# shanjiayao/PTT

Measured on AMD Instinct MI355X. Metric: tracklet frames/sec (hot path: PointNet++ SA stack + Point-Track-Transformer blocks), higher is better.
Workload: dtype f32

## Files before the change

include/ptt_hip.h:

```cpp
#ifndef PTT_HIP_H
#define PTT_HIP_H

#include <stddef.h>
#include <stdint.h>

#ifdef __cplusplus
extern "C" {
#endif

#define PTT_ABI_VERSION 31

enum {
    PTT_OK = 0,
    PTT_EINVAL = -1,
    PTT_EUNSUPPORTED = -2,
    PTT_ELAUNCH = -3,
    PTT_EWORKSPACE = -4
};

typedef void* ptt_stream_t;

int ptt_version(void);
const char* ptt_error_name(int code);
const char* ptt_last_error_string(void);

int ptt_fps_f32(const float* xyz, int B, int N, int npoint, int32_t* idx_out,
                ptt_stream_t stream);
int ptt_fps_ws_f32(const float* xyz, int B, int N, int npoint, int32_t* idx_out, float* workspace,
                   size_t workspace_elems, ptt_stream_t stream);

int ptt_ffps_f32(const float* xyz, const float* feat, int64_t feat_sb, int64_t feat_sc, int64_t feat_sn,
                 int B, int N, int C, int npoint, int32_t* idx_out, ptt_stream_t stream);

int ptt_gather_f32(const float* feat, const int32_t* idx, int B, int C, int N, int M,
                   float* out, ptt_stream_t stream);
int ptt_gather_grad_f32(const float* grad_out, const int32_t* idx, int B, int C, int N,
                        int M, float* grad_feat, ptt_stream_t stream);

int ptt_select_centres_f32(const float* xyz, const int32_t* idx, int B, int N, int M, float* new_xyz,
                           int64_t* idx64_out, ptt_stream_t stream);

int ptt_ball_query_f32(const float* new_xyz, const float* xyz, int B, int M, int N,
                       float radius, int nsample, int32_t* idx_out, ptt_stream_t stream);

int ptt_centres_ball_query_f32(const float* xyz, const int32_t* sel, int B, int N, int M, float radius, int nsample,
                               float* new_xyz, int64_t* idx64_out, int32_t* idx_out, ptt_stream_t stream);

int ptt_group_f32(const float* feat, const int32_t* idx, int B, int C, int N, int M,
                  int ns, float* out, ptt_stream_t stream);
int ptt_group_grad_f32(const float* grad_out, const int32_t* idx, int B, int C, int N,
                       int M, int ns, float* grad_feat, ptt_stream_t stream);

size_t ptt_scatter_add_det_workspace(int B, int N, int E);
int ptt_scatter_add_det_f32(const float* src, const int32_t* idx, int B, int C, int N, int E, float* out,
                            void* workspace, size_t workspace_bytes, ptt_stream_t stream);

int ptt_knn_f32(const float* xyz, int B, int N, int k, int32_t* idx_out,
                ptt_stream_t stream);
int ptt_knn_rel_f32(const float* xyz, int B, int N, int k, int32_t* idx_out, float* rel_out,
                    ptt_stream_t stream);

size_t ptt_packed_weight_elems(int Cout, int K);
int ptt_pack_weight_f32(const float* W, int Cout, int K, float* packed,
// ... 211 lines not shown
    float* template_points;
    float* cls_label;
    float* reg_label;
    int32_t* src_out;
    int32_t* idx_search_out;
    int32_t* idx_template_out;
    int32_t* info;
    int64_t* totals;
    int32_t B, n_cand;
    int32_t search_size, template_size;
    int32_t min_points;
    uint32_t seed_lo, seed_hi;
    int32_t reserved;
} ptt_train_batch_desc;

int ptt_train_batch_f32(const ptt_train_cand* cands_device, const ptt_train_batch_desc* desc_host, ptt_stream_t stream);
int ptt_philox4x32_10(const uint32_t* counter4, const uint32_t* key2, uint32_t* out4);

size_t ptt_bn_stats_workspace(int R, int C);
int ptt_bn_stats_f32(const float* X, int R, int C, int ldx, float eps, float* mean, float* var, float* invstd,
                     void* workspace, size_t workspace_bytes, ptt_stream_t stream);
int ptt_bn_apply_f32(const float* Z, int ldz, const float* mean, const float* invstd, const float* gamma,
                     const float* beta, int R, int C, int relu, float* X, int ldx, ptt_stream_t stream);
int ptt_bn_bwd_f32(const float* G, int ldg, const float* Act, int lda, const float* Z, int ldz, const float* mean,
                   const float* invstd, const float* gamma, int R, int C, int relu, float* dZ, int ldd,
                   float* dgamma, float* dbeta, void* workspace, size_t workspace_bytes, const float* act_scale,
                   const float* act_shift, ptt_stream_t stream);
int ptt_bn_sums_f64(const float* X, int R, int C, int ldx, double* sums, void* workspace, size_t workspace_bytes,
                    ptt_stream_t stream);
int ptt_bn_finish_f64(const double* sums, int C, float eps, float* mean, float* var, float* invstd,
                      ptt_stream_t stream);
int ptt_bn_bwd_sums_f64(const float* G, int ldg, const float* Act, int lda, const float* Z, int ldz, const float* mean,
                        const float* invstd, int R, int C, double* sums, void* workspace, size_t workspace_bytes,
                        const float* act_scale, const float* act_shift, ptt_stream_t stream);
int ptt_bn_bwd_apply_f32(const float* G, int ldg, const float* Act, int lda, const float* Z, int ldz, const float* mean,
                         const float* invstd, const float* gamma, const float* sum_dy, const float* sum_dy_xhat,
                         const double* count, int R, int C, float* dZ, int ldd, const float* act_scale, const float* act_shift,
                         ptt_stream_t stream);
int ptt_pool_rows_f32(const float* X, int ldx, int G, int ns, int C, float* out, int ldo, int32_t* arg,
                      const float* act_scale, const float* act_shift, ptt_stream_t stream);
int ptt_pool_rows_bwd_f32(const float* dOut, int ldo, const int32_t* arg, int G, int ns, int C, float* dX, int ldx,
                          ptt_stream_t stream);
int ptt_pt_pair_input_f32(const float* q, const float* kf, const int32_t* knn, const float* pos, int B, int N, int k, int D,
                          float* t, ptt_stream_t stream);
int ptt_pt_attn_train_fwd_f32(const float* a, const float* vf, const int32_t* knn, const float* pos, int B, int N, int k, int D,
                              float scale, float* attn, float* res, ptt_stream_t stream);
int ptt_pt_attn_train_bwd_f32(const float* attn, const float* vf, const int32_t* knn, const float* pos, const float* dres, int B,
                              int N, int k, int D, float scale, float* da, float* dvp, ptt_stream_t stream);

int ptt_pt_pair_input_ld_f32(const float* q, int ldq, const float* kf, int ldk, const int32_t* knn, const float* pos, int B, int N,
                             int k, int D, float* t, ptt_stream_t stream);
int ptt_pt_attn_fwd_ld_f32(const float* a, const float* vf, int ldv, const int32_t* knn, const float* pos, int B, int N, int k, int D,
                           float scale, float* attn, float* res, ptt_stream_t stream);

int ptt_gather_rows_f32(const float* src, const int32_t* idx, int B, int N, int E, int C, float* out, ptt_stream_t stream);
int ptt_scatter_csr_i32(const int32_t* idx, int B, int N, int E, int32_t* order, int32_t* start, ptt_stream_t stream);
int ptt_scatter_rows_csr_f32(const float* g, const int32_t* order, const int32_t* start, int B, int N, int E, int C,
                             float* out, ptt_stream_t stream);
int ptt_rows_gemm_pool_supported(int rows, int K, int N, int ldx, int ns);
int ptt_rows_gemm_pool_f32(const float* X, int rows, int K, int ldx, const float* in_scale, const float* in_shift,
                           const float* Wpacked, int N, float* out, int ldo, double* stats, size_t stats_elems, int ns,
                           float* pmax, float* pmin, int32_t* amax, int32_t* amin, ptt_stream_t stream);
int ptt_pool_select_f32(const float* pmax, const float* pmin, const int32_t* amax, const int32_t* amin, const float* act_scale,
                        const float* act_shift, int G, int C, float* out, int32_t* arg, ptt_stream_t stream);
size_t ptt_colsum_workspace(int R, int C);
int ptt_colsum_f32(const float* X, int R, int C, int ldx, float* out, void* workspace, size_t workspace_bytes, ptt_stream_t stream);
size_t ptt_linear_wgrad_workspace(int R, int Cout, int Cin);
int ptt_linear_wgrad_f32(const float* dZ, int ldz, const float* X, int ldx, int R, int Cout, int Cin, float* dW,
                         int accumulate, void* workspace, size_t workspace_bytes, const float* x_scale, const float* x_shift,
                         ptt_stream_t stream);
int ptt_linear_act_in_f32(const float* X, int rows, int K, int ldx, const float* in_scale, const float* in_shift,
                          const float* Wpacked, int Cout, float* out, int ldo, ptt_stream_t stream);

int ptt_pack_weight_strided_f32(const float* W, int Cout, int K, int64_t stride_out, int64_t stride_k, int batch,
                                int64_t stride_batch, float* packed, ptt_stream_t stream);
int ptt_linear_batched_f32(const float* X, int rows, int K, int ldx, int64_t x_batch_stride, const float* Wpacked,
                           int64_t w_batch_stride, int Cout, const float* scale, const float* shift, int relu,
                           const float* residual, int ldr, int64_t r_batch_stride, float* out, int ldo,
                           int64_t o_batch_stride, int batch, ptt_stream_t stream);
int ptt_softmax_rows_f32(float* X, int64_t rows, int n, int ld, float scale, ptt_stream_t stream);
int ptt_layernorm_f32(const float* x, int rows, int C, int ldx, const float* weight, const float* bias, float eps,
                      const float* residual, int ldr, float* out, int ldo, ptt_stream_t stream);

int ptt_rows_gemm_supported(int rows, int K, int N, int ldx, int ldo);
int ptt_rows_gemm_stat_chunks(int rows, int K, int N);
int ptt_rows_gemm_f32(const float* X, int rows, int K, int ldx, const float* in_scale, const float* in_shift,
                      const float* Wpacked, int N, const float* bias, int relu, const float* residual, int ldr,
                      float* out, int ldo, double* stats, size_t stats_elems, ptt_stream_t stream);
int ptt_rows_gemm_masked_f32(const float* X, int rows, int K, int ldx, const float* Wpacked, int N, const float* mask, int ldm,
                             float* out, int ldo, double* stats, size_t stats_elems, ptt_stream_t stream);
int ptt_rows_gemm_bnbwd_f32(const float* X, int rows, int K, int ldx, const float* Wpacked, int N, const float* Z, int ldz,
                            const float* mean, const float* invstd, const float* act_scale, const float* act_shift, float* out,
                            int ldo, double* sums_partial, size_t partial_elems, ptt_stream_t stream);
int ptt_bn_bwd_from_partials_f32(const double* partial, int chunks, const float* G, int ldg, const float* Z, int ldz, const float* mean,
                                 const float* invstd, const float* gamma, int R, int C, float* dZ, int ldd, float* dgamma, float* dbeta,
                                 const float* act_scale, const float* act_shift, ptt_stream_t stream);
int ptt_bn_bwd_sums_partials_f64(const double* partial, int chunks, int C, double* sums, ptt_stream_t stream);
typedef struct ptt_bn_bwd_input {
    const float* g; int ldg;
    const int32_t* arg; int ns;
    const float* z; int ldz;
    const float* k1; const float* c0; const float* c1; const float* mean;
    const float* act_a; const float* act_b;
    float* dz_out; int ldd;
} ptt_bn_bwd_input;
int ptt_bn_bwd_consts_f32(const double* partial, int chunks, const float* mean, const float* invstd, const float* gamma, int R, int C,
                          float* dgamma, float* dbeta, float* k1, float* c0, float* c1, ptt_stream_t stream);
int ptt_bn_bwd_pooled_consts_f32(const float* dPooled, int ldp, const int32_t* arg, int ns, const float* Z, int ldz, const float* mean,
                                 const float* invstd, const float* gamma, int R, int C, float* dgamma, float* dbeta, float* k1,
                                 float* c0, float* c1, void* workspace, size_t workspace_bytes, const float* act_scale,
                                 const float* act_shift, ptt_stream_t stream);
int ptt_rows_gemm_bnbwd_fused_supported(int rows, int K, int N, int ns);
int ptt_rows_gemm_bnbwd_fused_f32(const ptt_bn_bwd_input* in, int rows, int K, const float* Wpacked, int N, const float* Z, int ldz,
                                  const float* mean, const float* invstd, const float* act_scale, const float* act_shift, float* out,
                                  int ldo, double* sums_partial, size_t partial_elems, ptt_stream_t stream);
int ptt_bn_finish_partials_f32(const double* partial, int chunks, int C, int R, float eps, float* mean, float* var, float* invstd,
                               ptt_stream_t stream);
int ptt_bn_sums_partials_f64(const double* partial, int chunks, int C, int R, double* sums, ptt_stream_t stream);
int ptt_bn_bwd_pooled_f32(const float* dPooled, int ldp, const int32_t* arg, int ns, const float* Z, int ldz, const float* mean,
                          const float* invstd, const float* gamma, int R, int C, float* dZ, int ldd, float* dgamma, float* dbeta,
                          void* workspace, size_t workspace_bytes, const float* act_scale, const float* act_shift, ptt_stream_t stream);
int ptt_bn_bwd_pooled_sums_f64(const float* dPooled, int ldp, const int32_t* arg, int ns, const float* Z, int ldz, const float* mean,
                               const float* invstd, int R, int C, double* sums, void* workspace, size_t workspace_bytes,
                               const float* act_scale, const float* act_shift, ptt_stream_t stream);
int ptt_bn_bwd_pooled_apply_f32(const float* dPooled, int ldp, const int32_t* arg, int ns, const float* Z, int ldz, const float* mean,
                                const float* invstd, const float* gamma, const float* sum_dy, const float* sum_dy_xhat,
                                const double* count, int R, int C, float* dZ, int ldd, const float* act_scale,
                                const float* act_shift, ptt_stream_t stream);
int ptt_bn_update_running_f32(const float* mean, const float* var, const double* count, float momentum, int C, float* running_mean,
                              float* running_var, int64_t* num_batches_tracked, ptt_stream_t stream);
int ptt_xcorr_z0_f32(const float* P, const float* cos_t, const float* w_sim, int B, int n2, int n1, int C, float* z0, ptt_stream_t stream);
int ptt_xcorr_z0_stat_chunks(int B, int n2, int n1, int C);
int ptt_xcorr_z0_stats_f32(const float* P, const float* cos_t, const float* w_sim, int B, int n2, int n1, int C, float* z0,
                           double* stats_partial, size_t partial_elems, ptt_stream_t stream);
size_t ptt_xcorr_z0_bwd_workspace(int B, int n1, int C);
int ptt_xcorr_z0_bnbwd_f32(const double* partial, int chunks, const float* G, const float* P, const float* cos_t, const float* w_sim,
                           const float* mean, const float* invstd, const float* gamma, const float* act_scale, const float* act_shift,
                           int B, int n2, int n1, int C, float* dP, float* dcos, float* dw, float* dgamma, float* dbeta, void* workspace,
                           size_t workspace_bytes, ptt_stream_t stream);
int ptt_xcorr_z0_bwd_f32(const float* dz0, const float* cos_t, const float* w_sim, int B, int n2, int n1, int C, float* dP, float* dcos,
                         float* dw, void* workspace, size_t workspace_bytes, ptt_stream_t stream);
int ptt_sa_z0_rows_f32(const float* xyz, const float* new_xyz, const int32_t* idx, const float* term, const float* wx, int ldw, int B,
                       int N, int M, int ns, int C, float radius, int normalize_xyz, float* z0, float* rel_rows, ptt_stream_t stream);
int ptt_sa_z0_rows_stat_chunks(int B, int M, int ns, int C);
int ptt_sa_z0_rows_stats_f32(const float* xyz, const float* new_xyz, const int32_t* idx, const float* term, const float* wx, int ldw, int B,
                             int N, int M, int ns, int C, float radius, int normalize_xyz, float* z0, float* rel_rows,
                             double* stats_partial, size_t partial_elems, ptt_stream_t stream);
typedef struct ptt_bn_train_tail {
    const float* gamma; const float* beta;
    float* act_a; float* act_b;
    float* running_mean; float* running_var;
    int64_t* num_batches_tracked;
    float momentum;
} ptt_bn_train_tail;
int ptt_bn_stats_train_f32(const float* X, int R, int C, int ldx, float eps, float* mean, float* var, float* invstd,
                           void* workspace, size_t workspace_bytes, const ptt_bn_train_tail* tail, ptt_stream_t stream);
int ptt_bn_finish_partials_train_f32(const double* partial, int chunks, int C, int R, float eps, float* mean, float* var,
                                     float* invstd, const ptt_bn_train_tail* tail, ptt_stream_t stream);
typedef struct ptt_pack_job {
    const float* W;
    int64_t out_offset, stride_out, stride_k;
    int32_t Cout, K;
} ptt_pack_job;
int ptt_pack_weights_f32(const ptt_pack_job* jobs_device, int n_jobs, float* arena, ptt_stream_t stream);
size_t ptt_linear_wgrad2_workspace(int R, int Cout, int Cin);
int ptt_linear_wgrad2_f32(const float* dZ, int ldz, const float* X, int ldx, int R, int Cout, int Cin, float* dW,
                          int accumulate, void* workspace, size_t workspace_bytes, const float* x_scale, const float* x_shift,
                          ptt_stream_t stream);

typedef struct ptt_track_loss_desc {
    const float* seed_cls;
    const float* cls_label;
    const int64_t* search_inds;
    const float* votes;
    const float* reg_label;
    const float* box_data;
    const float* centres;
    const float* pos_weight_seed;
    const float* pos_weight_box;
    int32_t B, N, Ns, M, ld_reg;
    float w_seed_cls, w_seed_reg, w_box_cls, w_box_reg;
} ptt_track_loss_desc;
int ptt_track_losses_f32(const ptt_track_loss_desc* desc, float* out8, float* total , ptt_stream_t stream);
int ptt_track_losses_bwd_f32(const ptt_track_loss_desc* desc, const float* out8, const float* upstream, float* d_seed_cls,
                             float* d_votes, float* d_box_data, ptt_stream_t stream);
typedef struct ptt_adam_tensor {
    float* param;
    float* grad;
    float* exp_avg;
    float* exp_avg_sq;
    int64_t n;
} ptt_adam_tensor;
typedef struct ptt_adam_hyper {
    float beta1, beta2, one_minus_beta1, one_minus_beta2 , eps, step_size, bias2_sqrt,
          weight_decay, max_norm;
    int32_t write_clipped;
} ptt_adam_hyper;
int ptt_adam_chunk_elems(void);
int ptt_adam_clip_step_f32(const ptt_adam_tensor* tensors_device, const int32_t* chunk_tensor_device, const int64_t* chunk_first_device,
                           int n_chunks, const ptt_adam_hyper* hyper, double* partial, size_t partial_elems, float* norm_out,
                           ptt_stream_t stream);
int ptt_adam_clip_step_dev_f32(const ptt_adam_tensor* tensors_device, const int32_t* chunk_tensor_device, const int64_t* chunk_first_device,
                               int n_chunks, const ptt_adam_hyper* hyper_device, int clip, double* partial, size_t partial_elems,
                               float* norm_out, ptt_stream_t stream);
int ptt_unit_rows_f32(const float* x, long long sb, long long sn, long long sc, int B, int n, int C, float eps, float* unit, float* nrm,
                      ptt_stream_t stream);
int ptt_cos_bwd_rows_f32(const float* A, const float* unit, const float* nrm, const float* G, const float* cosm, long long map_sb,
                         long long own, long long other, int m, int B, int n, int C, float* dx, long long sb, long long sn, long long sc,
                         ptt_stream_t stream);
size_t ptt_sa_z0_bnbwd_workspace(long long R, int C);
int ptt_sa_z0_bnbwd_f32(const double* partial, int chunks, const float* G, const float* Z0, const float* rel_rows, const float* mean,
                        const float* invstd, const float* gamma, const float* act_scale, const float* act_shift, long long R, int C,
                        float* dz_out, float* dwx, float* dgamma, float* dbeta, void* workspace, size_t workspace_bytes, ptt_stream_t stream);

typedef struct ptt_grad_job {
    const float* partial;
    int32_t nchunks, reserved;
} ptt_grad_job;
typedef struct ptt_grad_segment {
    int64_t dst;
    int32_t n, cols, ld, job0, njobs, out, vec, reserved;
} ptt_grad_segment;
int ptt_linear_wgrad_partials_f32(const float* dZ, int ldz, const float* X, int ldx, int R, int Cout, int Cin, void* workspace,
                                  size_t workspace_bytes, const float* x_scale, const float* x_shift, int* nchunks, ptt_stream_t stream);
int ptt_linear_wgrad2_partials_f32(const float* dZ, int ldz, const float* X, int ldx, int R, int Cout, int Cin, void* workspace,
                                   size_t workspace_bytes, const float* x_scale, const float* x_shift, int* nchunks, ptt_stream_t stream);
int ptt_colsum_partials_f32(const float* X, int R, int C, int ldx, void* workspace, size_t workspace_bytes, int* nchunks,
                            ptt_stream_t stream);
int ptt_grad_finish_f32(const ptt_grad_segment* segments_device, const ptt_grad_job* jobs_device, const int32_t* blocks_device,
                        int n_blocks, float* flat, ptt_stream_t stream);

int ptt_rows_gemm_rsum16_supported(int rows, int K, int N, int ldx);
int ptt_rows_gemm_rsum16_f32(const float* X, int rows, int K, int ldx, const float* Wpacked, int N, const float* residual, int ldr,
                             float* out, int ldo, float* plain, int ldp, float* gsum, int ldg, ptt_stream_t stream);
int ptt_scatter_rows_csr_sub_f32(const float* g, const int32_t* order, const int32_t* start, int B, int N, int E, int C,
                                 const float* minuend, float* out, ptt_stream_t stream);

int ptt_layernorm_train_fwd_f32(const float* x, int rows, int C, int ldx, const float* weight, const float* bias, float eps,
                                const float* residual, int ldr, float* out, int ldo, float* mean, float* rstd, ptt_stream_t stream);
size_t ptt_layernorm_bwd_workspace(int rows, int C);
int ptt_layernorm_bwd_f32(const float* dy, int ldg, const float* x, int ldx, const float* mean, const float* rstd, const float* weight,
                          int rows, int C, float* dx, int ldd, float* dweight, float* dbias, void* workspace, size_t workspace_bytes,
                          ptt_stream_t stream);
int ptt_rows_gemm_rsum16_heads_supported(int rows, int D, int hd, int ldx);
int ptt_rows_gemm_rsum16_heads_f32(const float* X, int rows, int D, int hd, int ldx, const float* Wpacked, const float* residual, int ldr,
                                   float* out, int ldo, float* plain, int ldp, float* gsum, int ldg, ptt_stream_t stream);

#ifdef __cplusplus
}
#endif
#endif
```

ptt_amd/_lib.py:

```python
import ctypes
import os
import re
from ctypes import Structure, c_char_p, c_double, c_float, c_int, c_int32, c_int64, c_longlong, c_size_t, c_uint32, c_void_p

from .build import HEADER as HEADER_PATH, LIB as LIB_PATH


def _strip_comments(text):
    return re.sub(r"/\*.*?\*/|//[^\n]*", " ", text, flags=re.S)


def parse_defines(text):
    return {n: int(v) for n, v in re.findall(r"^[ \t]*#[ \t]*define[ \t]+(PTT_\w+)[ \t]+(-?\d+)[ \t]*$", _strip_comments(text), re.M)}


CTYPES = {"int": c_int, "int32_t": c_int32, "uint32_t": c_uint32, "int64_t": c_int64, "long long": c_longlong, "size_t": c_size_t,
          "float": c_float, "double": c_double, "ptt_stream_t": c_void_p}


def _ctype(decl, name, is_return=False):
    words = decl.replace("*", " * ").split()
    if not is_return and len(words) > 1 and words[-1] != "*":
        words.pop()
    if "*" in words:
# ... 37 lines not shown
EXPORTS = list(PROTOTYPES)
DEFINES = parse_defines(_header)
ABI_VERSION = DEFINES["PTT_ABI_VERSION"]
PTT_SA_MAX_LAYERS = DEFINES["PTT_SA_MAX_LAYERS"]
PTT_MAX_SEGMENTS = DEFINES["PTT_MAX_SEGMENTS"]
PTT_CROP_JOBS_BY_VALUE_MAX = DEFINES["PTT_CROP_JOBS_BY_VALUE_MAX"]
PTT_TRAIN_MAX_CANDS = DEFINES["PTT_TRAIN_MAX_CANDS"]


class CropJob(Structure):
    _fields_ = [("points", c_void_p), ("ld", c_int64),
                ("lo1", c_double * 3), ("hi1", c_double * 3), ("trans", c_double * 3), ("rot", c_double * 9),
                ("lo2", c_double * 3), ("hi2", c_double * 3),
                ("out", c_void_p), ("count", c_void_p), ("n_points", c_int32), ("capacity", c_int32),
                ("label_out", c_void_p), ("ltrans", c_double * 3), ("lrot", c_double * 9), ("llo", c_double * 3), ("lhi", c_double * 3),
                ("append", c_int32), ("reserved", c_int32)]


class RegularizeJob(Structure):
    _fields_ = [("seg", c_void_p * PTT_MAX_SEGMENTS), ("seg_count", c_void_p * PTT_MAX_SEGMENTS),
                ("seg_capacity", c_int32 * PTT_MAX_SEGMENTS), ("out", c_void_p), ("info", c_void_p),
                ("n_seg", c_int32), ("input_size", c_int32)]


class TrackBox(Structure):
    _fields_ = [("center", c_double * 3), ("wlh", c_double * 3), ("quat", c_double * 4)]


class TrainCand(Structure):
    _fields_ = [("search", c_void_p), ("label", c_void_p), ("first", c_void_p), ("prev", c_void_p), ("counts", c_void_p),
                ("reg", c_float * 4), ("index", c_uint32), ("epoch", c_uint32), ("capacity", c_int32), ("reserved", c_int32)]


class TrainBatchDesc(Structure):
    _fields_ = [("search_points", c_void_p), ("template_points", c_void_p), ("cls_label", c_void_p), ("reg_label", c_void_p),
                ("src_out", c_void_p), ("idx_search_out", c_void_p), ("idx_template_out", c_void_p), ("info", c_void_p), ("totals", c_void_p),
                ("B", c_int32), ("n_cand", c_int32), ("search_size", c_int32), ("template_size", c_int32), ("min_points", c_int32),
                ("seed_lo", c_uint32), ("seed_hi", c_uint32), ("reserved", c_int32)]


class BnTrainTail(Structure):
    _fields_ = [("gamma", c_void_p), ("beta", c_void_p), ("act_a", c_void_p), ("act_b", c_void_p),
                ("running_mean", c_void_p), ("running_var", c_void_p), ("num_batches_tracked", c_void_p), ("momentum", c_float)]


class BnBwdInput(Structure):
    _fields_ = [("g", c_void_p), ("ldg", c_int), ("arg", c_void_p), ("ns", c_int), ("z", c_void_p), ("ldz", c_int),
                ("k1", c_void_p), ("c0", c_void_p), ("c1", c_void_p), ("mean", c_void_p), ("act_a", c_void_p), ("act_b", c_void_p),
                ("dz_out", c_void_p), ("ldd", c_int)]


class PackJob(Structure):
    _fields_ = [("W", c_void_p), ("out_offset", c_int64), ("stride_out", c_int64), ("stride_k", c_int64),
                ("Cout", c_int32), ("K", c_int32)]


class RowJob(Structure):
    _fields_ = [("X", c_void_p), ("X2", c_void_p), ("Xmax", c_void_p), ("Wpacked", c_void_p), ("scale", c_void_p), ("shift", c_void_p),
                ("res", c_void_p), ("res2", c_void_p), ("out", c_void_p), ("out2", c_void_p), ("raw", c_void_p),
                ("rel", c_void_p), ("w1", c_void_p), ("qkv", c_void_p), ("knn", c_void_p), ("pos", c_void_p),
                ("rows", c_int32), ("K", c_int32), ("K1", c_int32), ("ldx", c_int32), ("ldx2", c_int32), ("Cout", c_int32),
                ("act", c_int32), ("res_split", c_int32), ("ldr", c_int32), ("ldr2", c_int32), ("out_split", c_int32),
                ("out_col0", c_int32), ("ldo", c_int32), ("ldo2", c_int32), ("ldraw", c_int32),
                ("prologue", c_int32), ("epilogue", c_int32), ("ldq", c_int32), ("q_off", c_int32), ("k_off", c_int32),
                ("v_off", c_int32), ("ldp", c_int32), ("N", c_int32), ("sm_scale", c_float), ("col_tiles", c_int32),
                ("idx", c_void_p), ("xyz", c_void_p), ("centres", c_void_p), ("wx", c_void_p), ("radius", c_float),
                ("ns", c_int32), ("M", c_int32), ("normalize_xyz", c_int32), ("pro_relu", c_int32)]


class PointJob(Structure):
    _fields_ = [("xyz", c_void_p), ("centre_sel", c_void_p), ("point_sel", c_void_p), ("new_xyz", c_void_p), ("idx64_out", c_void_p),
                ("idx_out", c_void_p), ("rel_out", c_void_p), ("kind", c_int32), ("sel_ld", c_int32), ("B", c_int32),
                ("Nraw", c_int32), ("Npts", c_int32), ("M", c_int32), ("nsample", c_int32), ("radius", c_float)]


class TrackLossDesc(Structure):
    _fields_ = [("seed_cls", c_void_p), ("cls_label", c_void_p), ("search_inds", c_void_p), ("votes", c_void_p), ("reg_label", c_void_p),
                ("box_data", c_void_p), ("centres", c_void_p), ("pos_weight_seed", c_void_p), ("pos_weight_box", c_void_p),
                ("B", c_int32), ("N", c_int32), ("Ns", c_int32), ("M", c_int32), ("ld_reg", c_int32),
                ("w_seed_cls", c_float), ("w_seed_reg", c_float), ("w_box_cls", c_float), ("w_box_reg", c_float)]


class AdamTensor(Structure):
    _fields_ = [("param", c_void_p), ("grad", c_void_p), ("exp_avg", c_void_p), ("exp_avg_sq", c_void_p), ("n", c_int64)]


class GradJob(Structure):
    _fields_ = [("partial", c_void_p), ("nchunks", c_int32), ("reserved", c_int32)]


class GradSegment(Structure):
    _fields_ = [("dst", c_int64), ("n", c_int32), ("cols", c_int32), ("ld", c_int32), ("job0", c_int32), ("njobs", c_int32), ("out", c_int32),
                ("vec", c_int32), ("reserved", c_int32)]


class AdamHyper(Structure):
    _fields_ = [("beta1", c_float), ("beta2", c_float), ("one_minus_beta1", c_float), ("one_minus_beta2", c_float), ("eps", c_float), ("step_size", c_float), ("bias2_sqrt", c_float),
                ("weight_decay", c_float), ("max_norm", c_float), ("write_clipped", c_int32)]


class SaLayer(Structure):
    _fields_ = [("Wpacked", c_void_p), ("scale", c_void_p), ("shift", c_void_p),
                ("Cin", c_int), ("Cout", c_int), ("relu", c_int)]


class SaDesc(Structure):
    _fields_ = [("xyz", c_void_p), ("new_xyz", c_void_p), ("idx", c_void_p), ("feat", c_void_p),
# ... 58 lines not shown
```

ptt_amd/csrc/gemm_ops.hip:

```cpp
#include <atomic>
#include <math.h>
#include <stdlib.h>
#include <type_traits>
#include "common.h"

namespace ptt {

typedef float g32x16 __attribute__((ext_vector_type(16)));
typedef float g32x4 __attribute__((ext_vector_type(4)));
typedef int gi32x4 __attribute__((ext_vector_type(4)));
typedef unsigned int gu32x4 __attribute__((__vector_size__(4 * sizeof(unsigned int))));

namespace {

__device__ __forceinline__ __amdgpu_buffer_rsrc_t g_rsrc(const void* p) {
    return __builtin_amdgcn_make_buffer_rsrc(const_cast<void*>(p), 0, 0x7fffffff, 0x00020000);
}
__device__ __forceinline__ g32x4 g_load4(__amdgpu_buffer_rsrc_t r, int voff, int soff) {
    return __builtin_bit_cast(g32x4, __builtin_amdgcn_raw_buffer_load_b128(r, voff, soff, 0));
}
__device__ __forceinline__ float g_load1(__amdgpu_buffer_rsrc_t r, int voff, int soff) {
    return __builtin_bit_cast(float, __builtin_amdgcn_raw_buffer_load_b32(r, voff, soff, 0));
}
__device__ __forceinline__ void g_store1(float v, __amdgpu_buffer_rsrc_t r, int voff, int soff) {
// ... 500 lines not shown
void launch_wgrad_finish(const float* partial, int nchunks, size_t n, int accumulate, float* dW, hipStream_t s);

static int cu_count() {
    constexpr int MAX_DEV = 64;
    static std::atomic<int> cached[MAX_DEV];
    int dev = 0;
    if (hipGetDevice(&dev) != hipSuccess || dev < 0 || dev >= MAX_DEV) return 256;
    int n = cached[dev].load(std::memory_order_relaxed);
    if (n == 0) {
        int v = 0;
        n = (hipDeviceGetAttribute(&v, hipDeviceAttributeMultiprocessorCount, dev) == hipSuccess && v > 0) ? v : 256;
        cached[dev].store(n, std::memory_order_relaxed);
    }
    return n;
}

struct RowsGemmGeom { int WR, RT, CT, KC, TR, ncg, ntiles, G, chunks; bool ok; };
static RowsGemmGeom rows_gemm_geom(int rows, int K, int N) {
    RowsGemmGeom g{};
    g.ok = false;
    if (rows <= 0 || K <= 0 || N <= 0) return g;
    if (N % 128 == 0 && K % 128 == 0) {
        const int tiles64 = (rows + 63) / 64;
        g.WR = 1; g.RT = 2; g.KC = 128;
        g.CT = (N % 256 == 0 && (long long)tiles64 * (N / 256) >= 2 * cu_count()) ? 2 : 1;
    }
    else if (N % 128 == 0 && K % 64 == 0) { g.WR = 1; g.RT = 4; g.CT = 1; g.KC = 64; }
    else if (N % 64 == 0 && K % 64 == 0) { g.WR = 2; g.RT = 2; g.CT = 1; g.KC = 64; }
    else return g;
    const int WC = 4 / g.WR;
    g.TR = 32 * g.RT * g.WR;
    g.ncg = N / (32 * WC * g.CT);
    g.ntiles = (rows + g.TR - 1) / g.TR;
    int cap = 2 * cu_count() / g.ncg;
    if (cap >= 8) cap &= ~7;
    if (cap < 1) cap = 1;
    g.G = g.ntiles < cap ? g.ntiles : cap;
    g.chunks = g.G * g.WR;
    g.ok = true;
    return g;
}

}

using namespace ptt;

extern "C" int ptt_rows_gemm_supported(int rows, int K, int N, int ldx, int ldo) {
    const RowsGemmGeom g = rows_gemm_geom(rows, K, N);
    if (!g.ok) return 0;
    if ((long long)rows * ldx >= (1LL << 29) || (long long)rows * ldo >= (1LL << 29) || (ldx & 3)) return 0;
    return 1;
}

extern "C" int ptt_rows_gemm_stat_chunks(int rows, int K, int N) {
    const RowsGemmGeom g = rows_gemm_geom(rows, K, N);
    return g.ok ? g.chunks : 0;
}

struct BnBwdArgs { const float* z; int ldz; const float* mean; const float* invstd; const float* a; const float* b; };
struct PoolArgs { float* pmax; float* pmin; int32_t* amax; int32_t* amin; int ns; };
struct GroupSumArgs { float* gsum; int ldgs; float* plain; int ldpl; int hd; };
static int rows_gemm_launch(const float* X, int rows, int K, int ldx, const float* in_scale, const float* in_shift,
                            const float* Wpacked, int N, const float* bias, int relu, const float* residual, int ldr,
                            const float* mask, int ldm, float* out, int ldo, double* stats, size_t stats_elems, ptt_stream_t stream,
                            const BnBwdArgs* bn = nullptr, const PoolArgs* pool = nullptr, const ptt_bn_bwd_input* ain = nullptr,
                            const GroupSumArgs* gs = nullptr);

extern "C" int ptt_rows_gemm_rsum16_supported(int rows, int K, int N, int ldx) {
    if (!ptt_rows_gemm_supported(rows, K, N, ldx, N) || rows % 16) return 0;
    const RowsGemmGeom g = rows_gemm_geom(rows, K, N);
    return (g.WR == 1 && g.RT == 2 && g.KC == 128) ? 1 : 0;
}

extern "C" int ptt_rows_gemm_rsum16_f32(const float* X, int rows, int K, int ldx, const float* Wpacked, int N, const float* residual,
                                        int ldr, float* out, int ldo, float* plain, int ldp, float* gsum, int ldg,
                                        ptt_stream_t stream) {
    if (!residual || !plain || !gsum || ldp < N || ldg < N) return fail(PTT_EINVAL, "ptt_rows_gemm_rsum16_f32: null pointer or ldp / ldg < N");
    if ((long long)rows * ldp >= (1LL << 31)) return fail(PTT_EUNSUPPORTED, "ptt_rows_gemm_rsum16_f32: rows * ldp >= 2^31");
    if (!ptt_rows_gemm_rsum16_supported(rows, K, N, ldx))
        return fail(PTT_EUNSUPPORTED, "ptt_rows_gemm_rsum16_f32: rows=%d K=%d N=%d (whole groups of 16 rows, K %% 128 == 0, N %% 128 == 0)", rows, K, N);
    const GroupSumArgs gs{gsum, ldg, plain, ldp, 0};
    return rows_gemm_launch(X, rows, K, ldx, nullptr, nullptr, Wpacked, N, nullptr, 0, residual, ldr, nullptr, 0, out, ldo, nullptr, 0, stream,
                            nullptr, nullptr, nullptr, &gs);
}

extern "C" int ptt_rows_gemm_rsum16_heads_supported(int rows, int D, int hd, int ldx) {
    if (hd <= 0 || D <= 0 || D % hd || hd % 128) return 0;
    return ptt_rows_gemm_rsum16_supported(rows, D, D, ldx);
}

extern "C" int ptt_rows_gemm_rsum16_heads_f32(const float* X, int rows, int D, int hd, int ldx, const float* Wpacked, const float* residual,
                                              int ldr, float* out, int ldo, float* plain, int ldp, float* gsum, int ldg,
                                              ptt_stream_t stream) {
    if (!residual || !plain || !gsum || ldp < D || ldg < D)
        return fail(PTT_EINVAL, "ptt_rows_gemm_rsum16_heads_f32: null pointer or ldp / ldg < D");
    if ((long long)rows * ldp >= (1LL << 31)) return fail(PTT_EUNSUPPORTED, "ptt_rows_gemm_rsum16_heads_f32: rows * ldp >= 2^31");
    if (!ptt_rows_gemm_rsum16_heads_supported(rows, D, hd, ldx))
        return fail(PTT_EUNSUPPORTED, "ptt_rows_gemm_rsum16_heads_f32: rows=%d D=%d hd=%d (whole groups of 16 rows, D %% hd == 0, hd %% 128 == 0)",
                    rows, D, hd);
    const GroupSumArgs gs{gsum, ldg, plain, ldp, hd};
    return rows_gemm_launch(X, rows, D, ldx, nullptr, nullptr, Wpacked, D, nullptr, 0, residual, ldr, nullptr, 0, out, ldo, nullptr, 0, stream,
                            nullptr, nullptr, nullptr, &gs);
}

extern "C" int ptt_rows_gemm_bnbwd_fused_supported(int rows, int K, int N, int ns) {
    if (!ptt_rows_gemm_supported(rows, K, N, K, N) || (ns != 0 && ns != 16 && ns != 32 && ns != 64) || (ns > 0 && rows % ns)) return 0;
// ... 197 lines not shown
        else if (stats) PTT_RG_LAUNCH(WR_, RT_, CT_, KC_, true, false)                                                  \
        else if (in_scale) PTT_RG_LAUNCH(WR_, RT_, CT_, KC_, false, true)                                               \
        else PTT_RG_LAUNCH(WR_, RT_, CT_, KC_, false, false)                                                            \
    }
    PTT_RG_CASE(1, 2, 2, 128, PTT_RG_AINS) PTT_RG_CASE(1, 2, 1, 128, PTT_RG_AINS) PTT_RG_CASE(1, 4, 1, 64, PTT_RG_NO_AINS)
    PTT_RG_CASE(2, 2, 1, 64, PTT_RG_AINS)
#undef PTT_RG_CASE
#undef PTT_RG_AINS
#undef PTT_RG_NO_AINS
#undef PTT_RG_AIN
#undef PTT_RG_LAUNCH
    return check_launch("rows_gemm_kernel");
}

namespace ptt {
#ifndef PTT_WG2_MIN_ROWS
#define PTT_WG2_MIN_ROWS 768
#endif
struct Wgrad2Geom { int TN, TK, BN, BK, nbo, nbk, chunk_rows, nchunks; bool ok; };
static Wgrad2Geom wgrad2_geom(int R, int Cout, int Cin) {
    Wgrad2Geom g{};
    g.ok = false;
    if (R < 2048 || Cout % 128 || Cin % 128) return g;
    const int ncu = cu_count();
    const int cand[4][2] = {{4, 2}, {4, 1}, {2, 2}, {2, 1}};
    int first = 0;
#ifdef PTT_GEMM_DEV
    if (const char* e = getenv("PTT_WG2_FIRST")) first = atoi(e);
#endif
    for (int k = first; k < 4; ++k) {
        const int TN = cand[k][0], TK = cand[k][1];
        if (Cout % (64 * TN) || Cin % (128 * TK)) continue;
        const int blocks = (Cout / (64 * TN)) * (Cin / (128 * TK));
        if (blocks > ncu) continue;
        int nch = ncu / blocks;
        int rows = (R + nch - 1) / nch;
        if (rows < PTT_WG2_MIN_ROWS) rows = PTT_WG2_MIN_ROWS;
        rows = (rows + 31) & ~31;
        const int nchunks = (R + rows - 1) / rows;
        if (nchunks * blocks * 4 < ncu * 3 && k < 3) continue;
        if (nchunks * blocks * 2 < ncu) break;
        g.TN = TN; g.TK = TK; g.BN = 64 * TN; g.BK = 128 * TK; g.nbo = Cout / g.BN; g.nbk = Cin / g.BK;
        g.chunk_rows = rows; g.nchunks = nchunks; g.ok = true;
        return g;
    }
    return g;
}
}

extern "C" size_t ptt_linear_wgrad2_workspace(int R, int Cout, int Cin) {
    const Wgrad2Geom g = wgrad2_geom(R, Cout, Cin);
    return g.ok ? (size_t)g.nchunks * Cout * Cin * sizeof(float) : 0;
}

static int linear_wgrad2_run(const float* dZ, int ldz, const float* X, int ldx, int R, int Cout, int Cin, float* dW,
                             int accumulate, void* ws, size_t ws_bytes, const float* x_scale, const float* x_shift,
                             int* nchunks_out, ptt_stream_t stream) {
    const Wgrad2Geom g = wgrad2_geom(R, Cout, Cin);
    if (!g.ok || (ldz & 3) || (ldx & 3) || ((reinterpret_cast<uintptr_t>(dZ) | reinterpret_cast<uintptr_t>(X)) & 15) ||
        (long long)R * ldz >= (1LL << 29) || (long long)R * ldx >= (1LL << 29))
        return fail(PTT_EUNSUPPORTED, "ptt_linear_wgrad2_f32: R=%d Cout=%d Cin=%d ldz=%d ldx=%d (needs R >= 2048, Cout %% 128 == 0, "
                                      "Cin %% 128 == 0, 16-byte aligned rows)", R, Cout, Cin, ldz, ldx);
    if (ldz < Cout || ldx < Cin || !dZ || !X || (!dW && !nchunks_out)) return fail(PTT_EINVAL, "ptt_linear_wgrad2_f32: bad argument");
    if (x_scale && (!x_shift || ((reinterpret_cast<uintptr_t>(x_scale) | reinterpret_cast<uintptr_t>(x_shift)) & 15)))
        return fail(PTT_EINVAL, "ptt_linear_wgrad2_f32: the input transform needs 16-byte aligned scale / shift");
    if (!ws || ws_bytes < ptt_linear_wgrad2_workspace(R, Cout, Cin)) return fail(PTT_EWORKSPACE, "ptt_linear_wgrad2_f32: workspace too small");
    hipStream_t s = as_stream(stream);
    const int lds = 2 * 32 * (g.BN + 4 + g.BK + 4) * (int)sizeof(float);
    const dim3 grid(g.nbo * g.nbk * g.nchunks);
    int rc = PTT_OK;
#define PTT_WG2_CASE(TN_, TK_)                                                                                          \
    if (g.TN == TN_ && g.TK == TK_) {                                                                                   \
        if ((rc = set_lds_limit(reinterpret_cast<const void*>(wgrad2_kernel<TN_, TK_>), lds))) return rc;               \
        hipLaunchKernelGGL((wgrad2_kernel<TN_, TK_>), grid, dim3(512), lds, s, dZ, ldz, X, ldx, R, Cout, Cin, g.nbk, g.chunk_rows, \
                           static_cast<float*>(ws), x_scale, x_shift);                                                  \
    }
#ifdef PTT_GEMM_DEV
    if (const char* e = getenv("PTT_WG2_EXP")) {
        const int x = atoi(e);
#define PTT_WG2_EXP_CASE(X)                                                                                             \
        if (x == X && g.TN == 4 && g.TK == 2) {                                                                         \
            if ((rc = set_lds_limit(reinterpret_cast<const void*>(wgrad2_kernel<4, 2, X>), lds))) return rc;            \
            hipLaunchKernelGGL((wgrad2_kernel<4, 2, X>), grid, dim3(512), lds, s, dZ, ldz, X_, ldx, R, Cout, Cin, g.nbk, g.chunk_rows, \
                               static_cast<float*>(ws), x_scale, x_shift);                                              \
            return check_launch("wgrad2_kernel(exp)");                                                                  \
        }
        const float* X_ = X;
        PTT_WG2_EXP_CASE(1) PTT_WG2_EXP_CASE(2) PTT_WG2_EXP_CASE(3) PTT_WG2_EXP_CASE(4) PTT_WG2_EXP_CASE(7) PTT_WG2_EXP_CASE(8)
        PTT_WG2_EXP_CASE(15) PTT_WG2_EXP_CASE(16) PTT_WG2_EXP_CASE(31)
#undef PTT_WG2_EXP_CASE
    }
#endif
    PTT_WG2_CASE(4, 2) PTT_WG2_CASE(4, 1) PTT_WG2_CASE(2, 2) PTT_WG2_CASE(2, 1)
#undef PTT_WG2_CASE
    if (dW) launch_wgrad_finish(static_cast<const float*>(ws), g.nchunks, (size_t)Cout * Cin, accumulate, dW, s);
    if (nchunks_out) *nchunks_out = g.nchunks;
    return check_launch("wgrad2_kernel");
}
extern "C" int ptt_linear_wgrad2_f32(const float* dZ, int ldz, const float* X, int ldx, int R, int Cout, int Cin, float* dW,
                                     int accumulate, void* ws, size_t ws_bytes, const float* x_scale, const float* x_shift,
                                     ptt_stream_t stream) {
    if (!dW) return fail(PTT_EINVAL, "ptt_linear_wgrad2_f32: bad argument");
    return linear_wgrad2_run(dZ, ldz, X, ldx, R, Cout, Cin, dW, accumulate, ws, ws_bytes, x_scale, x_shift, nullptr, stream);
}
extern "C" int ptt_linear_wgrad2_partials_f32(const float* dZ, int ldz, const float* X, int ldx, int R, int Cout, int Cin, void* ws,
                                              size_t ws_bytes, const float* x_scale, const float* x_shift, int* nchunks,
                                              ptt_stream_t stream) {
    if (!nchunks) return fail(PTT_EINVAL, "ptt_linear_wgrad2_partials_f32: null pointer");
    return linear_wgrad2_run(dZ, ldz, X, ldx, R, Cout, Cin, nullptr, 0, ws, ws_bytes, x_scale, x_shift, nchunks, stream);
}
```

ptt_amd/csrc/mfma_ops.hip:

```cpp
#include <math.h>
#include <stdlib.h>
#include <string.h>
#include "common.h"
#include "mfma_common.h"

#ifndef PTT_PAIR_PF
#define PTT_PAIR_PF 1
#endif
#ifndef PTT_GATHER_BATCH
#define PTT_GATHER_BATCH 16
#endif
#ifndef PTT_SA_WAVES
#define PTT_SA_WAVES 2
#endif

namespace ptt {

#ifdef PTT_DEV
#define PTT_STAMP(i) do { if (p.dbg && threadIdx.x == 0 && blockIdx.x < 4096) p.dbg[blockIdx.x * 8 + (i)] = __builtin_readcyclecounter(); } while (0)
#else
#define PTT_STAMP(i) do { } while (0)
#endif

__device__ __forceinline__ void stagger_second_slot(int first_wave_blocks, int quanta) {
    if ((int)blockIdx.x < first_wave_blocks && quanta > 0) {
        const unsigned alloc = __builtin_amdgcn_s_getreg((31 << 11) | (0 << 6) | 6);
        const unsigned lds_base = alloc & 0xffu, lds_size = (alloc >> 12) & 0x1ffu;
        int slot = lds_size ? (int)(lds_base / lds_size) : 0;
        if (lds_base != 0 && slot == 0) slot = 1;
        for (int i = 0; i < slot * quanta; ++i) __builtin_amdgcn_s_sleep(127);
    }
}

#ifndef PTT_LINEAR_PF
#define PTT_LINEAR_PF 0
#endif
#ifndef PTT_XCD_REMAP
#define PTT_XCD_REMAP 1
#endif
__device__ __forceinline__ int logical_block() {
#if PTT_XCD_REMAP
    const int bid = blockIdx.x, per = (int)gridDim.x >> 3;
    if (bid >= (per << 3)) return bid;
    return (bid & 7) * per + (bid >> 3);
#else
    return blockIdx.x;
#endif
}

__global__ void pack_weight_kernel(const float* __restrict__ W, int Cout, int K, int NT, int rot, size_t total,
                                   float* __restrict__ P, long long so, long long sk, long long sb) {
    const float* Wb = W + (size_t)blockIdx.y * sb;
    float* Pb = P + (size_t)blockIdx.y * total;
    for (size_t e = (size_t)blockIdx.x * blockDim.x + threadIdx.x; e < total; e += (size_t)gridDim.x * blockDim.x) {
        const int j = (int)(e & 3);
        const int lane = (int)((e >> 2) & 63);
        const size_t tile = e >> 8;
        const int ct = (int)(tile % NT);
        const int kb = (int)(tile / NT);
        const int col = ct * 32 + (lane & 31);
        const int k = kb * 8 + 4 * (lane >> 5) + j;
        Pb[e] = (col < Cout && k < K) ? Wb[(size_t)col * so + (size_t)((k + rot) % K) * sk] : 0.0f;
    }
}

__global__ __launch_bounds__(256) void pack_weights_kernel(const ptt_pack_job* __restrict__ jobs, float* __restrict__ arena) {
    const ptt_pack_job jb = jobs[blockIdx.y];
    const int NT = (jb.Cout + 31) / 32;
    const size_t total = (size_t)NT * (size_t)((jb.K + 7) / 8) * 256;
    float* Pb = arena + jb.out_offset;
    for (size_t e = (size_t)blockIdx.x * blockDim.x + threadIdx.x; e < total; e += (size_t)gridDim.x * blockDim.x) {
        const int j = (int)(e & 3);
        const int lane = (int)((e >> 2) & 63);
        const size_t tile = e >> 8;
        const int ct = (int)(tile % NT);
        const int kb = (int)(tile / NT);
        const int col = ct * 32 + (lane & 31);
        const int k = kb * 8 + 4 * (lane >> 5) + j;
        Pb[e] = (col < jb.Cout && k < jb.K) ? jb.W[(long long)col * jb.stride_out + (long long)k * jb.stride_k] : 0.0f;
    }
}

#ifndef PTT_BUFFER_WEIGHTS
#define PTT_BUFFER_WEIGHTS 1
#endif
template <int RT, int CT, int ACT>
__device__ __forceinline__ void gemm_mfma_block(const f32x4 (&a)[RT], const f32x4 (&b)[CT], f32x16 (&acc)[RT][ACT]) {
#pragma unroll
    for (int j = 0; j < 4; ++j)
#pragma unroll
        for (int u = 0; u < CT; ++u)
#pragma unroll
            for (int rt = 0; rt < RT; ++rt)
                acc[rt][u] = __builtin_amdgcn_mfma_f32_32x32x2f32(a[rt][j], b[u][j], acc[rt][u], 0, 0, 0);
}

template <int RT, int CT, int ACT, int CTS = 4, int PF = 1>
__device__ __forceinline__ void gemm_core(const float* Xs, int ldk, int nkb, const f32x4* __restrict__ Wp, int NT,
                                          int ct0, int lane, f32x16 (&acc)[RT][ACT], const f32x4* pre = nullptr) {
    static_assert(CT <= ACT, "accumulator array too narrow");
    const int row = lane & 31, half = lane >> 5;
    const float* arow = Xs + row * ldk + 4 * half;
    const f32x4* bp = Wp + (size_t)ct0 * 64 + lane;
    const size_t bstep = (size_t)NT * 64;
#if PTT_BUFFER_WEIGHTS
    const __amdgpu_buffer_rsrc_t wr = weight_rsrc(Wp);
    const int wvoff = (ct0 * 64 + lane) * 16;
    const int wkstep = NT * 1024;
#define PTT_WFRAG(KB, U) weight_load(wr, wvoff, (KB) * wkstep + (U) * CTS * 1024)
#else
#define PTT_WFRAG(KB, U) (bp[(size_t)(KB) * bstep + (size_t)(U) * CTS * 64])
#endif

    if constexpr (PF == 0) {
        f32x4 a0[RT], a1[RT], b0[CT], b1[CT];
#define PTT_LOAD_BLOCK(A, Bv, KB)                                                             \
        {                                                                                     \
            _Pragma("unroll") for (int u = 0; u < CT; ++u) Bv[u] = PTT_WFRAG(KB, u);          \
            _Pragma("unroll") for (int rt = 0; rt < RT; ++rt)                                 \
                A[rt] = *reinterpret_cast<const f32x4*>(arow + rt * 32 * ldk + (KB) * 8);     \
        }
        if (pre) {
#pragma unroll
            for (int u = 0; u < CT; ++u) b0[u] = pre[u];
#pragma unroll
            for (int rt = 0; rt < RT; ++rt) a0[rt] = *reinterpret_cast<const f32x4*>(arow + rt * 32 * ldk);
        } else {
            PTT_LOAD_BLOCK(a0, b0, 0)
        }
        int kb = 0;
#pragma unroll 1
        for (; kb + 2 < nkb; kb += 2) {
// ... 2207 lines not shown
```

ptt_amd/csrc/train_ops.hip:

```cpp
#include <math.h>
#include "common.h"

namespace ptt {

typedef float f32x4t __attribute__((ext_vector_type(4)));
typedef float f32x16t __attribute__((ext_vector_type(16)));

constexpr int ST_ROWS = 2048;

template <int MODE>
__global__ __launch_bounds__(256) void col_stats_kernel(const float* __restrict__ X, const float* __restrict__ Act,
                                                        const float* __restrict__ Z, const float* __restrict__ mean,
                                                        const float* __restrict__ invstd, int R, int C, int ldx, int lda,
                                                        int ldz, double* __restrict__ partial) {
    __shared__ double red[2][4][64];
    const int lane = threadIdx.x & 63, rg = threadIdx.x >> 6;
    const int r0 = blockIdx.x * ST_ROWS, r1 = min(R, r0 + ST_ROWS);
    for (int cg = 0; cg * 64 < C; ++cg) {
        const int c = cg * 64 + lane;
        double s0 = 0.0, s1 = 0.0;
        if (c < C) {
            float mu = 0.f, is = 0.f;
            if (MODE == 1) { mu = mean[c]; is = invstd[c]; }
            for (int r = r0 + rg; r < r1; r += 4) {
// ... 954 lines not shown
__global__ __launch_bounds__(256) void sa_z0_rows_kernel(const float* __restrict__ xyz, const float* __restrict__ new_xyz,
                                                         const int32_t* __restrict__ idx, const float* __restrict__ term,
                                                         const float* __restrict__ wx, int ldw, int N, int M, int ns, int C,
                                                         float rmul, float* __restrict__ z0, float* __restrict__ rel_out,
                                                         double* __restrict__ stats) {
#pragma clang fp contract(off)
    __shared__ double red[2][256][4];
    const int Cq = C >> 2, span = Cq < 256 ? Cq : 256, RG = 256 / span;
    const int q0 = threadIdx.x % span, rg = threadIdx.x / span;
    const int b = blockIdx.y, E = M * ns;
    const float* xb = xyz + (size_t)b * N * 3;
    const float* cb = new_xyz + (size_t)b * M * 3;
    const float* tb = term ? term + (size_t)b * N * C : nullptr;
    const int32_t* ib = idx + (size_t)b * E;
    float* zb = z0 + (size_t)b * E * C;
    float* rb = rel_out + (size_t)b * E * 3;
    double s1[4] = {0.0, 0.0, 0.0, 0.0}, s2[4] = {0.0, 0.0, 0.0, 0.0};
    if (rg < RG) {
        for (int e = blockIdx.x * RG + rg; e < E; e += gridDim.x * RG) {
            const int n = ib[e], m = e / ns;
            const float rx = (xb[3 * n + 0] - cb[3 * m + 0]) * rmul, ry = (xb[3 * n + 1] - cb[3 * m + 1]) * rmul,
                        rz = (xb[3 * n + 2] - cb[3 * m + 2]) * rmul;
            if (q0 == 0) { rb[3 * e + 0] = rx; rb[3 * e + 1] = ry; rb[3 * e + 2] = rz; }
            for (int q = q0; q < Cq; q += span) {
                f32x4t v = tb ? *reinterpret_cast<const f32x4t*>(tb + (size_t)n * C + 4 * q) : f32x4t{0.f, 0.f, 0.f, 0.f};
#pragma unroll
                for (int j = 0; j < 4; ++j) {
                    const float* w = wx + (size_t)(4 * q + j) * ldw;
                    const float y = __builtin_fmaf(w[2], rz, __builtin_fmaf(w[1], ry, w[0] * rx));
                    v[j] = v[j] + y;
                    if (stats) { s1[j] += (double)v[j]; s2[j] += (double)v[j] * (double)v[j]; }
                }
                *reinterpret_cast<f32x4t*>(zb + (size_t)e * C + 4 * q) = v;
            }
        }
    }
    if (!stats) return;
#pragma unroll
    for (int j = 0; j < 4; ++j) { red[0][threadIdx.x][j] = s1[j]; red[1][threadIdx.x][j] = s2[j]; }
    __syncthreads();
    if (rg == 0) {
        double* sp = stats + ((size_t)blockIdx.y * gridDim.x + blockIdx.x) * 2 * C;
#pragma unroll
        for (int j = 0; j < 4; ++j) {
            double t1 = 0.0, t2 = 0.0;
            for (int g = 0; g < RG; ++g) { t1 += red[0][g * span + q0][j]; t2 += red[1][g * span + q0][j]; }
            sp[4 * q0 + j] = t1; sp[C + 4 * q0 + j] = t2;
        }
    }
}

__global__ __launch_bounds__(256) void scatter_rows_det_kernel(const float* __restrict__ g, const int32_t* __restrict__ order,
                                                               const int32_t* __restrict__ start, int N, int E, int C,
                                                               float* __restrict__ out, const float* __restrict__ minuend, int negate) {
    const int Cq = C >> 2, span = Cq < 256 ? Cq : 256, RG = 256 / span;
    const int q0 = threadIdx.x % span, rg = threadIdx.x / span;
    if (rg >= RG) return;
    const int b = blockIdx.y;
    const float* gb = g + (size_t)b * E * C;
    const int32_t* ob = order + (size_t)b * E;
    const int32_t* st = start + (size_t)b * (N + 1);
    for (int n = blockIdx.x * RG + rg; n < N; n += gridDim.x * RG) {
        const int k0 = st[n], k1 = st[n + 1];
        for (int q = q0; q < Cq; q += span) {
            f32x4t acc = {0.f, 0.f, 0.f, 0.f};
            int k = k0;
            for (; k + 3 < k1; k += 4) {
                const int e0 = ob[k], e1 = ob[k + 1], e2 = ob[k + 2], e3 = ob[k + 3];
                const f32x4t v0 = *reinterpret_cast<const f32x4t*>(gb + (size_t)e0 * C + 4 * q);
                const f32x4t v1 = *reinterpret_cast<const f32x4t*>(gb + (size_t)e1 * C + 4 * q);
                const f32x4t v2 = *reinterpret_cast<const f32x4t*>(gb + (size_t)e2 * C + 4 * q);
                const f32x4t v3 = *reinterpret_cast<const f32x4t*>(gb + (size_t)e3 * C + 4 * q);
#pragma unroll
                for (int x = 0; x < 4; ++x) acc[x] = (((acc[x] + v0[x]) + v1[x]) + v2[x]) + v3[x];
            }
            for (; k < k1; ++k) {
                const f32x4t v = *reinterpret_cast<const f32x4t*>(gb + (size_t)ob[k] * C + 4 * q);
                acc[0] += v[0]; acc[1] += v[1]; acc[2] += v[2]; acc[3] += v[3];
            }
            if (negate) {
                f32x4t m = {0.f, 0.f, 0.f, 0.f};
                if (minuend) m = *reinterpret_cast<const f32x4t*>(minuend + ((size_t)b * N + n) * C + 4 * q);
#pragma unroll
                for (int x = 0; x < 4; ++x) acc[x] = m[x] - acc[x];
            }
            *reinterpret_cast<f32x4t*>(out + ((size_t)b * N + n) * C + 4 * q) = acc;
        }
    }
}

__global__ __launch_bounds__(256) void sa_z0_bnbwd_kernel(const float* __restrict__ G, const float* __restrict__ Z0,
                                                          const float* __restrict__ rel, const float* __restrict__ mean,
                                                          const float* __restrict__ invstd, const float* __restrict__ gamma,
                                                          const float* __restrict__ s0, const float* __restrict__ s1,
                                                          const float* __restrict__ act_a, const float* __restrict__ act_b, float rinv,
                                                          long long R, int C, int rows_per_wg, float* dz_out,
                                                          float* __restrict__ dwx_partial) {
    __shared__ float red[256][12];
    const int Cq = C >> 2, span = Cq < 256 ? Cq : 256, RG = 256 / span;
    const int q = threadIdx.x % span, rg = threadIdx.x / span;
    float wacc[4][3];
#pragma unroll
    for (int x = 0; x < 4; ++x) wacc[x][0] = wacc[x][1] = wacc[x][2] = 0.f;
    if (rg < RG) {
        const f32x4t mu = *reinterpret_cast<const f32x4t*>(mean + 4 * q), is = *reinterpret_cast<const f32x4t*>(invstd + 4 * q);
        const f32x4t ga = *reinterpret_cast<const f32x4t*>(gamma + 4 * q);
        const f32x4t a0 = *reinterpret_cast<const f32x4t*>(s0 + 4 * q), a1 = *reinterpret_cast<const f32x4t*>(s1 + 4 * q);
        const f32x4t ca = *reinterpret_cast<const f32x4t*>(act_a + 4 * q), cb = *reinterpret_cast<const f32x4t*>(act_b + 4 * q);
        auto dz_of = [&](const f32x4t& g, const f32x4t& z) {
            f32x4t d;
#pragma unroll
            for (int x = 0; x < 4; ++x) {
                const float dy = __builtin_fmaf(z[x], ca[x], cb[x]) > 0.f ? g[x] : 0.f;
                const float xh = (z[x] - mu[x]) * is[x];
                d[x] = ga[x] * is[x] * (dy - a0[x] * rinv - xh * (a1[x] * rinv));
            }
            return d;
        };
        const long long r0 = (long long)blockIdx.x * rows_per_wg, r1 = r0 + rows_per_wg < R ? r0 + rows_per_wg : R;
        long long r = r0 + rg;
        for (; r + 3LL * RG < r1; r += 4LL * RG) {
            f32x4t g[4], z[4];
            float rl[4][3];
#pragma unroll
            for (int u = 0; u < 4; ++u) {
                const long long e = r + (long long)u * RG;
                g[u] = *reinterpret_cast<const f32x4t*>(G + e * C + 4 * q);
                z[u] = *reinterpret_cast<const f32x4t*>(Z0 + e * C + 4 * q);
                rl[u][0] = rel[e * 3 + 0]; rl[u][1] = rel[e * 3 + 1]; rl[u][2] = rel[e * 3 + 2];
            }
#pragma unroll
            for (int u = 0; u < 4; ++u) {
                const f32x4t d = dz_of(g[u], z[u]);
                if (dz_out) *reinterpret_cast<f32x4t*>(dz_out + (r + (long long)u * RG) * C + 4 * q) = d;
#pragma unroll
                for (int x = 0; x < 4; ++x) {
                    wacc[x][0] = __builtin_fmaf(d[x], rl[u][0], wacc[x][0]);
                    wacc[x][1] = __builtin_fmaf(d[x], rl[u][1], wacc[x][1]);
                    wacc[x][2] = __builtin_fmaf(d[x], rl[u][2], wacc[x][2]);
// ... 47 lines not shown
            const f32x4t pv = *reinterpret_cast<const f32x4t*>(pos + (pt * KN + j) * D + c);
            f32x4t o;
#pragma unroll
            for (int x = 0; x < 4; ++x) o[x] = (qv[x] - kv[x]) + pv[x];
            *reinterpret_cast<f32x4t*>(t + (pt * KN + j) * D + c) = o;
        }
    }
}

template <int KN>
__global__ __launch_bounds__(256) void attn_fwd_kernel(const float* __restrict__ a, const float* __restrict__ vf,
                                                       const int32_t* __restrict__ knn, const float* __restrict__ pos, int N, int D,
                                                       long long total_pts, float scale, float* __restrict__ attn,
                                                       float* __restrict__ res, int ldv) {
    const int Dq = D >> 2;
    for (long long e = (long long)blockIdx.x * 256 + threadIdx.x; e < total_pts * Dq; e += (long long)gridDim.x * 256) {
        const long long pt = e / Dq;
        const int c = (int)(e - pt * Dq) * 4;
        const long long b = pt / N;
        f32x4t av[KN];
        f32x4t m = {-3.0e38f, -3.0e38f, -3.0e38f, -3.0e38f};
#pragma unroll
        for (int j = 0; j < KN; ++j) {
            av[j] = *reinterpret_cast<const f32x4t*>(a + (pt * KN + j) * D + c);
#pragma unroll
            for (int x = 0; x < 4; ++x) { av[j][x] *= scale; m[x] = fmaxf(m[x], av[j][x]); }
        }
        f32x4t sum = {0.f, 0.f, 0.f, 0.f};
#pragma unroll
        for (int j = 0; j < KN; ++j)
#pragma unroll
            for (int x = 0; x < 4; ++x) { av[j][x] = __expf(av[j][x] - m[x]); sum[x] += av[j][x]; }
        f32x4t inv, acc = {0.f, 0.f, 0.f, 0.f};
#pragma unroll
        for (int x = 0; x < 4; ++x) inv[x] = 1.0f / sum[x];
#pragma unroll
        for (int j = 0; j < KN; ++j) {
            const int n = knn[pt * KN + j];
            const f32x4t vv = *reinterpret_cast<const f32x4t*>(vf + (b * N + n) * ldv + c);
            const f32x4t pv = *reinterpret_cast<const f32x4t*>(pos + (pt * KN + j) * D + c);
            f32x4t w;
#pragma unroll
            for (int x = 0; x < 4; ++x) { w[x] = av[j][x] * inv[x]; acc[x] += w[x] * (vv[x] + pv[x]); }
            if (attn) *reinterpret_cast<f32x4t*>(attn + (pt * KN + j) * D + c) = w;
        }
        *reinterpret_cast<f32x4t*>(res + pt * D + c) = acc;
    }
}

template <int KN>
__global__ __launch_bounds__(256) void attn_bwd_kernel(const float* __restrict__ attn, const float* __restrict__ vf,
                                                       const int32_t* __restrict__ knn, const float* __restrict__ pos,
                                                       const float* __restrict__ dres, int N, int D, long long total_pts, float scale,
                                                       float* __restrict__ da, float* __restrict__ dvp) {
    const int Dq = D >> 2;
    for (long long e = (long long)blockIdx.x * 256 + threadIdx.x; e < total_pts * Dq; e += (long long)gridDim.x * 256) {
        const long long pt = e / Dq;
        const int c = (int)(e - pt * Dq) * 4;
        const long long b = pt / N;
        const f32x4t g = *reinterpret_cast<const f32x4t*>(dres + pt * D + c);
        f32x4t w[KN], dat[KN];
        f32x4t s = {0.f, 0.f, 0.f, 0.f};
#pragma unroll
        for (int j = 0; j < KN; ++j) {
            const int n = knn[pt * KN + j];
            w[j] = *reinterpret_cast<const f32x4t*>(attn + (pt * KN + j) * D + c);
            const f32x4t vv = *reinterpret_cast<const f32x4t*>(vf + (b * N + n) * D + c);
            const f32x4t pv = *reinterpret_cast<const f32x4t*>(pos + (pt * KN + j) * D + c);
            f32x4t o;
#pragma unroll
            for (int x = 0; x < 4; ++x) { dat[j][x] = g[x] * (vv[x] + pv[x]); s[x] += w[j][x] * dat[j][x]; o[x] = w[j][x] * g[x]; }
            *reinterpret_cast<f32x4t*>(dvp + (pt * KN + j) * D + c) = o;
        }
#pragma unroll
        for (int j = 0; j < KN; ++j) {
            f32x4t o;
#pragma unroll
            for (int x = 0; x < 4; ++x) o[x] = w[j][x] * (dat[j][x] - s[x]) * scale;
            *reinterpret_cast<f32x4t*>(da + (pt * KN + j) * D + c) = o;
        }
    }
}

void launch_wgrad_finish(const float* partial, int nchunks, size_t n, int accumulate, float* dW, hipStream_t s) {
    const int out = nchunks > 1024 ? 4 : nchunks > 256 ? 8 : nchunks > 64 ? 16 : nchunks > 8 ? 32 : nchunks > 2 ? 64 : 256;
    size_t fgrid = (n + out - 1) / out;
    if (fgrid > 4096) fgrid = 4096;
#define PTT_WF(O) if (out == O) hipLaunchKernelGGL(wgrad_finish_kernel<O>, dim3((unsigned)fgrid), dim3(256), 0, s, partial, nchunks, n, accumulate, dW);
    PTT_WF(4) PTT_WF(8) PTT_WF(16) PTT_WF(32) PTT_WF(64) PTT_WF(256)
#undef PTT_WF
}

constexpr int LNT_VPL = 16, LNB_ROWS = 32;

__device__ __forceinline__ float ln_wave_sum(float v) {
#pragma unroll
    for (int o = 32; o > 0; o >>= 1) v += __shfl_xor(v, o, 64);
    return v;
}

__global__ __launch_bounds__(256) void layernorm_train_fwd_kernel(const float* __restrict__ X, int rows, int C, int ldx,
                                                                  const float* __restrict__ weight, const float* __restrict__ bias,
                                                                  float eps, const float* __restrict__ R, int ldr,
                                                                  float* __restrict__ Y, int ldy, float* __restrict__ mean_out,
                                                                  float* __restrict__ rstd_out) {
    const int lane = threadIdx.x & 63;
    const int r = blockIdx.x * 4 + (threadIdx.x >> 6);
    if (r >= rows) return;
    const float* x = X + (size_t)r * ldx;
    float v[LNT_VPL];
    float sum = 0.f;
#pragma unroll
    for (int i = 0; i < LNT_VPL; ++i) {
        const int c = lane + 64 * i;
        v[i] = c < C ? x[c] : 0.f;
        sum += v[i];
    }
    const float mean0 = ln_wave_sum(sum) / (float)C;
    float rest = 0.f;
#pragma unroll
// ... 368 lines not shown
extern "C" int ptt_gather_rows_f32(const float* src, const int32_t* idx, int B, int N, int E, int C, float* out,
                                   ptt_stream_t stream) {
    if (B < 0 || N <= 0 || E < 0 || C <= 0 || (C & 3)) return fail(PTT_EINVAL, "ptt_gather_rows_f32: B=%d N=%d E=%d C=%d (C %% 4)", B, N, E, C);
    if (B == 0 || E == 0) return PTT_OK;
    if (!src || !idx || !out || ((reinterpret_cast<uintptr_t>(src) | reinterpret_cast<uintptr_t>(out)) & 15))
        return fail(PTT_EINVAL, "ptt_gather_rows_f32: null or unaligned pointer");
    const int Cq = C >> 2, RG = 256 / (Cq < 256 ? Cq : 256);
    int gx = (E + RG * 4 - 1) / (RG * 4);
    if (gx > 4096) gx = 4096;
    hipLaunchKernelGGL(gather_rows_kernel, dim3(gx, B), dim3(256), 0, as_stream(stream), src, idx, N, E, C, out);
    return check_launch("gather_rows_kernel");
}

static inline int sa_z0_grid(int B, int M, int ns, int C, bool stats) {
    const int E = M * ns, Cq = C >> 2, RG = 256 / (Cq < 256 ? Cq : 256);
    int gx = (E + RG * 4 - 1) / (RG * 4);
    if (gx > 4096) gx = 4096;
    if (stats) { const int cap = (4096 + B - 1) / B; if (gx > cap) gx = cap; }
    return gx;
}
extern "C" int ptt_sa_z0_rows_stat_chunks(int B, int M, int ns, int C) {
    if (B <= 0 || M <= 0 || ns <= 0 || C <= 0 || (C & 3) || C > 1024) return 0;
    return sa_z0_grid(B, M, ns, C, true) * B;
}
static int sa_z0_rows_launch(const float* xyz, const float* new_xyz, const int32_t* idx, const float* term, const float* wx,
                             int ldw, int B, int N, int M, int ns, int C, float radius, int normalize_xyz, float* z0,
                             float* rel_rows, double* stats, ptt_stream_t stream) {
    if (B < 0 || N <= 0 || M <= 0 || ns <= 0 || C <= 0 || (C & 3) || !(radius > 0.f) || ldw < 3)
        return fail(PTT_EINVAL, "ptt_sa_z0_rows_f32: B=%d N=%d M=%d ns=%d C=%d (C %% 4) radius=%g", B, N, M, ns, C, (double)radius);
    if ((long long)M * ns > 0x7fffffffLL / 4) return fail(PTT_EUNSUPPORTED, "ptt_sa_z0_rows_f32: M * ns = %lld rows per cloud", (long long)M * ns);
    if (stats && C > 1024) return fail(PTT_EUNSUPPORTED, "ptt_sa_z0_rows_stats_f32: C=%d (at most 1024 channels)", C);
    if (B == 0) return PTT_OK;
    if (!xyz || !new_xyz || !idx || !wx || !z0 || !rel_rows ||
        ((reinterpret_cast<uintptr_t>(z0) | reinterpret_cast<uintptr_t>(term)) & 15))
        return fail(PTT_EINVAL, "ptt_sa_z0_rows_f32: null or unaligned pointer");
    hipLaunchKernelGGL(sa_z0_rows_kernel, dim3(sa_z0_grid(B, M, ns, C, stats != nullptr), B), dim3(256), 0, as_stream(stream), xyz, new_xyz, idx, term, wx, ldw,
                       N, M, ns, C, normalize_xyz ? 1.0f / radius : 1.0f, z0, rel_rows, stats);
    return check_launch("sa_z0_rows_kernel");
}
extern "C" int ptt_sa_z0_rows_f32(const float* xyz, const float* new_xyz, const int32_t* idx, const float* term, const float* wx,
                                  int ldw, int B, int N, int M, int ns, int C, float radius, int normalize_xyz, float* z0,
                                  float* rel_rows, ptt_stream_t stream) {
    return sa_z0_rows_launch(xyz, new_xyz, idx, term, wx, ldw, B, N, M, ns, C, radius, normalize_xyz, z0, rel_rows, nullptr, stream);
}
extern "C" int ptt_sa_z0_rows_stats_f32(const float* xyz, const float* new_xyz, const int32_t* idx, const float* term, const float* wx,
                                        int ldw, int B, int N, int M, int ns, int C, float radius, int normalize_xyz, float* z0,
                                        float* rel_rows, double* stats_partial, size_t partial_elems, ptt_stream_t stream) {
    if (!stats_partial || partial_elems < (size_t)ptt_sa_z0_rows_stat_chunks(B, M, ns, C) * 2 * (size_t)C)
        return fail(PTT_EWORKSPACE, "ptt_sa_z0_rows_stats_f32: the partial sums need %d x 2 x %d doubles", ptt_sa_z0_rows_stat_chunks(B, M, ns, C), C);
    return sa_z0_rows_launch(xyz, new_xyz, idx, term, wx, ldw, B, N, M, ns, C, radius, normalize_xyz, z0, rel_rows, stats_partial, stream);
}

static int scatter_rows_run(const float* g, const int32_t* order, const int32_t* start, int B, int N, int E, int C, float* out,
                            const float* minuend, int negate, ptt_stream_t stream) {
    if (B < 0 || N <= 0 || E < 0 || C <= 0 || (C & 3)) return fail(PTT_EINVAL, "ptt_scatter_rows_csr_f32: B=%d N=%d E=%d C=%d", B, N, E, C);
    if (B == 0) return PTT_OK;
    if (!g || !order || !start || !out || ((reinterpret_cast<uintptr_t>(g) | reinterpret_cast<uintptr_t>(out) | reinterpret_cast<uintptr_t>(minuend)) & 15))
        return fail(PTT_EINVAL, "ptt_scatter_rows_csr_f32: null or unaligned pointer");
    const int Cq = C >> 2, RG = 256 / (Cq < 256 ? Cq : 256);
    int gx = (N + RG - 1) / RG;
    if (gx > 4096) gx = 4096;
    hipLaunchKernelGGL(scatter_rows_det_kernel, dim3(gx, B), dim3(256), 0, as_stream(stream), g, order, start, N, E, C, out, minuend, negate);
    return check_launch("scatter_rows_det_kernel");
}
extern "C" int ptt_scatter_rows_csr_f32(const float* g, const int32_t* order, const int32_t* start, int B, int N, int E, int C,
                                        float* out, ptt_stream_t stream) {
    return scatter_rows_run(g, order, start, B, N, E, C, out, nullptr, 0, stream);
}
extern "C" int ptt_scatter_rows_csr_sub_f32(const float* g, const int32_t* order, const int32_t* start, int B, int N, int E, int C,
                                            const float* minuend, float* out, ptt_stream_t stream) {
    return scatter_rows_run(g, order, start, B, N, E, C, out, minuend, 1, stream);
}

static int pt_train_check(const char* what, int B, int N, int k, int D, const void* p0, const void* p1, const void* p2, const void* p3) {
    if (B < 0 || N <= 0 || D <= 0 || (D & 3)) return fail(PTT_EINVAL, "%s: B=%d N=%d D=%d (D %% 4)", what, B, N, D);
    if (k != 8 && k != 16 && k != 32) return fail(PTT_EUNSUPPORTED, "%s: k=%d (8, 16 and 32 neighbours are instantiated)", what, k);
    if (B > 0 && (!p0 || !p1 || !p2 || !p3)) return fail(PTT_EINVAL, "%s: null pointer", what);
    return PTT_OK;
}

#define PTT_PAIR_EW(KERNEL, ...)                                                                                                 \
    do {                                                                                                                         \
        const dim3 g_(ew_grid((size_t)pts * (D >> 2)));                                                                          \
        if (k == 8) hipLaunchKernelGGL((KERNEL<8>), g_, dim3(256), 0, as_stream(stream), __VA_ARGS__);                           \
        else if (k == 16) hipLaunchKernelGGL((KERNEL<16>), g_, dim3(256), 0, as_stream(stream), __VA_ARGS__);                    \
        else hipLaunchKernelGGL((KERNEL<32>), g_, dim3(256), 0, as_stream(stream), __VA_ARGS__);                                 \
    } while (0)

extern "C" int ptt_pt_pair_input_f32(const float* q, const float* kf, const int32_t* knn, const float* pos, int B, int N, int k,
                                     int D, float* t, ptt_stream_t stream) {
    if (int rc = pt_train_check("ptt_pt_pair_input_f32", B, N, k, D, q, kf, knn, pos)) return rc;
    if (B == 0) return PTT_OK;
    if (!t) return fail(PTT_EINVAL, "ptt_pt_pair_input_f32: null pointer");
    const long long pts = (long long)B * N;
    PTT_PAIR_EW(pair_input_kernel, q, kf, knn, pos, N,
                       D, pts, t, D, D);
    return check_launch("pair_input_kernel");
}

extern "C" int ptt_pt_pair_input_ld_f32(const float* q, int ldq, const float* kf, int ldk, const int32_t* knn, const float* pos, int B,
                                        int N, int k, int D, float* t, ptt_stream_t stream) {
    if (int rc = pt_train_check("ptt_pt_pair_input_ld_f32", B, N, k, D, q, kf, knn, pos)) return rc;
    if (ldq < D || ldk < D || (ldq & 3) || (ldk & 3)) return fail(PTT_EINVAL, "ptt_pt_pair_input_ld_f32: ldq=%d ldk=%d", ldq, ldk);
    if (B == 0) return PTT_OK;
    if (!t) return fail(PTT_EINVAL, "ptt_pt_pair_input_ld_f32: null pointer");
    const long long pts = (long long)B * N;
    PTT_PAIR_EW(pair_input_kernel, q, kf, knn, pos, N,
                       D, pts, t, ldq, ldk);
    return check_launch("pair_input_kernel");
}

extern "C" int ptt_pt_attn_fwd_ld_f32(const float* a, const float* vf, int ldv, const int32_t* knn, const float* pos, int B, int N, int k,
                                      int D, float scale, float* attn, float* res, ptt_stream_t stream) {
    if (int rc = pt_train_check("ptt_pt_attn_fwd_ld_f32", B, N, k, D, a, vf, knn, pos)) return rc;
    if (ldv < D || (ldv & 3)) return fail(PTT_EINVAL, "ptt_pt_attn_fwd_ld_f32: ldv=%d", ldv);
    if (B == 0) return PTT_OK;
    if (!res) return fail(PTT_EINVAL, "ptt_pt_attn_fwd_ld_f32: null pointer");
    const long long pts = (long long)B * N;
    PTT_PAIR_EW(attn_fwd_kernel, a, vf, knn, pos, N, D,
                       pts, scale, attn, res, ldv);
    return check_launch("attn_fwd_kernel");
}

extern "C" int ptt_pt_attn_train_fwd_f32(const float* a, const float* vf, const int32_t* knn, const float* pos, int B, int N, int k,
                                         int D, float scale, float* attn, float* res, ptt_stream_t stream) {
    if (int rc = pt_train_check("ptt_pt_attn_train_fwd_f32", B, N, k, D, a, vf, knn, pos)) return rc;
    if (B == 0) return PTT_OK;
    if (!attn || !res) return fail(PTT_EINVAL, "ptt_pt_attn_train_fwd_f32: null pointer");
    const long long pts = (long long)B * N;
    PTT_PAIR_EW(attn_fwd_kernel, a, vf, knn, pos, N, D,
                       pts, scale, attn, res, D);
    return check_launch("attn_fwd_kernel");
}

extern "C" int ptt_pt_attn_train_bwd_f32(const float* attn, const float* vf, const int32_t* knn, const float* pos, const float* dres,
                                         int B, int N, int k, int D, float scale, float* da, float* dvp, ptt_stream_t stream) {
    if (int rc = pt_train_check("ptt_pt_attn_train_bwd_f32", B, N, k, D, attn, vf, knn, pos)) return rc;
    if (B == 0) return PTT_OK;
    if (!dres || !da || !dvp) return fail(PTT_EINVAL, "ptt_pt_attn_train_bwd_f32: null pointer");
    const long long pts = (long long)B * N;
    PTT_PAIR_EW(attn_bwd_kernel, attn, vf, knn, pos,
                       dres, N, D, pts, scale, da, dvp);
    return check_launch("attn_bwd_kernel");
}

#undef PTT_PAIR_EW

static inline bool wgrad_smallk_ok(int Cout, int Cin) { return Cin >= 1 && Cin <= 4 && (Cout & 3) == 0; }

static inline int colsum_rows_per_chunk(int R, int C) {
    const int colblocks = (C + 255) / 256;
    int chunks = 512 / colblocks;
    int rows = (R + chunks - 1) / chunks;
    if (rows < CS_ROWS) rows = CS_ROWS;
    return (rows + 3) / 4 * 4;
}
extern "C" size_t ptt_colsum_workspace(int R, int C) {
    if (R <= 0 || C <= 0) return 0;
    const int rows = colsum_rows_per_chunk(R, C);
    return (size_t)((R + rows - 1) / rows) * (size_t)C * sizeof(float);
}
static int colsum_run(const float* X, int R, int C, int ldx, float* out, void* ws, size_t ws_bytes, int* nchunks_out, ptt_stream_t stream) {
    if (R <= 0 || C <= 0 || ldx < C) return fail(PTT_EINVAL, "ptt_colsum_f32: R=%d C=%d ldx=%d", R, C, ldx);
    if (!X || (!out && !nchunks_out)) return fail(PTT_EINVAL, "ptt_colsum_f32: null pointer");
    const int rows = colsum_rows_per_chunk(R, C), nch = (R + rows - 1) / rows;
    hipStream_t s2 = as_stream(stream);
    if ((nch > 1 || !out) && (!ws || ws_bytes < ptt_colsum_workspace(R, C))) return fail(PTT_EWORKSPACE, "ptt_colsum_f32: workspace too small");
    float* part = (nch == 1 && out) ? out : static_cast<float*>(ws);
    const bool vec = !(C & 3) && !(ldx & 3) && !((reinterpret_cast<uintptr_t>(X) | reinterpret_cast<uintptr_t>(part)) & 15);
    if (vec) hipLaunchKernelGGL(colsum_partial_kernel, dim3(nch, (C / 4 + 63) / 64), dim3(256), 0, s2, X, ldx, R, C, rows, part);
    else hipLaunchKernelGGL(colsum_partial_scalar_kernel, dim3(nch, (C + 63) / 64), dim3(256), 0, s2, X, ldx, R, C, rows, part);
    if (nch > 1 && out) launch_wgrad_finish(part, nch, (size_t)C, 0, out, s2);
    if (nchunks_out) *nchunks_out = nch;
    return check_launch("colsum_partial_kernel");
}
extern "C" int ptt_colsum_f32(const float* X, int R, int C, int ldx, float* out, void* ws, size_t ws_bytes, ptt_stream_t stream) {
    if (!out) return fail(PTT_EINVAL, "ptt_colsum_f32: null pointer");
    return colsum_run(X, R, C, ldx, out, ws, ws_bytes, nullptr, stream);
}
extern "C" int ptt_colsum_partials_f32(const float* X, int R, int C, int ldx, void* ws, size_t ws_bytes, int* nchunks, ptt_stream_t stream) {
    if (!nchunks) return fail(PTT_EINVAL, "ptt_colsum_partials_f32: null pointer");
    return colsum_run(X, R, C, ldx, nullptr, ws, ws_bytes, nchunks, stream);
}

extern "C" size_t ptt_linear_wgrad_workspace(int R, int Cout, int Cin) {
    if (R <= 0 || Cout <= 0 || Cin <= 0) return 0;
    int rows = wgrad_stream_ok(R, Cout, Cin, Cout, Cin) ? wgrad_stream_rows(R) : wgrad_chunk_rows(R, Cout, Cin);
    if (wgrad_smallk_ok(Cout, Cin) && WK_ROWS < rows) rows = WK_ROWS;
    return (size_t)((R + rows - 1) / rows) * (size_t)Cout * Cin * sizeof(float);
}

static int linear_wgrad_run(const float* dZ, int ldz, const float* X, int ldx, int R, int Cout, int Cin, float* dW,
                            int accumulate, void* ws, size_t ws_bytes, const float* x_scale, const float* x_shift,
                            int* nchunks_out, ptt_stream_t stream) {
    if (x_scale && (!x_shift || (Cin & 3) || ((reinterpret_cast<uintptr_t>(x_scale) | reinterpret_cast<uintptr_t>(x_shift)) & 15)))
        return fail(PTT_EINVAL, "ptt_linear_wgrad_f32: the input transform needs Cin %% 4 == 0 and 16-byte aligned scale / shift");
    if (R <= 0 || Cout <= 0 || Cin <= 0 || ldz < Cout || ldx < Cin)
        return fail(PTT_EINVAL, "ptt_linear_wgrad_f32: R=%d Cout=%d Cin=%d ldz=%d ldx=%d", R, Cout, Cin, ldz, ldx);
    if (!dZ || !X || (!dW && !nchunks_out)) return fail(PTT_EINVAL, "ptt_linear_wgrad_f32: null pointer");
    if (!ws || ws_bytes < ptt_linear_wgrad_workspace(R, Cout, Cin))
        return fail(PTT_EWORKSPACE, "ptt_linear_wgrad_f32: workspace too small");
    if (wgrad_smallk_ok(Cout, Cin) && !x_scale && (ldz & 3) == 0 && (reinterpret_cast<uintptr_t>(dZ) & 15) == 0) {
        const int nch = (R + WK_ROWS - 1) / WK_ROWS;
        hipStream_t s2 = as_stream(stream);
        float* part = static_cast<float*>(ws);
        if (Cin == 1) hipLaunchKernelGGL((wgrad_smallk_kernel<1>), dim3(nch), dim3(256), 0, s2, dZ, ldz, X, ldx, R, Cout, part);
        else if (Cin == 2) hipLaunchKernelGGL((wgrad_smallk_kernel<2>), dim3(nch), dim3(256), 0, s2, dZ, ldz, X, ldx, R, Cout, part);
        else if (Cin == 3) hipLaunchKernelGGL((wgrad_smallk_kernel<3>), dim3(nch), dim3(256), 0, s2, dZ, ldz, X, ldx, R, Cout, part);
        else hipLaunchKernelGGL((wgrad_smallk_kernel<4>), dim3(nch), dim3(256), 0, s2, dZ, ldz, X, ldx, R, Cout, part);
        if (dW) launch_wgrad_finish(part, nch, (size_t)Cout * Cin, accumulate, dW, s2);
        if (nchunks_out) *nchunks_out = nch;
        return check_launch("wgrad_smallk_kernel");
    }
    if (wgrad_stream_ok(R, Cout, Cin, ldz, ldx)) {
        const int rows = wgrad_stream_rows(R), nch = (R + rows - 1) / rows;
        hipStream_t s2 = as_stream(stream);
        if (int rc = launch_wgrad_stream(dZ, ldz, X, ldx, R, Cout, Cin, rows, static_cast<float*>(ws), x_scale, x_shift, s2)) return rc;
        if (dW) launch_wgrad_finish(static_cast<const float*>(ws), nch, (size_t)Cout * Cin, accumulate, dW, s2);
        if (nchunks_out) *nchunks_out = nch;
        return check_launch("wgrad_stream_kernel");
    }
    const int rows = wgrad_chunk_rows(R, Cout, Cin);
    const int nchunks = (R + rows - 1) / rows;
    const int nbo = (Cout + 127) / 128, nbi = (Cin + 127) / 128;
    hipStream_t s = as_stream(stream);
    const int lds = 4 * WG_KC * WG_LD * (int)sizeof(float);
    const bool vz = (ldz & 3) == 0 && (reinterpret_cast<uintptr_t>(dZ) & 15) == 0;
    const bool vx = (ldx & 3) == 0 && (reinterpret_cast<uintptr_t>(X) & 15) == 0;
    const int narrow_o = (Cout <= 64), narrow_i = (Cin <= 64);
    const int ns = (narrow_o ? 2 : 1) * (narrow_i ? 2 : 1);
#define PTT_WGRAD_CASE(VZ, VX)                                                                                        \
    if (vz == VZ && vx == VX) {                                                                                       \
        if (ns == 1) {                                                                                                \
            if (int rc = set_lds_limit(reinterpret_cast<const void*>(linear_wgrad_kernel<VZ, VX, 1>), lds)) return rc; \
            hipLaunchKernelGGL((linear_wgrad_kernel<VZ, VX, 1>), dim3(nbo * nbi, nchunks), dim3(256), lds, s, dZ, ldz, X, ldx, R, Cout, \
                               Cin, nbi, rows, static_cast<float*>(ws), x_scale, x_shift, 0, 0);                      \
        } else if (ns == 2) {                                                                                         \
            if (int rc = set_lds_limit(reinterpret_cast<const void*>(linear_wgrad_kernel<VZ, VX, 2>), lds)) return rc; \
            hipLaunchKernelGGL((linear_wgrad_kernel<VZ, VX, 2>), dim3(nbo * nbi, nchunks), dim3(256), lds, s, dZ, ldz, X, ldx, R, Cout, \
                               Cin, nbi, rows, static_cast<float*>(ws), x_scale, x_shift, narrow_o, narrow_i);        \
        } else {                                                                                                      \
            if (int rc = set_lds_limit(reinterpret_cast<const void*>(linear_wgrad_kernel<VZ, VX, 4>), lds)) return rc; \
// ... 246 lines not shown
```

ptt_amd/models/transformer_block/multitransformer.py:

```python
import numpy as np
import torch
import torch.nn as nn
import torch.nn.functional as F

from ... import ops, train_ops
from ...param_cache import ParamCache
from ..model_utils import get_clones, index_points, square_distance
from .variants import PER_LAYER_MAX_POINTS, SPATIAL_ORDER_MIN_POINTS, _rows2d

FUSED_HEADS = (1, 2, 4, 8)


class MulHeadTransformerLayer(nn.Module):
    def __init__(self, d_points, d_model, k, heads, drop=0.) -> None:
        super().__init__()
        self.heads = heads
        head_dim = d_model // heads
        self.fc1 = nn.Linear(d_points, d_model)
        self.fc2 = nn.Linear(d_model, d_points)
        self.fc_delta = nn.Sequential(nn.Linear(3, d_model), nn.ReLU(), nn.Linear(d_model, d_model))
        self.fc_gamma = nn.Sequential(nn.Linear(head_dim, head_dim), nn.ReLU(), nn.Linear(head_dim, head_dim))
        self.w_qs = nn.Linear(d_model, d_model, bias=False)
        self.w_ks = nn.Linear(d_model, d_model, bias=False)
        self.w_vs = nn.Linear(d_model, d_model, bias=False)
# ... 14 lines not shown
              self.fc_gamma[2].bias, self.proj.weight, self.norm1.weight, self.norm1.bias, self.norm2.weight, self.norm2.bias]
        return self._cache.get(ts, ts[0].device, self._pack)

    def _pack(self):
        f = lambda t: t.detach().float().contiguous()
        H = self.heads
        wqkv = torch.cat([self.w_qs.weight, self.w_ks.weight, self.w_vs.weight], 0).double()
        blockdiag = lambda wt: torch.block_diag(*([f(wt)] * H)).contiguous()
        return dict(
            qkv=ops.pack_weight((wqkv @ self.fc1.weight.double()).float().contiguous()),
            qkv_b=(wqkv @ self.fc1.bias.double()).float().contiguous(),
            wd1=ops.pack_delta0(self.fc_delta[0].weight, self.fc_delta[0].bias),
            wd2=ops.pack_weight(self.fc_delta[2].weight), bd2=f(self.fc_delta[2].bias),
            wg1=ops.pack_weight(self.fc_gamma[0].weight), wg2=ops.pack_weight(self.fc_gamma[2].weight),
            bg1=f(self.fc_gamma[0].bias).repeat(H).contiguous(), bg2=f(self.fc_gamma[2].bias).repeat(H).contiguous(),
            wg1_bd=ops.pack_weight(blockdiag(self.fc_gamma[0].weight)),
            wg2_bd=ops.pack_weight(blockdiag(self.fc_gamma[2].weight)),
            w1b=torch.cat((f(self.fc_delta[0].weight), f(self.fc_delta[0].bias)[:, None]), 1).contiguous(),
            proj=ops.pack_weight(self.proj.weight),
            fc2=ops.pack_weight(self.fc2.weight), fc2_b=f(self.fc2.bias),
            n1w=f(self.norm1.weight), n1b=f(self.norm1.bias), n2w=f(self.norm2.weight), n2b=f(self.norm2.bias))

    def _fused(self, xyz, features, knn_idx, rel, want_attn, order):
        P = self._params()
        D, H, k = self.d_model, self.heads, self.k
        B, N = xyz.shape[0], xyz.shape[1]
        dev = xyz.device
        if B * N <= PER_LAYER_MAX_POINTS and not want_attn:
            qkv = torch.empty((B, N, 3 * D), dtype=torch.float32, device=dev)
            pos = torch.empty((B * N * k, D), dtype=torch.float32, device=dev)
            g = torch.empty_like(pos)
            res = torch.empty((B, N, D), dtype=torch.float32, device=dev)
            knn2 = knn_idx.view(-1, k)
            ops.row_jobs([ops.row_job(P['wd2'], D, prologue=1, rel=rel.view(-1, 3), w1=P['w1b'], K=D, shift=P['bd2'], out=pos),
                          ops.row_job(P['qkv'], 3 * D, x=features, shift=P['qkv_b'], out=qkv)])
            ops.row_jobs([ops.row_job(P['wg1_bd'], D, prologue=2, qkv=qkv, knn=knn2, pos=pos, q_off=0, k_off=D, N=N, K=D,
                                      shift=P['bg1'], act=1, out=g)])
            ops.row_jobs([ops.row_job(P['wg2_bd'], D, x=g, epilogue=1, qkv=qkv, knn=knn2, pos=pos, v_off=2 * D, N=N,
                                      sm_scale=1.0 / np.sqrt(self.head_dim), out=res)])
            attn = None
        else:
            qkv = ops.linear(features, P['qkv'], 3 * D, None, P['qkv_b'])
            res, attn = ops.pt_attn_pair(xyz, knn_idx, qkv, P['wd1'], P['wd2'], P['bd2'], P['wg1'], P['bg1'], P['wg2'],
                                         P['bg2'], D, want_attn, rel=rel, order=order, heads=H)
        r = ops.linear(res, P['proj'], D)
        ops.layernorm(r, P['n1w'], P['n1b'], self.norm1.eps, out=r)
        o = ops.linear(r, P['fc2'], self.d_points, None, P['fc2_b'])
        ops.layernorm(o, P['n2w'], P['n2b'], self.norm2.eps, residual=features, out=o)
        return o, attn

    def _train_rows(self, features, knn_idx, rel, order, start, want_attn):
        H = self.heads
        x = train_ops.rows_linear(self.fc1, features)
        q, kf, vf = (train_ops.rows_linear(m, x) for m in (self.w_qs, self.w_ks, self.w_vs))
        pos_enc = train_ops.rows_mlp2(self.fc_delta, rel)
        res, attn = train_ops.attn_core(self.fc_gamma, q, kf, vf, knn_idx, pos_enc, 1.0 / np.sqrt(self.head_dim), order, start, heads=H)
        res = train_ops.rows_layernorm(self.norm1, train_ops.rows_linear(self.proj, res))
        res = train_ops.rows_layernorm(self.norm2, train_ops.rows_linear(self.fc2, res), residual=features)
        if not want_attn:
            return res, None
        B, N, k, D = attn.shape
        return res, attn.view(B, N, k, H, D // H).permute(0, 3, 1, 2, 4).flatten(0, 1)

    def forward(self, xyz, features):
        dists = square_distance(xyz, xyz)
        knn_idx = dists.argsort()[:, :, :self.k]
        knn_xyz = index_points(xyz, knn_idx)
        pre = features
        x = self.fc1(features)
        B, N, C = x.shape
        H = self.heads
        query, key, value = self.w_qs(x), index_points(self.w_ks(x), knn_idx), index_points(self.w_vs(x), knn_idx)
        query = query.view(B, N, H, -1).permute(0, 2, 1, 3).flatten(0, 1)
        pos_enc = _rows2d(self.fc_delta, xyz[:, :, None] - knn_xyz)
        pos_enc, key, value = (t.view(B, N, t.shape[2], H, -1).permute(0, 3, 1, 2, 4).flatten(0, 1)
                               for t in (pos_enc, key, value))
        attn = _rows2d(self.fc_gamma, query[:, :, None] - key + pos_enc)
        attn = F.softmax(attn / np.sqrt(key.size(-1)), dim=-2)
        res = (attn * (value + pos_enc)).sum(dim=2)
        if H > 1:
            res = res.permute(0, 2, 1).reshape(B, C, N).permute(0, 2, 1)
        res = self.norm1(self.proj_drop(self.proj(res)))
        res = self.norm2(self.fc2(res)) + pre
        return res, attn


class MulTransformerBlock(nn.Module):
    def __init__(self, d_points, d_model, k, heads, layers, **kwargs):
        super().__init__()
        transformer_layer = MulHeadTransformerLayer(d_points, d_model, k, heads)
        self.layers = get_clones(transformer_layer, layers)
        self.k = k
        self.heads = heads
        self.d_model = d_model
        self.d_points = d_points

    def _fusable(self, xyz, features):
        if self.training or not xyz.is_cuda:
            return False
        name = 'MulTransformerBlock(d_model=%d, k=%d, heads=%d)' % (self.d_model, self.k, self.heads)
        if ops.autograd_recording(self, xyz, features):
            return ops.note_unfused(name, 'autograd is recording (wrap inference in torch.no_grad())')
        if self.d_model != 512 or self.k != 16:
            return ops.note_unfused(name, 'ptt_pt_attn_pair_f32 instantiates d_model 512, k 16')
        if self.heads not in FUSED_HEADS:
            return ops.note_unfused(name, 'ptt_pt_attn_pair_f32 instantiates heads %s' % (FUSED_HEADS,))
        if xyz.shape[1] % 2 != 0 or xyz.shape[1] < self.k:
            return ops.note_unfused(name, 'needs an even number of points >= k (got %d)' % xyz.shape[1])
        if features.dtype != torch.float32 or xyz.dtype != torch.float32:
# ... 30 lines not shown
```

ptt_amd/models/transformer_block/variants.py:

```python
import numpy as np
import torch
import torch.nn as nn
import torch.nn.functional as F

from ... import ops, train_ops
from ...param_cache import ParamCache
from ..model_utils import index_points, square_distance


PER_LAYER_MAX_POINTS = ops.ONE_FRAME_MAX_POINTS


def _rows2d(layers, x):
    return layers(x.reshape(-1, x.shape[-1])).reshape(*x.shape[:-1], -1)


SPATIAL_ORDER_MIN_POINTS = 512
FUSED_D_MODEL, FUSED_KNN = (128, 256, 512), (8, 16, 32)


class TransformerBlock(nn.Module):
    def __init__(self, d_points, d_model, k, **kwargs) -> None:
        super().__init__()
        self.fc1 = nn.Linear(d_points, d_model)
# ... 41 lines not shown
            wg1=ops.pack_weight(self.fc_gamma[0].weight), bg1=f(self.fc_gamma[0].bias),
            wg2=ops.pack_weight(self.fc_gamma[2].weight), bg2=f(self.fc_gamma[2].bias),
            fc2=ops.pack_weight(self.fc2.weight), fc2_b=f(self.fc2.bias),
            wd1_lin=ops.pack_weight(self.fc_delta[0].weight), bd1=f(self.fc_delta[0].bias),
            w1b=torch.cat((f(self.fc_delta[0].weight), f(self.fc_delta[0].bias)[:, None]), 1).contiguous())

    def forward(self, xyz, features, knn=None, want_attn=True):
        if self._fusable(xyz, features):
            P = self._params()
            D = self.d_model
            xyz = xyz.contiguous()
            if knn is not None and knn[0].shape == (xyz.shape[0], xyz.shape[1], self.k):
                knn_idx, rel = knn
            else:
                knn_idx, rel = ops.knn(xyz, self.k, want_rel=True)
            per_layer = (D, self.k) == (512, 16) and xyz.shape[0] * xyz.shape[1] <= PER_LAYER_MAX_POINTS
            if per_layer and not want_attn:
                B, N = xyz.shape[0], xyz.shape[1]
                dev = xyz.device
                qkv = torch.empty((B, N, 3 * D), dtype=torch.float32, device=dev)
                pos = torch.empty((B * N * self.k, D), dtype=torch.float32, device=dev)
                g = torch.empty_like(pos)
                res = torch.empty((B, N, D), dtype=torch.float32, device=dev)
                out = torch.empty((B, N, self.d_points), dtype=torch.float32, device=dev)
                ops.row_jobs([ops.row_job(P['wd2'], D, prologue=1, rel=rel.view(-1, 3), w1=P['w1b'], K=D, shift=P['bd2'], out=pos),
                              ops.row_job(P['qkv'], 3 * D, x=features, shift=P['qkv_b'], out=qkv)])
                ops.row_jobs([ops.row_job(P['wg1'], D, prologue=2, qkv=qkv, knn=knn_idx.view(-1, self.k), pos=pos, q_off=0, k_off=D,
                                          N=N, K=D, shift=P['bg1'], act=1, out=g)])
                ops.row_jobs([ops.row_job(P['wg2'], D, x=g, epilogue=1, qkv=qkv, knn=knn_idx.view(-1, self.k), pos=pos, v_off=2 * D,
                                          N=N, sm_scale=1.0 / np.sqrt(D), out=res)])
                ops.row_jobs([ops.row_job(P['fc2'], self.d_points, x=res, shift=P['fc2_b'], res=features, out=out)])
                return out, None
            qkv = ops.linear(features, P['qkv'], 3 * D, None, P['qkv_b'])
            if per_layer:
                pairs = rel.view(-1, 3)
                h = ops.linear(pairs, P['wd1_lin'], D, None, P['bd1'], relu=True)
                pos = ops.linear(h, P['wd2'], D, None, P['bd2']).view(xyz.shape[0], xyz.shape[1], self.k, D)
                t = ops.pt_pair_input_qkv(qkv, knn_idx, pos, D)
                g = ops.linear(t.view(-1, D), P['wg1'], D, None, P['bg1'], relu=True)
                a = ops.linear(g, P['wg2'], D, None, P['bg2']).view_as(t)
                res, attn = ops.pt_attn_fwd_qkv(a, qkv, knn_idx, pos, D, 1.0 / np.sqrt(D), want_attn)
            else:
                order = ops.spatial_order(xyz) if SPATIAL_ORDER_MIN_POINTS <= xyz.shape[1] <= 8192 else None
                res, attn = ops.pt_attn_pair(xyz, knn_idx, qkv, P['wd1'], P['wd2'], P['bd2'], P['wg1'],
                                             P['bg1'], P['wg2'], P['bg2'], D, want_attn, rel=rel, order=order)
            res = ops.linear(res, P['fc2'], self.d_points, None, P['fc2_b'], False, features)
            return res, attn

        if train_ops.pt_block_usable(self, xyz, features):
            knn_idx, rel = ops.knn(xyz.contiguous(), self.k, want_rel=True)
            if xyz.requires_grad:
                rel = train_ops._KnnRel.apply(xyz, knn_idx, rel)
            x = train_ops.rows_linear(self.fc1, features)
            q, kf, vf = (train_ops.rows_linear(m, x) for m in (self.w_qs, self.w_ks, self.w_vs))
            pos_enc = train_ops.rows_mlp2(self.fc_delta, rel)
            order, start = ops.scatter_csr(knn_idx.view(knn_idx.shape[0], -1), knn_idx.shape[1])
            if train_ops.ATTN_CORE:
                res, attn = train_ops.attn_core(self.fc_gamma, q, kf, vf, knn_idx, pos_enc, 1.0 / np.sqrt(self.d_model), order, start)
            else:
                t = train_ops._PairInput.apply(q, kf, knn_idx, pos_enc, order, start)
                a = train_ops.rows_mlp2(self.fc_gamma, t)
                res, attn = train_ops._AttnAggregate.apply(a, vf, knn_idx, pos_enc, 1.0 / np.sqrt(self.d_model), order, start)
            res = train_ops.rows_linear(self.fc2, res, residual=features)
            return res, attn

        dists = square_distance(xyz, xyz)
        knn_idx = dists.argsort()[:, :, :self.k]
        knn_xyz = index_points(xyz, knn_idx)
        pre = features
        x = self.fc1(features)
        q, k, v = self.w_qs(x), index_points(self.w_ks(x), knn_idx), index_points(self.w_vs(x), knn_idx)
        pos_enc = _rows2d(self.fc_delta, xyz[:, :, None] - knn_xyz)
        attn = _rows2d(self.fc_gamma, q[:, :, None] - k + pos_enc)
        attn = F.softmax(attn / np.sqrt(k.size(-1)), dim=-2)
        res = (attn * (v + pos_enc)).sum(dim=2)
        res = self.fc2(res) + pre
        return res, attn


class TransformerBlockSTD(nn.Module):

    def __init__(self, d_points, d_model, k, **kwargs) -> None:
        super().__init__()
        self.fc1 = nn.Linear(d_points, d_model)
        self.fc2 = nn.Linear(d_model, d_points)
        self.fc_delta = nn.Sequential(nn.Linear(3, d_model), nn.ReLU(), nn.Linear(d_model, d_model))
        self.w_qs = nn.Linear(d_model, d_model, bias=False)
        self.w_ks = nn.Linear(d_model, d_model, bias=False)
        self.w_vs = nn.Linear(d_model, d_model, bias=False)
        self.k = k
        self.d_model = d_model
        self.d_points = d_points
        self._cache = ParamCache()

    def _fusable(self, xyz, features):
        if self.training or not xyz.is_cuda:
            return False
        name = 'TransformerBlockSTD(d_model=%d)' % self.d_model
        if ops.autograd_recording(self, xyz, features):
            return ops.note_unfused(name, 'autograd is recording (wrap inference in torch.no_grad())')
        if features.dtype != torch.float32 or xyz.dtype != torch.float32:
            return ops.note_unfused(name, 'inputs must be float32')
        return True

    def _params(self):
        ts = [self.fc1.weight, self.fc1.bias, self.fc2.weight, self.fc2.bias, self.w_qs.weight, self.w_ks.weight,
              self.w_vs.weight, self.fc_delta[0].weight, self.fc_delta[0].bias, self.fc_delta[2].weight, self.fc_delta[2].bias]
        return self._cache.get(ts, ts[0].device, self._pack)

    def _pack(self):
        f = lambda t: t.detach().float().contiguous()
        wqkv = torch.cat([self.w_qs.weight, self.w_ks.weight, self.w_vs.weight], 0).double()
# ... 28 lines not shown
```

ptt_amd/ops.py:

```python
import contextlib
import ctypes
import os

import torch

from . import _lib
from ._lib import AttnDesc, SaDesc, SaLayer, XcorrDesc


def _stream():
    return ctypes.c_void_p(torch.cuda.current_stream().cuda_stream)


_timing = None


def start_kernel_timing(names):
    global _timing
    _timing = {n: [] for n in names}


def stop_kernel_timing():
    global _timing
    t, _timing = _timing, None
# ... 893 lines not shown
    _rows(dpooled, "dpooled"); _rows(z, "z")
    R, C = z.shape
    sums = torch.empty((2, C), dtype=torch.float64, device=z.device)
    ws, ws_arg = _workspace("ptt_bn_stats_workspace", z.device, R, C)
    _launch("ptt_bn_bwd_pooled_sums_f64", z.device, _ptr(dpooled), dpooled.stride(0), _ptr(arg), int(ns), _ptr(z), z.stride(0), _ptr(mean),
            _ptr(invstd), R, C, _ptr(sums), *ws_arg, _ptr(act_scale), _ptr(act_shift))
    return sums


def bn_bwd_pooled_apply(dpooled, arg, ns, z, mean, invstd, gamma, sum_dy, sum_dy_xhat, count, act_scale, act_shift, out=None):
    _rows(dpooled, "dpooled"); _rows(z, "z")
    R, C = z.shape
    if out is None:
        out = torch.empty((R, C), dtype=torch.float32, device=z.device)
    _launch("ptt_bn_bwd_pooled_apply_f32", z.device, _ptr(dpooled), dpooled.stride(0), _ptr(arg), int(ns), _ptr(z), z.stride(0), _ptr(mean),
            _ptr(invstd), _ptr(gamma), _ptr(sum_dy), _ptr(sum_dy_xhat), _ptr(count), R, C, _ptr(out), out.stride(0), _ptr(act_scale), _ptr(act_shift))
    return out


def pool_rows(x, ns, act_scale=None, act_shift=None):
    _rows(x, "x")
    R, C = x.shape
    G = R // int(ns)
    out = torch.empty((G, C), dtype=torch.float32, device=x.device)
    arg = torch.empty((G, C), dtype=torch.int32, device=x.device)
    _launch("ptt_pool_rows_f32", x.device, _ptr(x), x.stride(0), G, int(ns), C, _ptr(out), C, _ptr(arg), _ptr(act_scale), _ptr(act_shift))
    return out, arg


def pool_rows_bwd(dout, arg, ns):
    _rows(dout, "dout")
    G, C = dout.shape
    dx = torch.empty((G * int(ns), C), dtype=torch.float32, device=dout.device)
    _launch("ptt_pool_rows_bwd_f32", dout.device, _ptr(dout), dout.stride(0), _ptr(arg), G, int(ns), C, _ptr(dx), C)
    return dx


def linear_act_in(x, in_scale, in_shift, wpacked, cout):
    _rows(x, "x")
    rows, K = x.shape
    out = torch.empty((rows, int(cout)), dtype=torch.float32, device=x.device)
    _launch("ptt_linear_act_in_f32", x.device, _ptr(x), rows, K, x.stride(0), _ptr(in_scale), _ptr(in_shift), _ptr(wpacked), int(cout), _ptr(out),
            int(cout), timed='ptt_linear_f32')
    return out


def rows_gemm_supported(rows, K, N, ldx=None, ldo=None, x=None):
    if x is not None and x.data_ptr() % 16:
        return False
    return bool(_host("ptt_rows_gemm_supported", int(rows), int(K), int(N), int(ldx if ldx is not None else K),
                                                   int(ldo if ldo is not None else N)))


def rows_gemm(x, wpacked, cout, in_scale=None, in_shift=None, bias=None, relu=False, residual=None, want_stats=False, out=None):
    _rows(x, "x")
    rows, K = x.shape
    cout = int(cout)
    if out is None:
        out = torch.empty((rows, cout), dtype=torch.float32, device=x.device)
    stats = None
    if want_stats:
        chunks = _host("ptt_rows_gemm_stat_chunks", rows, K, cout)
        stats = torch.empty((max(1, chunks), 2, cout), dtype=torch.float64, device=x.device)
    r2 = None
    if residual is not None:
        r2 = _rows(residual, "residual")
    _launch("ptt_rows_gemm_f32", x.device, _ptr(x), rows, K, x.stride(0), _ptr(in_scale), _ptr(in_shift), _ptr(wpacked), cout, _ptr(bias),
            1 if relu else 0, _ptr(r2), r2.stride(0) if r2 is not None else cout, _ptr(out), out.stride(0), _ptr(stats),
            stats.numel() if stats is not None else 0, timed='ptt_rows_gemm_f32')
    return (out, stats) if want_stats else out


def rows_gemm_pool_supported(rows, K, N, ldx, ns, x=None):
    if x is not None and x.data_ptr() % 16:
        return False
    return bool(_host("ptt_rows_gemm_pool_supported", int(rows), int(K), int(N), int(ldx), int(ns)))


def rows_gemm_pool(x, wpacked, cout, in_scale, in_shift, ns):
    _rows(x, "x")
    rows, K = x.shape
    cout, ns = int(cout), int(ns)
    G = rows // ns
    out = torch.empty((rows, cout), dtype=torch.float32, device=x.device)
    chunks = _host("ptt_rows_gemm_stat_chunks", rows, K, cout)
    stats = torch.empty((max(1, chunks), 2, cout), dtype=torch.float64, device=x.device)
    pmax = torch.empty((G, cout), dtype=torch.float32, device=x.device)
    pmin = torch.empty((G, cout), dtype=torch.float32, device=x.device)
    amax = torch.empty((G, cout), dtype=torch.int32, device=x.device)
    amin = torch.empty((G, cout), dtype=torch.int32, device=x.device)
    _launch("ptt_rows_gemm_pool_f32", x.device, _ptr(x), rows, K, x.stride(0), _ptr(in_scale), _ptr(in_shift), _ptr(wpacked), cout, _ptr(out), cout,
            _ptr(stats), stats.numel(), ns, _ptr(pmax), _ptr(pmin), _ptr(amax), _ptr(amin), timed='ptt_rows_gemm_f32')
    return out, stats, (pmax, pmin, amax, amin)


def pool_select(extrema, act_scale, act_shift):
    pmax, pmin, amax, amin = extrema
    G, C = pmax.shape
    out = torch.empty((G, C), dtype=torch.float32, device=pmax.device)
    arg = torch.empty((G, C), dtype=torch.int32, device=pmax.device)
    _launch("ptt_pool_select_f32", pmax.device, _ptr(pmax), _ptr(pmin), _ptr(amax), _ptr(amin), _ptr(act_scale), _ptr(act_shift), G, C, _ptr(out),
            _ptr(arg))
    return out, arg


def rows_gemm_masked(x, wpacked, cout, mask, want_colsum=False):
# ... 97 lines not shown
        _bn_tail_done(bn)
        return mean, var, invstd, a, b
    _launch("ptt_bn_finish_partials_f32", partials.device, _ptr(partials), chunks, C, int(rows), float(eps), _ptr(mean), _ptr(var), _ptr(invstd))
    return mean, var, invstd


def bn_sums_partials(partials, rows):
    chunks, _, C = partials.shape
    sums = torch.empty((2 * C + 1,), dtype=torch.float64, device=partials.device)
    _launch("ptt_bn_sums_partials_f64", partials.device, _ptr(partials), chunks, C, int(rows), _ptr(sums))
    return sums


def colsum(x, out=None):
    _rows(x, "x")
    R, C = x.shape
    if R == 0:
        return x.sum(0) if out is None else out.zero_()
    if out is None:
        out = torch.empty((C,), dtype=torch.float32, device=x.device)
    ws, ws_arg = _workspace("ptt_colsum_workspace", x.device, R, C)
    _launch("ptt_colsum_f32", x.device, _ptr(x), R, C, x.stride(0), _ptr(out), *ws_arg)
    return out


def linear_wgrad(dz, x, out=None, accumulate=False, x_scale=None, x_shift=None):
    _rows(dz, "dz"); _rows(x, "x")
    R, Cout = dz.shape
    Cin = x.shape[1]
    if out is None:
        out = torch.empty((Cout, Cin), dtype=torch.float32, device=dz.device)
    ok2 = (dz.stride(0) % 4 == 0 and x.stride(0) % 4 == 0 and dz.data_ptr() % 16 == 0 and x.data_ptr() % 16 == 0
           and R * max(dz.stride(0), x.stride(0)) < (1 << 29))
    nb2 = _host("ptt_linear_wgrad2_workspace", R, Cout, Cin) if ok2 else 0
    two = bool(nb2 and WGRAD2)
    ws = _ws(nb2 if two else _host("ptt_linear_wgrad_workspace", R, Cout, Cin), dz.device)
    _launch("ptt_linear_wgrad2_f32" if two else "ptt_linear_wgrad_f32", dz.device, _ptr(dz), dz.stride(0), _ptr(x), x.stride(0), R, Cout, Cin,
            _ptr(out), int(bool(accumulate)), _ptr(ws), ws.numel() * 8, _ptr(x_scale), _ptr(x_shift), timed='ptt_linear_wgrad_f32')
    return out


def linear_wgrad_partials(dz, x, x_scale=None, x_shift=None):
    _rows(dz, "dz"); _rows(x, "x")
    R, Cout = dz.shape
    Cin = x.shape[1]
    ok2 = (dz.stride(0) % 4 == 0 and x.stride(0) % 4 == 0 and dz.data_ptr() % 16 == 0 and x.data_ptr() % 16 == 0
           and R * max(dz.stride(0), x.stride(0)) < (1 << 29))
    nb2 = _host("ptt_linear_wgrad2_workspace", R, Cout, Cin) if ok2 else 0
    nch = ctypes.c_int(0)
    two = bool(nb2 and WGRAD2)
    ws = _ws(nb2 if two else _host("ptt_linear_wgrad_workspace", R, Cout, Cin), dz.device)
    _launch("ptt_linear_wgrad2_partials_f32" if two else "ptt_linear_wgrad_partials_f32", dz.device, _ptr(dz), dz.stride(0), _ptr(x), x.stride(0),
            R, Cout, Cin, _ptr(ws), ws.numel() * 8, _ptr(x_scale), _ptr(x_shift), ctypes.byref(nch), timed='ptt_linear_wgrad_f32')
    return ws, nch.value


def colsum_partials(x):
    _rows(x, "x")
    R, C = x.shape
    ws, ws_arg = _workspace("ptt_colsum_workspace", x.device, R, C)
    nch = ctypes.c_int(0)
    _launch("ptt_colsum_partials_f32", x.device, _ptr(x), R, C, x.stride(0), *ws_arg, ctypes.byref(nch))
    return ws, nch.value


_capture_uploads = []


def finish_capture_uploads():
    done = []
    while _capture_uploads:
        table, host, keep = _capture_uploads.pop(0)
        table.copy_(host)
        done.append((table, keep))
    return done


class GradFinishPlan(object):

    def __init__(self, device):
        self.device = torch.device(device)
        self.signature = None
        self.capture_table = None
        self.uploaded = torch.cuda.Event()

    def prepare_capture(self):
        if self.signature is None:
            raise RuntimeError("GradFinishPlan: a step must have run eagerly before it is captured")
        self.capture_table = (torch.empty_like(self.table), torch.zeros(tuple(self.host.shape), dtype=torch.uint8))

    @staticmethod
    def _outputs_per_group(total_chunks):
        return 4 if total_chunks > 1024 else 8 if total_chunks > 256 else 16 if total_chunks > 64 else 32 if total_chunks > 8 else 64 if total_chunks > 2 else 256

    def _build(self, sig):
        by_dst, order = {}, []
        for k, (dst, cols, ld, n, nch) in enumerate(sig):
            key = (dst, cols, ld, n)
            if key not in by_dst:
                by_dst[key] = []
                order.append(key)
            by_dst[key].append(k)
        nseg = len(order)
        segs = (_lib.GradSegment * nseg)()
        blocks, self.job_order = [], []
        for si, key in enumerate(order):
# ... 18 lines not shown
        self.blocks = torch.tensor(blocks, dtype=torch.int32, device=self.device)
        nj = len(self.job_order)
        self.host = torch.zeros((nj, ctypes.sizeof(_lib.GradJob)), dtype=torch.uint8).pin_memory()
        self.rows = (_lib.GradJob * nj).from_address(self.host.data_ptr())
        self.table = torch.empty_like(self.host, device=self.device)
        self.signature = sig

    def run(self, jobs, flat):
        if not jobs:
            return
        if flat.dtype != torch.float32 or not flat.is_contiguous() or flat.device != self.device or flat.data_ptr() % 16:
            raise ValueError("GradFinishPlan: a contiguous, 16-byte aligned float32 gradient buffer on %s expected" % self.device)
        total = flat.numel()
        sig = tuple((int(d), int(c), int(l), int(n), int(nch)) for d, c, l, n, _, nch in jobs)
        if sig != self.signature:
            for d, c, l, n, nch in sig:
                if n <= 0 or c <= 0 or n % c or l < c or nch <= 0 or d < 0 or d + (n // c - 1) * l + c > total:
                    raise ValueError("GradFinishPlan: job (dst %d, cols %d, ld %d, n %d, chunks %d) outside the %d-element buffer" % (d, c, l, n, nch, total))
            self._build(sig)
        capturing = torch.cuda.is_current_stream_capturing()
        if capturing:
            if sig != self.signature:
                raise RuntimeError("GradFinishPlan: a step must have run eagerly before it is captured (the segment tables are built then)")
            if self.capture_table is None:
                raise RuntimeError("GradFinishPlan: prepare_capture() must be called before the stream starts capturing")
            table, host = self.capture_table
            self.capture_table = None
            rows = (_lib.GradJob * len(self.job_order)).from_address(host.data_ptr())
            _capture_uploads.append((table, host, (self.segs, self.blocks)))
        else:
            self.uploaded.synchronize()
            rows, table = self.rows, self.table
        for r, k, vec in zip(rows, self.job_order, self.vec_jobs):
            ptr = int(jobs[k][4])
            if vec and ptr % 16:
                raise ValueError("GradFinishPlan: partial sums of a float4 segment must be 16-byte aligned")
            r.partial, r.nchunks = ptr, sig[k][4]
        if not capturing:
            self.table.copy_(self.host, non_blocking=True)
            self.uploaded.record()
        _launch("ptt_grad_finish_f32", self.device, _ptr(self.segs), _ptr(table), _ptr(self.blocks), self.n_blocks, _ptr(flat))


def pack_weight_strided(src, cout, k, stride_out, stride_k, batch, stride_batch):
    if not src.is_cuda or src.dtype != torch.float32:
        raise RuntimeError("src must be a float32 device tensor")
    n = _host("ptt_packed_weight_elems", int(cout), int(k))
    out = torch.empty((int(batch), n), dtype=torch.float32, device=src.device)
    _launch("ptt_pack_weight_strided_f32", src.device, _ptr(src), int(cout), int(k), int(stride_out), int(stride_k), int(batch), int(stride_batch),
            _ptr(out))
    return out


def pack_jobs_table(jobs, device):
    arr = (_lib.PackJob * len(jobs))()
    for n, (ptr, off, so, sk, cout, k) in enumerate(jobs):
        arr[n] = _lib.PackJob(W=ptr, out_offset=off, stride_out=so, stride_k=sk, Cout=cout, K=k)
    host = torch.frombuffer(bytearray(bytes(arr)), dtype=torch.uint8)
    return host.to(device)


def pack_weights(table, n_jobs, arena):
    if not arena.is_cuda or arena.dtype != torch.float32 or not arena.is_contiguous():
        raise RuntimeError("arena must be a contiguous float32 device tensor")
    _launch("ptt_pack_weights_f32", arena.device, _ptr(table), int(n_jobs), _ptr(arena))
    return arena


def linear_batched(x, wpacked, cout, residual=None):
    if not x.is_cuda or x.dtype != torch.float32 or x.dim() != 3 or x.stride(2) != 1:
        raise RuntimeError("x must be a (batch, rows, K) float32 device tensor with contiguous channels")
    Bt, rows, K = x.shape
    out = torch.empty((Bt, rows, int(cout)), dtype=torch.float32, device=x.device)
    r = residual
    if r is not None and (r.dim() != 3 or r.stride(2) != 1):
        raise RuntimeError("residual must be (batch, rows, cout) with contiguous channels")
    _launch("ptt_linear_batched_f32", x.device, _ptr(x), rows, K, x.stride(1), x.stride(0), _ptr(wpacked), wpacked.stride(0), int(cout), None, None,
            0, _ptr(r), r.stride(1) if r is not None else int(cout), r.stride(0) if r is not None else 0, _ptr(out), int(cout), rows * int(cout), Bt,
            timed='ptt_linear_f32')
    return out


def softmax_rows_(x, scale):
    _chk(x, "x", torch.float32)
    n = x.shape[-1]
    _launch("ptt_softmax_rows_f32", x.device, _ptr(x), x.numel() // n, n, n, float(scale))
    return x


def gather_rows(src, idx):
    _chk(src, "src", torch.float32, 3)
    _chk(idx, "idx", torch.int32, 2)
    B, N, C = src.shape
    E = idx.shape[1]
    out = torch.empty((B, E, C), dtype=torch.float32, device=src.device)
    _launch("ptt_gather_rows_f32", src.device, _ptr(src), _ptr(idx), B, N, E, C, _ptr(out))
    return out


def sa_z0_rows(xyz, new_xyz, idx, term, wx, radius, normalize_xyz, want_stats=False):
    _chk(xyz, "xyz", torch.float32, 3)
    _chk(new_xyz, "new_xyz", torch.float32, 3)
    _chk(idx, "idx", torch.int32, 3)
    if not (wx.is_cuda and wx.dtype == torch.float32 and wx.dim() == 2 and wx.stride(1) == 1):
        raise RuntimeError("wx must be a float32 (C,3) device tensor with unit column stride (a column slice of the weight is fine)")
    B, N, _ = xyz.shape
    _, M, ns = idx.shape
    C = wx.shape[0]
    if term is not None:
        _chk(term, "term", torch.float32, 3)
        if tuple(term.shape) != (B, N, C):
            raise RuntimeError("term must be (B,N,C) = %s, got %s" % ((B, N, C), tuple(term.shape)))
    if wx.shape[1] != 3 or new_xyz.shape[1] != M:
        raise RuntimeError("wx must be (C,3) and new_xyz (B,M,3)")
    z0 = torch.empty((B * M * ns, C), dtype=torch.float32, device=xyz.device)
    rel = torch.empty((B * M * ns, 3), dtype=torch.float32, device=xyz.device)
    chunks = _host("ptt_sa_z0_rows_stat_chunks", B, M, ns, C) if want_stats else 0
    if chunks:
        part = torch.empty((chunks, 2, C), dtype=torch.float64, device=xyz.device)
        _launch("ptt_sa_z0_rows_stats_f32", xyz.device, _ptr(xyz), _ptr(new_xyz), _ptr(idx), _ptr(term), _ptr(wx), wx.stride(0), B, N, M, ns, C,
                float(radius), int(bool(normalize_xyz)), _ptr(z0), _ptr(rel), _ptr(part), part.numel())
        return z0, rel, part
    _launch("ptt_sa_z0_rows_f32", xyz.device, _ptr(xyz), _ptr(new_xyz), _ptr(idx), _ptr(term), _ptr(wx), wx.stride(0), B, N, M, ns, C, float(radius),
            int(bool(normalize_xyz)), _ptr(z0), _ptr(rel))
    return (z0, rel, None) if want_stats else (z0, rel)


def sa_z0_bnbwd(part, g, z0, rel, mean, invstd, gamma, act_scale, act_shift, want_dz, dwx_partials=False):
    _rows(g, "g"); _rows(z0, "z0")
    R, C = z0.shape
    dev = g.device
    d_wx = torch.empty((C, 3), dtype=torch.float32, device=dev) if not dwx_partials else None
    dgamma, dbeta = (torch.empty((C,), dtype=torch.float32, device=dev) for _ in range(2))
    ws, ws_arg = _workspace("ptt_sa_z0_bnbwd_workspace", dev, R, C)
    _launch("ptt_sa_z0_bnbwd_f32", dev, _ptr(part), part.shape[0], _ptr(g), _ptr(z0), _ptr(rel), _ptr(mean), _ptr(invstd), _ptr(gamma),
            _ptr(act_scale), _ptr(act_shift), R, C, _ptr(g) if want_dz else None, _ptr(d_wx), _ptr(dgamma), _ptr(dbeta), *ws_arg)
    if dwx_partials:
        d_wx = (ws, _host("ptt_sa_z0_bnbwd_workspace", R, C) // (12 * C))
    return (g if want_dz else None), d_wx, dgamma, dbeta


def scatter_csr(idx, N):
    _chk(idx, "idx", torch.int32, 2)
    B, E = idx.shape
    order = torch.empty((B, E), dtype=torch.int32, device=idx.device)
    start = torch.empty((B, int(N) + 1), dtype=torch.int32, device=idx.device)
    _launch("ptt_scatter_csr_i32", idx.device, _ptr(idx), B, int(N), E, _ptr(order), _ptr(start))
    return order, start


def scatter_rows_det(g, idx, N, csr=None, minuend=None, negate=False):
    _chk(g, "g", torch.float32, 3)
    _chk(idx, "idx", torch.int32, 2)
    B, E, C = g.shape
    order, start = csr if csr is not None else scatter_csr(idx, N)
    out = torch.empty((B, int(N), C), dtype=torch.float32, device=g.device)
    if minuend is None and not negate:
        _launch("ptt_scatter_rows_csr_f32", g.device, _ptr(g), _ptr(order), _ptr(start), B, int(N), E, C, _ptr(out))
    else:
        if minuend is not None:
            _chk(minuend, "minuend", torch.float32, 3)
            if tuple(minuend.shape) != (B, int(N), C):
                raise ValueError("minuend: (B,N,C) expected")
        _launch("ptt_scatter_rows_csr_sub_f32", g.device, _ptr(g), _ptr(order), _ptr(start), B, int(N), E, C, _ptr(minuend), _ptr(out))
    return out


def rows_gemm_rsum16_supported(x, K, N):
    return bool(x.dim() == 2 and x.stride(1) == 1 and x.data_ptr() % 16 == 0
                and _host("ptt_rows_gemm_rsum16_supported", x.shape[0], int(K), int(N), x.stride(0)))


def rows_gemm_rsum16(x, wpacked, N, residual):
    _rows(x, "x"); _rows(residual, "residual")
    rows, K = x.shape
    if tuple(residual.shape) != (rows, int(N)):
        raise ValueError("rows_gemm_rsum16: residual (rows, N) expected")
    out, plain = (torch.empty((rows, int(N)), dtype=torch.float32, device=x.device) for _ in range(2))
    gsum = torch.empty((rows // 16, int(N)), dtype=torch.float32, device=x.device)
    _launch("ptt_rows_gemm_rsum16_f32", x.device, _ptr(x), rows, K, x.stride(0), _ptr(wpacked), int(N), _ptr(residual), residual.stride(0), _ptr(out),
            int(N), _ptr(plain), int(N), _ptr(gsum), int(N), timed='ptt_linear_f32')
    return plain, out, gsum


def rows_gemm_rsum16_heads_supported(x, D, hd):
    return bool(x.dim() == 2 and x.stride(1) == 1 and x.data_ptr() % 16 == 0 and x.shape[1] == int(D)
                and _host("ptt_rows_gemm_rsum16_heads_supported", x.shape[0], int(D), int(hd), x.stride(0)))


def rows_gemm_rsum16_heads(x, wpacked, hd, residual):
    _rows(x, "x"); _rows(residual, "residual")
    rows, D = x.shape
    hd = int(hd)
    if tuple(residual.shape) != (rows, D):
        raise ValueError("rows_gemm_rsum16_heads: residual (rows, D) expected")
    if hd <= 0 or D % hd or wpacked.numel() < hd * hd:
        raise ValueError("rows_gemm_rsum16_heads: D %% hd == 0 and a packed hd x hd weight expected (D=%d hd=%d)" % (D, hd))
    out, plain = (torch.empty((rows, D), dtype=torch.float32, device=x.device) for _ in range(2))
    gsum = torch.empty((rows // 16, D), dtype=torch.float32, device=x.device)
    _launch("ptt_rows_gemm_rsum16_heads_f32", x.device, _ptr(x), rows, D, hd, x.stride(0), _ptr(wpacked), _ptr(residual), residual.stride(0),
            _ptr(out), D, _ptr(plain), D, _ptr(gsum), D, timed='ptt_linear_f32')
    return plain, out, gsum


def layernorm_train_fwd(x, weight, bias, eps, residual=None):
    _rows(x, "x")
    rows, C = x.shape
    for t, name in ((weight, "weight"), (bias, "bias")):
        if t is None or not t.is_cuda or t.dtype != torch.float32 or not t.is_contiguous() or t.numel() != C:
            raise RuntimeError("%s must be a contiguous float32 (%d,) device tensor" % (name, C))
    if residual is not None:
        _rows(residual, "residual")
        if tuple(residual.shape) != (rows, C):
            raise ValueError("layernorm_train_fwd: residual (rows, C) expected")
    y = torch.empty((rows, C), dtype=torch.float32, device=x.device)
    mean, rstd = (torch.empty((rows,), dtype=torch.float32, device=x.device) for _ in range(2))
    _launch("ptt_layernorm_train_fwd_f32", x.device, _ptr(x), rows, C, x.stride(0) if rows > 1 else C, _ptr(weight), _ptr(bias), float(eps),
            _ptr(residual), (residual.stride(0) if (residual is not None and rows > 1) else C), _ptr(y), C, _ptr(mean), _ptr(rstd),
            timed='ptt_layernorm_train_fwd_f32')
    return y, mean, rstd


def layernorm_bwd(dy, x, mean, rstd, weight):
    _rows(dy, "dy"); _rows(x, "x")
    rows, C = x.shape
    if tuple(dy.shape) != (rows, C):
        raise ValueError("layernorm_bwd: dy (rows, C) expected")
    for t, name, n in ((mean, "mean", rows), (rstd, "rstd", rows), (weight, "weight", C)):
        if t is None or not t.is_cuda or t.dtype != torch.float32 or not t.is_contiguous() or t.numel() != n:
            raise RuntimeError("%s must be a contiguous float32 (%d,) device tensor" % (name, n))
    dx = torch.empty((rows, C), dtype=torch.float32, device=x.device)
    dw, db = (torch.empty((C,), dtype=torch.float32, device=x.device) for _ in range(2))
    if rows == 0:
        return dx, dw.zero_(), db.zero_()
    ws, ws_arg = _workspace("ptt_layernorm_bwd_workspace", x.device, rows, C)
    _launch("ptt_layernorm_bwd_f32", x.device, _ptr(dy), dy.stride(0) if rows > 1 else C, _ptr(x), x.stride(0) if rows > 1 else C, _ptr(mean),
            _ptr(rstd), _ptr(weight), rows, C, _ptr(dx), C, _ptr(dw), _ptr(db), *ws_arg, timed='ptt_layernorm_bwd_f32')
    return dx, dw, db


def pt_pair_input(q, kf, knn, pos):
    B, N, D = q.shape
    k = knn.shape[2]
    t = torch.empty((B, N, k, D), dtype=torch.float32, device=q.device)
    _launch("ptt_pt_pair_input_f32", q.device, _ptr(q), _ptr(kf), _ptr(knn), _ptr(pos), B, N, k, D, _ptr(t))
    return t


def pt_pair_input_qkv(qkv, knn, pos, D):
    B, N, _ = qkv.shape
    k = knn.shape[2]
    t = torch.empty((B, N, k, D), dtype=torch.float32, device=qkv.device)
    _launch("ptt_pt_pair_input_ld_f32", qkv.device, qkv.data_ptr(), 3 * D, qkv.data_ptr() + 4 * D, 3 * D, _ptr(knn), _ptr(pos), B, N, k, D, _ptr(t))
    return t


def pt_attn_fwd_qkv(a, qkv, knn, pos, D, scale, want_attn=False):
    B, N, k, _ = a.shape
    res = torch.empty((B, N, D), dtype=torch.float32, device=a.device)
    attn = torch.empty_like(a) if want_attn else None
    _launch("ptt_pt_attn_fwd_ld_f32", a.device, _ptr(a), qkv.data_ptr() + 8 * D, 3 * D, _ptr(knn), _ptr(pos), B, N, k, D, float(scale), _ptr(attn),
            _ptr(res))
    return res, attn


def pt_attn_train_fwd(a, vf, knn, pos, scale):
    B, N, k, D = a.shape
    attn = torch.empty_like(a)
    res = torch.empty((B, N, D), dtype=torch.float32, device=a.device)
    _launch("ptt_pt_attn_train_fwd_f32", a.device, _ptr(a), _ptr(vf), _ptr(knn), _ptr(pos), B, N, k, D, float(scale), _ptr(attn), _ptr(res))
    return attn, res


def pt_attn_train_bwd(attn, vf, knn, pos, dres, scale):
    B, N, k, D = attn.shape
    da, dvp = torch.empty_like(attn), torch.empty_like(attn)
    _launch("ptt_pt_attn_train_bwd_f32", attn.device, _ptr(attn), _ptr(vf), _ptr(knn), _ptr(pos), _ptr(dres), B, N, k, D, float(scale), _ptr(da),
            _ptr(dvp))
    return da, dvp


def _rows2(t, name):
    if t is None:
        return None
    if not t.is_cuda or t.dtype != torch.float32:
        raise RuntimeError("%s must be a float32 device tensor" % name)
    t2 = t.reshape(-1, t.shape[-1])
    if t2.shape[1] > 1 and t2.stride(1) != 1:
        raise RuntimeError("%s must have unit column stride" % name)
    return t2


def _ld(t2):
    return int(t2.stride(0)) if t2.shape[0] > 1 else max(int(t2.shape[1]), int(t2.stride(0)))


def row_job(wpacked, cout, x=None, x2=None, xmax=None, scale=None, shift=None, act=0, res=None, res2=None, res_split=0, out=None,
            out2=None, out_split=0, out_col0=0, raw=None, rel=None, w1=None, qkv=None, knn=None, pos=None, q_off=0,
            k_off=0, v_off=0, N=0, sm_scale=1.0, prologue=0, epilogue=0, K=None, col_tiles=0, idx=None, xyz=None, centres=None,
            wx=None, radius=1.0, ns=0, M=0, normalize_xyz=False, pro_relu=False):
    j = _lib.RowJob()
    keep = [wpacked, scale, shift]
    j.Wpacked, j.scale, j.shift = wpacked.data_ptr(), (scale.data_ptr() if scale is not None else None), \
        (shift.data_ptr() if shift is not None else None)
    j.Cout, j.act, j.prologue, j.epilogue, j.col_tiles = int(cout), int(act), int(prologue), int(epilogue), int(col_tiles)
    if prologue == 0:
        x_ = _rows2(x, "x")
        j.X, j.ldx, j.K1, j.rows = x_.data_ptr(), _ld(x_), x_.shape[1], x_.shape[0]
        j.K = j.K1
        if x2 is not None:
            y_ = _rows2(x2, "x2")
            if y_.shape[0] != x_.shape[0]:
                raise RuntimeError("x and x2 must have the same number of rows")
            j.X2, j.ldx2, j.K = y_.data_ptr(), _ld(y_), j.K1 + y_.shape[1]
            keep.append(y_)
        if xmax is not None:
            m_ = _rows2(xmax, "xmax")
            if m_.shape != x_.shape or _ld(m_) != _ld(x_):
                raise RuntimeError("xmax must have x's shape and row stride")
            j.Xmax = m_.data_ptr()
            keep.append(m_)
        keep.append(x_)
    elif prologue == 1:
        r_ = _rows2(rel, "rel")
        if r_.shape[1] != 3 or not r_.is_contiguous() or w1.shape != (int(K), 4) or not w1.is_contiguous():
            raise RuntimeError("prologue 1: rel (rows,3) and w1 (K,4) contiguous")
        j.rel, j.w1, j.rows, j.K, j.K1 = r_.data_ptr(), w1.data_ptr(), r_.shape[0], int(K), int(K)
        keep += [r_, w1]
    elif prologue == 2:
# ... 241 lines not shown
```

ptt_amd/train_ops.py:

```python
import os
import weakref
from collections import namedtuple

import torch
import torch.distributed as dist
import torch.nn as nn

from . import ops


def _raw_pointer_ready(conv, bn, device):
    ts = [conv.weight] + ([conv.bias] if conv.bias is not None else [])
    if bn is not None:
        ts += [bn.weight, bn.bias, bn.running_mean, bn.running_var]
        nbt = bn.num_batches_tracked
        if nbt is not None and (nbt.dtype != torch.int64 or nbt.device != device):
            return False
    return all(t is not None and t.dtype == torch.float32 and t.device == device and t.is_contiguous() for t in ts)


def _pointwise_conv(conv, conv_cls, one):
    return (isinstance(conv, conv_cls) and conv.kernel_size == one and conv.stride == one and conv.padding == (0,) * len(one)
            and conv.groups == 1)


def _conv_bn_relu_unit(unit, conv_cls, bn_cls, one, device):
    conv = getattr(unit, 'conv', None)
    bn = getattr(getattr(unit, 'normlayer', None), 'bn', None)
    if not _pointwise_conv(conv, conv_cls, one) or conv.bias is not None or conv.weight.shape[0] % 4:
        return False
    if not isinstance(bn, (bn_cls, nn.SyncBatchNorm)) or not bn.affine or not bn.track_running_stats or bn.momentum is None:
        return False
    if not bn.training:
        return False
    if not isinstance(getattr(unit, 'activation', None), nn.ReLU) or list(unit._modules.keys()) != ['conv', 'normlayer', 'activation']:
        return False
    return _raw_pointer_ready(conv, bn, device)


def usable(mlp, x):
    if not (mlp.training and x.is_cuda and x.dtype == torch.float32 and len(mlp) > 0):
        return False
    return all(_conv_bn_relu_unit(unit, nn.Conv2d, nn.BatchNorm2d, (1, 1), x.device) and unit.conv.dilation == (1, 1) for unit in mlp)


_pack_cache = {}


def _pack_slot(base):
    e = _pack_cache.get(id(base))
    if e is not None and e[0]() is base:
        return e[1]
    slot = {}
    try:
        ref = weakref.ref(base, lambda _r, k=id(base): _pack_cache.pop(k, None))
    except TypeError:
        return slot
    _pack_cache[id(base)] = (ref, slot)
    return slot


class _PackPlan:

    def __init__(self):
        self.entries = {}
        self.table = None

    def register(self, ekey, base, elems):
        if ekey not in self.entries:
            self.entries[ekey] = [weakref.ref(base), int(elems)]
            self.table = None

    def _build(self, device):
        jobs, keys, ptrs, off = [], [], [], 0
        for ekey, (ref, elems) in list(self.entries.items()):
            base = ref()
            if base is None or id(base) != ekey[0] or not base.is_cuda or base.device != device:
                del self.entries[ekey]
                continue
            _, boff, shape, stride, transposed = ekey
            so, sk = (stride[1], stride[0]) if transposed else (stride[0], stride[1])
            cout, k = (shape[1], shape[0]) if transposed else (shape[0], shape[1])
            jobs.append((base.data_ptr() + boff, off, so, sk, cout, k))
            keys.append(ekey)
            ptrs.append(base.data_ptr())
            off += elems
        self.table = (ops.pack_jobs_table(jobs, device), keys, ptrs, off) if jobs else None

    def repack(self, device):
        if self.table is not None:
            for ekey, ptr in zip(self.table[1], self.table[2]):
                base = self.entries[ekey][0]()
                if base is None or base.data_ptr() != ptr:
                    self.table = None
                    break
        if self.table is None:
            self._build(device)
            if self.table is None:
                return False
        table, keys, _, total = self.table
        arena = ops.pack_weights(table, len(keys), torch.empty((total,), dtype=torch.float32, device=device))
        off = 0
        for ekey in keys:
            ref, elems = self.entries[ekey]
            base = ref()
            slot = _pack_slot(base)
            version = (base._version, base.data_ptr())
            for k in [k for k in slot if k[3] != version]:
                del slot[k]
            slot[(ekey[1], ekey[2], ekey[3], version, ekey[4])] = arena[off:off + elems]
            off += elems
        return True


FUSED_BN_BWD = os.environ.get("PTT_FUSED_BN_BWD", "1") != "0"
_pack_plans = {}
PACK_PLAN = True


_pack_capture = None


class PackCapture(object):

    def __init__(self, params, device):
        ids = set(id(p) for p in params)
        self.device = torch.device(device)
        self.plan = _PackPlan()
        shared = _pack_plans.get(self.device)
        for ekey, (ref, elems) in (list(shared.entries.items()) if shared is not None else []):
            if ekey[0] in ids and ref() is not None:
                self.plan.entries[ekey] = [ref, elems]
        self.plan._build(self.device)
        self.cache, self.arena = {}, None

    def __enter__(self):
        global _pack_capture
        if _pack_capture is not None:
            raise RuntimeError("PackCapture: another capture is active")
        _pack_capture = self
        return self

    def __exit__(self, *exc):
        global _pack_capture
        _pack_capture = None

    def get(self, W, transpose):
        base = W._base if W._base is not None else W
        ekey = (id(base), W.data_ptr() - base.data_ptr(), tuple(W.shape), tuple(W.stride()), bool(transpose))
        hit = self.cache.get(ekey)
        if hit is not None:
            return hit
        if self.arena is None and self.plan.table is not None:
            table, keys, _, total = self.plan.table
            self.arena = ops.pack_weights(table, len(keys), torch.empty((total,), dtype=torch.float32, device=self.device))
            off = 0
            for k in keys:
                elems = self.plan.entries[k][1]
                self.cache[k] = self.arena[off:off + elems]
                off += elems
            hit = self.cache.get(ekey)
            if hit is not None:
                return hit
        w = W.detach()
        cout, k = (w.shape[1], w.shape[0]) if transpose else w.shape
        so, sk = (w.stride(1), w.stride(0)) if transpose else (w.stride(0), w.stride(1))
        hit = self.cache[ekey] = ops.pack_weight_strided(w, cout, k, so, sk, 1, 0)[0]
        return hit


def packed(W, transpose=False):
    if _pack_capture is not None:
        return _pack_capture.get(W, transpose)
    base = W._base if W._base is not None else W
    slot = _pack_slot(base)
    off = (W.data_ptr() - base.data_ptr())
    key = (off, tuple(W.shape), tuple(W.stride()), (W._version, base.data_ptr()), bool(transpose))
    hit = slot.get(key)
    if hit is not None:
        return hit
    ekey = (id(base), off, key[1], key[2], key[4])
    plan = _pack_plans.setdefault(W.device, _PackPlan()) if PACK_PLAN and W.dim() == 2 else None
    if plan is not None and ekey in plan.entries and plan.repack(W.device):
        hit = slot.get(key)
        if hit is not None:
            return hit
    for k in [k for k in slot if k[3] != key[3]]:
        del slot[k]
    w = W.detach()
    cout, k = (w.shape[1], w.shape[0]) if transpose else w.shape
    so, sk = (w.stride(1), w.stride(0)) if transpose else (w.stride(0), w.stride(1))
    hit = slot[key] = ops.pack_weight_strided(w, cout, k, so, sk, 1, 0)[0]
    if plan is not None:
        plan.register(ekey, base, hit.numel())
    return hit


def invalidate_packed():
    _pack_cache.clear()
    _pack_plans.clear()


def conv_rows(x, W2d, in_a=None, in_b=None, want_stats=False, transpose=False):
    cout, K = (W2d.shape[1], W2d.shape[0]) if transpose else W2d.shape
    wp = packed(W2d, transpose)
    if ops.rows_gemm_supported(x.shape[0], K, cout, x.stride(0), cout, x=x):
        if want_stats:
            return ops.rows_gemm(x, wp, cout, in_scale=in_a, in_shift=in_b, want_stats=True)
        return ops.rows_gemm(x, wp, cout, in_scale=in_a, in_shift=in_b), None
    z = ops.linear_act_in(x, in_a, in_b, wp, cout) if in_a is not None else ops.linear(x, wp, cout)
    return z, None


_row_counts = {}


def _row_count(rows, device):
    key = (int(rows), str(device))
    if key not in _row_counts:
        _row_counts[key] = torch.full((1,), float(rows), dtype=torch.float64, device=device)
# ... 32 lines not shown
                if GradSink.active is not None:
                    raise RuntimeError("GradSink: another backward pass is being collected")
                if any(p.grad is not v for p, v in zip(sink.params, sink.views)):
                    sink.attach()
                sink.flat.zero_()
                sink.jobs, sink.keep = [], []
                GradSink.active = sink

            def __exit__(self, *exc):
                GradSink.active = None
                if exc[0] is not None:
                    sink.jobs, sink.keep = [], []
        return _Scope()

    def locate(self, w):
        if w is None:
            return None
        base = w._base if w._base is not None else w
        hit = self.index.get(base.data_ptr())
        if hit is None or hit[1] != base.numel():
            return None
        rel = (w.data_ptr() - base.data_ptr()) // 4
        n = w.numel()
        if n == 0 or rel < 0 or w.dtype != torch.float32:
            return None
        if w.is_contiguous():
            return (hit[0] + rel, n, n, n) if rel + n <= hit[1] else None
        if w.dim() == 2 and w.stride(1) == 1 and w.stride(0) >= w.shape[1] and rel + (w.shape[0] - 1) * w.stride(0) + w.shape[1] <= hit[1]:
            return (hit[0] + rel, w.shape[1], w.stride(0), n)
        return None

    def push(self, loc, partials, nchunks):
        self.jobs.append((loc[0], loc[1], loc[2], loc[3], partials.data_ptr(), int(nchunks)))
        self.keep.append(partials)

    def flush(self):
        self.plan.run(self.jobs, self.flat)
        self.jobs, self.keep = [], []


def _sunk(w):
    sink = GradSink.active
    loc = sink.locate(w) if sink is not None else None
    return (sink, loc) if loc is not None else (None, None)


def weight_grad(w, dz, x, x_scale=None, x_shift=None):
    sink, loc = _sunk(w)
    if sink is None:
        return ops.linear_wgrad(dz, x, x_scale=x_scale, x_shift=x_shift)
    ws, nch = ops.linear_wgrad_partials(dz, x, x_scale, x_shift)
    sink.push(loc, ws, nch)
    return None


def bias_grad(b, g2):
    sink, loc = _sunk(b)
    if sink is None:
        return ops.colsum(g2)
    ws, nch = ops.colsum_partials(g2)
    sink.push(loc, ws, nch)
    return None


def small_grad(p, g):
    if g is None:
        return None
    sink, loc = _sunk(p)
    if sink is None or g.numel() != loc[3] or g.dtype != torch.float32:
        return g
    g = g.contiguous()
    if g.data_ptr() % 16:
        g = g.clone()
    sink.push(loc, g, 1)
    return None


class _GatherRows(torch.autograd.Function):

    @staticmethod
    def forward(ctx, rows, idx):
        ctx.save_for_backward(idx)
        ctx.N = rows.shape[1]
        return ops.gather_rows(rows.contiguous(), idx)

    @staticmethod
    def backward(ctx, g):
        (idx,) = ctx.saved_tensors
        return ops.scatter_rows_det(g.contiguous(), idx, ctx.N), None


def gather_rows(rows, idx):
    return _GatherRows.apply(rows, idx)


class _AddRelTerm(torch.autograd.Function):

    @staticmethod
    def forward(ctx, gathered, rel, wx):
        ctx.save_for_backward(rel, wx)
        ctx.wx = wx
        return ops.linear(rel.contiguous(), packed(wx), wx.shape[0], residual=gathered.contiguous())

    @staticmethod
    def backward(ctx, g):
        rel, wx = ctx.saved_tensors
# ... 374 lines not shown

ATTN_CORE = os.environ.get("PTT_ATTN_CORE", "1") != "0"


class _AttnCore(torch.autograd.Function):

    @staticmethod
    def forward(ctx, q, kf, vf, knn, pos, W1, b1, W2, b2, scale, order, start, heads=1):
        ctx.set_materialize_grads(False)
        q, kf, vf, pos = q.contiguous(), kf.contiguous(), vf.contiguous(), pos.contiguous()
        t = ops.pt_pair_input(q, kf, knn, pos)
        x2 = t.view(-1, t.shape[-1] // heads)
        h, a = _mlp2_forward(x2, W1, b1, W2, b2)
        a = a.view(*t.shape[:-1], W2.shape[0] * heads)
        attn, res = ops.pt_attn_train_fwd(a, vf, knn, pos, scale)
        ctx.save_for_backward(x2, h, attn, vf, knn, pos, order, start, W1, W2)
        ctx.Ws, ctx.bs, ctx.scale, ctx.heads = (W1, W2), (b1, b2), float(scale), int(heads)
        ctx.mark_non_differentiable(attn)
        return res, attn

    @staticmethod
    def backward(ctx, dres, _dattn):
        x2, h, attn, vf, knn, pos, order, start = ctx.saved_tensors[:8]
        W1, W2 = ctx.Ws
        B, N, k, D = attn.shape
        csr = (order, start)
        dres = dres.contiguous()
        da, dvp = ops.pt_attn_train_bwd(attn, vf, knn, pos, dres, ctx.scale)
        dvf = ops.scatter_rows_det(dvp.view(B, N * k, D), knn.view(B, N * k), N, csr)
        heads = ctx.heads
        dz1, dW1, db1, dW2, db2 = _mlp2_backward(da.view(-1, D // heads), x2, h, W1, ctx.bs[0], W2, ctx.bs[1])
        D1, Din = W1.shape
        if heads == 1 and ops.rows_gemm_rsum16_supported(dz1, D1, Din) and k == 16 and Din == D:
            dt, dpos, dq = ops.rows_gemm_rsum16(dz1, packed(W1, True), Din, dvp.view(-1, D))
            dkf = ops.scatter_rows_det(dt.view(B, N * k, D), knn.view(B, N * k), N, csr, negate=True)
            dq, dpos = dq.view(B, N, D), dpos.view(B, N, k, D)
        elif heads > 1 and k == 16 and Din * heads == D and ops.rows_gemm_rsum16_heads_supported(dz1.view(-1, D), D, Din):
            dt, dpos, dq = ops.rows_gemm_rsum16_heads(dz1.view(-1, D), packed(W1, True), Din, dvp.view(-1, D))
            dkf = ops.scatter_rows_det(dt.view(B, N * k, D), knn.view(B, N * k), N, csr, negate=True)
            dq, dpos = dq.view(B, N, D), dpos.view(B, N, k, D)
        else:
            dt = lin_rows(dz1, W1, transpose=True).view(B, N, k, D)
            dq = dt.sum(dim=2)
            dkf = ops.scatter_rows_det(dt.view(B, N * k, D), knn.view(B, N * k), N, csr).neg_()
            dpos = dt + dvp
        return dq, dkf, dvf, None, dpos, dW1, db1, dW2, db2, None, None, None, None


def attn_core(fc_gamma, q, kf, vf, knn, pos, scale, order, start, heads=1):
    return _AttnCore.apply(q, kf, vf, knn, pos, fc_gamma[0].weight, fc_gamma[0].bias, fc_gamma[2].weight, fc_gamma[2].bias, scale, order, start,
                           int(heads))


def pt_block_usable(block, xyz, features):
    return (block.training and xyz.is_cuda and features.dtype == torch.float32 and block.k in (8, 16, 32) and block.d_model % 4 == 0
            and xyz.shape[1] * block.k <= 16384)


MUL_BLOCK_HEADS = (1, 2, 4, 8)


def mul_block_usable(block, xyz, features):
    return bool(block.training and xyz.is_cuda and features.is_cuda and features.dtype == torch.float32 and xyz.dtype == torch.float32
                and block.k == 16 and block.d_model == 512 and block.heads in MUL_BLOCK_HEADS and xyz.shape[1] >= block.k
                and xyz.shape[1] * block.k <= 16384 and all(layer.proj_drop.p == 0 for layer in block.layers))


class _RowsLayerNorm(torch.autograd.Function):

    @staticmethod
    def forward(ctx, x, w, b, eps, residual):
        x2 = x.reshape(-1, x.shape[-1]).contiguous()
        r2 = residual.reshape(-1, x.shape[-1]).contiguous() if residual is not None else None
        wd = w.detach()
        y, mean, rstd = ops.layernorm_train_fwd(x2, wd, b.detach(), eps, r2)
        ctx.save_for_backward(x2, mean, rstd, w)
        ctx.w, ctx.b, ctx.shape = w, b, x.shape
        return y.view(x.shape)

    @staticmethod
    def backward(ctx, dy):
        x2, mean, rstd, _ = ctx.saved_tensors
        dy2 = dy.reshape(-1, dy.shape[-1]).contiguous()
        dx, dw, db = ops.layernorm_bwd(dy2, x2, mean, rstd, ctx.w.detach())
        return (dx.view(ctx.shape) if ctx.needs_input_grad[0] else None, small_grad(ctx.w, dw) if ctx.needs_input_grad[1] else None,
                small_grad(ctx.b, db) if ctx.needs_input_grad[2] else None, None, (dy if ctx.needs_input_grad[4] else None))


def rows_layernorm(norm, x, residual=None):
    return _RowsLayerNorm.apply(x, norm.weight, norm.bias, float(norm.eps), residual)


def lin_rows(x2, W, b=None, relu=False, residual=None, transpose=False):
    cout, K = (W.shape[1], W.shape[0]) if transpose else W.shape
    wp = packed(W, transpose)
    if ops.rows_gemm_supported(x2.shape[0], K, cout, x2.stride(0), cout, x=x2):
        return ops.rows_gemm(x2, wp, cout, bias=b, relu=relu, residual=residual)
    return ops.linear(x2, wp, cout, None, b, relu, residual)


def _mlp2_forward(x2, W1, b1, W2, b2):
    h = lin_rows(x2, W1, b1.detach(), relu=True)
    return h, lin_rows(h, W2, b2.detach())


def _mlp2_backward(dy2, x2, h, W1, b1, W2, b2):
# ... 196 lines not shown
```

Before: 17380.

## Stack Q/K/V projections into one GEMM with fused attention core and stacked wgrad

New measurement: 17400, median of 4. About the same (+0.1%).

```diff
diff --git a/include/ptt_hip.h b/include/ptt_hip.h
--- a/include/ptt_hip.h
+++ b/include/ptt_hip.h
@@ -8,7 +8,7 @@
 extern "C" {
 #endif
 
-#define PTT_ABI_VERSION 31
+#define PTT_ABI_VERSION 32
 
 enum {
     PTT_OK = 0,
@@ -326,6 +326,8 @@
                              int k, int D, float* t, ptt_stream_t stream);
 int ptt_pt_attn_fwd_ld_f32(const float* a, const float* vf, int ldv, const int32_t* knn, const float* pos, int B, int N, int k, int D,
                            float scale, float* attn, float* res, ptt_stream_t stream);
+int ptt_pt_attn_train_bwd_ld_f32(const float* attn, const float* vf, int ldv, const int32_t* knn, const float* pos, const float* dres,
+                                 int B, int N, int k, int D, float scale, float* da, float* dvp, ptt_stream_t stream);
 
 int ptt_gather_rows_f32(const float* src, const int32_t* idx, int B, int N, int E, int C, float* out, ptt_stream_t stream);
 int ptt_scatter_csr_i32(const int32_t* idx, int B, int N, int E, int32_t* order, int32_t* start, ptt_stream_t stream);
@@ -358,6 +360,7 @@
 
 int ptt_rows_gemm_supported(int rows, int K, int N, int ldx, int ldo);
 int ptt_rows_gemm_stat_chunks(int rows, int K, int N);
+int ptt_rows_gemm_rounds(int rows, int K, int N);
 int ptt_rows_gemm_f32(const float* X, int rows, int K, int ldx, const float* in_scale, const float* in_shift,
                       const float* Wpacked, int N, const float* bias, int relu, const float* residual, int ldr,
                       float* out, int ldo, double* stats, size_t stats_elems, ptt_stream_t stream);
@@ -435,8 +438,15 @@
     const float* W;
     int64_t out_offset, stride_out, stride_k;
     int32_t Cout, K;
+    int32_t NT_stack, tile0;
 } ptt_pack_job;
 int ptt_pack_weights_f32(const ptt_pack_job* jobs_device, int n_jobs, float* arena, ptt_stream_t stream);
+size_t ptt_linear_wgrad2_stack_workspace(int R, int Cout_part, int parts, int Cin);
+int ptt_linear_wgrad2_stack_partials_f32(const float* dZ, int ldz, const float* X, int ldx, int R, int Cout_part, int parts, int Cin,
+                                         void* workspace, size_t workspace_bytes, int* nchunks, ptt_stream_t stream);
+size_t ptt_linear_wgrad_stack_workspace(int R, int Cout_part, int parts, int Cin);
+int ptt_linear_wgrad_stack_partials_f32(const float* dZ, int ldz, const float* X, int ldx, int R, int Cout_part, int parts, int Cin,
+                                        void* workspace, size_t workspace_bytes, int* nchunks, ptt_stream_t stream);
 size_t ptt_linear_wgrad2_workspace(int R, int Cout, int Cin);
 int ptt_linear_wgrad2_f32(const float* dZ, int ldz, const float* X, int ldx, int R, int Cout, int Cin, float* dW,
                           int accumulate, void* workspace, size_t workspace_bytes, const float* x_scale, const float* x_shift,
@@ -509,6 +519,8 @@
                              float* out, int ldo, float* plain, int ldp, float* gsum, int ldg, ptt_stream_t stream);
 int ptt_scatter_rows_csr_sub_f32(const float* g, const int32_t* order, const int32_t* start, int B, int N, int E, int C,
                                  const float* minuend, float* out, ptt_stream_t stream);
+int ptt_scatter_rows_csr_ld_f32(const float* g, const int32_t* order, const int32_t* start, int B, int N, int E, int C,
+                                const float* minuend, int negate, float* out, int ldo, ptt_stream_t stream);
 
 int ptt_layernorm_train_fwd_f32(const float* x, int rows, int C, int ldx, const float* weight, const float* bias, float eps,
                                 const float* residual, int ldr, float* out, int ldo, float* mean, float* rstd, ptt_stream_t stream);
diff --git a/ptt_amd/_lib.py b/ptt_amd/_lib.py
--- a/ptt_amd/_lib.py
+++ b/ptt_amd/_lib.py
@@ -113,7 +113,7 @@
 
 class PackJob(Structure):
     _fields_ = [("W", c_void_p), ("out_offset", c_int64), ("stride_out", c_int64), ("stride_k", c_int64),
-                ("Cout", c_int32), ("K", c_int32)]
+                ("Cout", c_int32), ("K", c_int32), ("NT_stack", c_int32), ("tile0", c_int32)]
 
 
 class RowJob(Structure):
diff --git a/ptt_amd/csrc/gemm_ops.hip b/ptt_amd/csrc/gemm_ops.hip
--- a/ptt_amd/csrc/gemm_ops.hip
+++ b/ptt_amd/csrc/gemm_ops.hip
@@ -576,6 +576,11 @@
     return 1;
 }
 
+extern "C" int ptt_rows_gemm_rounds(int rows, int K, int N) {
+    const RowsGemmGeom g = rows_gemm_geom(rows, K, N);
+    return g.ok ? (g.ntiles + g.G - 1) / g.G : 0;
+}
+
 extern "C" int ptt_rows_gemm_stat_chunks(int rows, int K, int N) {
     const RowsGemmGeom g = rows_gemm_geom(rows, K, N);
     return g.ok ? g.chunks : 0;
@@ -879,11 +884,17 @@
     const Wgrad2Geom g = wgrad2_geom(R, Cout, Cin);
     return g.ok ? (size_t)g.nchunks * Cout * Cin * sizeof(float) : 0;
 }
+extern "C" size_t ptt_linear_wgrad2_stack_workspace(int R, int Cout_part, int parts, int Cin) {
+    if (parts < 1 || parts > 64) return 0;
+    const Wgrad2Geom g = wgrad2_geom(R, Cout_part, Cin);
+    return g.ok ? (size_t)g.nchunks * parts * Cout_part * Cin * sizeof(float) : 0;
+}
 
 static int linear_wgrad2_run(const float* dZ, int ldz, const float* X, int ldx, int R, int Cout, int Cin, float* dW,
                              int accumulate, void* ws, size_t ws_bytes, const float* x_scale, const float* x_shift,
-                             int* nchunks_out, ptt_stream_t stream) {
-    const Wgrad2Geom g = wgrad2_geom(R, Cout, Cin);
+                             int* nchunks_out, ptt_stream_t stream, int parts = 1) {
+    Wgrad2Geom g = wgrad2_geom(R, Cout / parts, Cin);
+    g.nbo = g.ok ? Cout / g.BN : 0;
     if (!g.ok || (ldz & 3) || (ldx & 3) || ((reinterpret_cast<uintptr_t>(dZ) | reinterpret_cast<uintptr_t>(X)) & 15) ||
         (long long)R * ldz >= (1LL << 29) || (long long)R * ldx >= (1LL << 29))
         return fail(PTT_EUNSUPPORTED, "ptt_linear_wgrad2_f32: R=%d Cout=%d Cin=%d ldz=%d ldx=%d (needs R >= 2048, Cout %% 128 == 0, "
@@ -891,7 +902,7 @@
     if (ldz < Cout || ldx < Cin || !dZ || !X || (!dW && !nchunks_out)) return fail(PTT_EINVAL, "ptt_linear_wgrad2_f32: bad argument");
     if (x_scale && (!x_shift || ((reinterpret_cast<uintptr_t>(x_scale) | reinterpret_cast<uintptr_t>(x_shift)) & 15)))
         return fail(PTT_EINVAL, "ptt_linear_wgrad2_f32: the input transform needs 16-byte aligned scale / shift");
-    if (!ws || ws_bytes < ptt_linear_wgrad2_workspace(R, Cout, Cin)) return fail(PTT_EWORKSPACE, "ptt_linear_wgrad2_f32: workspace too small");
+    if (!ws || ws_bytes < (size_t)g.nchunks * Cout * Cin * sizeof(float)) return fail(PTT_EWORKSPACE, "ptt_linear_wgrad2_f32: workspace too small");
     hipStream_t s = as_stream(stream);
     const int lds = 2 * 32 * (g.BN + 4 + g.BK + 4) * (int)sizeof(float);
     const dim3 grid(g.nbo * g.nbk * g.nchunks);
@@ -936,3 +947,9 @@
     if (!nchunks) return fail(PTT_EINVAL, "ptt_linear_wgrad2_partials_f32: null pointer");
     return linear_wgrad2_run(dZ, ldz, X, ldx, R, Cout, Cin, nullptr, 0, ws, ws_bytes, x_scale, x_shift, nchunks, stream);
 }
+extern "C" int ptt_linear_wgrad2_stack_partials_f32(const float* dZ, int ldz, const float* X, int ldx, int R, int Cout_part, int parts,
+                                                    int Cin, void* ws, size_t ws_bytes, int* nchunks, ptt_stream_t stream) {
+    if (!nchunks || parts < 1 || parts > 64 || Cout_part <= 0)
+        return fail(PTT_EINVAL, "ptt_linear_wgrad2_stack_partials_f32: parts=%d Cout_part=%d", parts, Cout_part);
+    return linear_wgrad2_run(dZ, ldz, X, ldx, R, Cout_part * parts, Cin, nullptr, 0, ws, ws_bytes, nullptr, nullptr, nchunks, stream, parts);
+}
diff --git a/ptt_amd/csrc/mfma_ops.hip b/ptt_amd/csrc/mfma_ops.hip
--- a/ptt_amd/csrc/mfma_ops.hip
+++ b/ptt_amd/csrc/mfma_ops.hip
@@ -69,6 +69,8 @@
     const int NT = (jb.Cout + 31) / 32;
     const size_t total = (size_t)NT * (size_t)((jb.K + 7) / 8) * 256;
     float* Pb = arena + jb.out_offset;
+    const size_t NTs = jb.NT_stack > 0 ? (size_t)jb.NT_stack : (size_t)NT;
+    const size_t t0 = jb.NT_stack > 0 ? (size_t)jb.tile0 : 0;
     for (size_t e = (size_t)blockIdx.x * blockDim.x + threadIdx.x; e < total; e += (size_t)gridDim.x * blockDim.x) {
         const int j = (int)(e & 3);
         const int lane = (int)((e >> 2) & 63);
@@ -77,7 +79,8 @@
         const int kb = (int)(tile / NT);
         const int col = ct * 32 + (lane & 31);
         const int k = kb * 8 + 4 * (lane >> 5) + j;
-        Pb[e] = (col < jb.Cout && k < jb.K) ? jb.W[(long long)col * jb.stride_out + (long long)k * jb.stride_k] : 0.0f;
+        Pb[(((size_t)kb * NTs + t0 + ct) << 8) + (e & 255)] =
+            (col < jb.Cout && k < jb.K) ? jb.W[(long long)col * jb.stride_out + (long long)k * jb.stride_k] : 0.0f;
     }
 }
 
diff --git a/ptt_amd/csrc/train_ops.hip b/ptt_amd/csrc/train_ops.hip
--- a/ptt_amd/csrc/train_ops.hip
+++ b/ptt_amd/csrc/train_ops.hip
@@ -1030,7 +1030,8 @@
 
 __global__ __launch_bounds__(256) void scatter_rows_det_kernel(const float* __restrict__ g, const int32_t* __restrict__ order,
                                                                const int32_t* __restrict__ start, int N, int E, int C,
-                                                               float* __restrict__ out, const float* __restrict__ minuend, int negate) {
+                                                               float* __restrict__ out, const float* __restrict__ minuend, int negate,
+                                                               int ldo) {
     const int Cq = C >> 2, span = Cq < 256 ? Cq : 256, RG = 256 / span;
     const int q0 = threadIdx.x % span, rg = threadIdx.x / span;
     if (rg >= RG) return;
@@ -1062,7 +1063,7 @@
 #pragma unroll
                 for (int x = 0; x < 4; ++x) acc[x] = m[x] - acc[x];
             }
-            *reinterpret_cast<f32x4t*>(out + ((size_t)b * N + n) * C + 4 * q) = acc;
+            *reinterpret_cast<f32x4t*>(out + ((size_t)b * N + n) * ldo + 4 * q) = acc;
         }
     }
 }
@@ -1216,7 +1217,7 @@
 __global__ __launch_bounds__(256) void attn_bwd_kernel(const float* __restrict__ attn, const float* __restrict__ vf,
                                                        const int32_t* __restrict__ knn, const float* __restrict__ pos,
                                                        const float* __restrict__ dres, int N, int D, long long total_pts, float scale,
-                                                       float* __restrict__ da, float* __restrict__ dvp) {
+                                                       float* __restrict__ da, float* __restrict__ dvp, int ldv) {
     const int Dq = D >> 2;
     for (long long e = (long long)blockIdx.x * 256 + threadIdx.x; e < total_pts * Dq; e += (long long)gridDim.x * 256) {
         const long long pt = e / Dq;
@@ -1229,7 +1230,7 @@
         for (int j = 0; j < KN; ++j) {
             const int n = knn[pt * KN + j];
             w[j] = *reinterpret_cast<const f32x4t*>(attn + (pt * KN + j) * D + c);
-            const f32x4t vv = *reinterpret_cast<const f32x4t*>(vf + (b * N + n) * D + c);
+            const f32x4t vv = *reinterpret_cast<const f32x4t*>(vf + (b * N + n) * ldv + c);
             const f32x4t pv = *reinterpret_cast<const f32x4t*>(pos + (pt * KN + j) * D + c);
             f32x4t o;
 #pragma unroll
@@ -1704,24 +1705,29 @@
 }
 
 static int scatter_rows_run(const float* g, const int32_t* order, const int32_t* start, int B, int N, int E, int C, float* out,
-                            const float* minuend, int negate, ptt_stream_t stream) {
+                            const float* minuend, int negate, ptt_stream_t stream, int ldo) {
     if (B < 0 || N <= 0 || E < 0 || C <= 0 || (C & 3)) return fail(PTT_EINVAL, "ptt_scatter_rows_csr_f32: B=%d N=%d E=%d C=%d", B, N, E, C);
+    if (ldo < C || (ldo & 3)) return fail(PTT_EINVAL, "ptt_scatter_rows_csr_ld_f32: ldo=%d (C=%d)", ldo, C);
     if (B == 0) return PTT_OK;
     if (!g || !order || !start || !out || ((reinterpret_cast<uintptr_t>(g) | reinterpret_cast<uintptr_t>(out) | reinterpret_cast<uintptr_t>(minuend)) & 15))
         return fail(PTT_EINVAL, "ptt_scatter_rows_csr_f32: null or unaligned pointer");
     const int Cq = C >> 2, RG = 256 / (Cq < 256 ? Cq : 256);
     int gx = (N + RG - 1) / RG;
     if (gx > 4096) gx = 4096;
-    hipLaunchKernelGGL(scatter_rows_det_kernel, dim3(gx, B), dim3(256), 0, as_stream(stream), g, order, start, N, E, C, out, minuend, negate);
+    hipLaunchKernelGGL(scatter_rows_det_kernel, dim3(gx, B), dim3(256), 0, as_stream(stream), g, order, start, N, E, C, out, minuend, negate, ldo);
     return check_launch("scatter_rows_det_kernel");
 }
 extern "C" int ptt_scatter_rows_csr_f32(const float* g, const int32_t* order, const int32_t* start, int B, int N, int E, int C,
                                         float* out, ptt_stream_t stream) {
-    return scatter_rows_run(g, order, start, B, N, E, C, out, nullptr, 0, stream);
+    return scatter_rows_run(g, order, start, B, N, E, C, out, nullptr, 0, stream, C);
 }
 extern "C" int ptt_scatter_rows_csr_sub_f32(const float* g, const int32_t* order, const int32_t* start, int B, int N, int E, int C,
                                             const float* minuend, float* out, ptt_stream_t stream) {
-    return scatter_rows_run(g, order, start, B, N, E, C, out, minuend, 1, stream);
+    return scatter_rows_run(g, order, start, B, N, E, C, out, minuend, 1, stream, C);
+}
+extern "C" int ptt_scatter_rows_csr_ld_f32(const float* g, const int32_t* order, const int32_t* start, int B, int N, int E, int C,
+                                           const float* minuend, int negate, float* out, int ldo, ptt_stream_t stream) {
+    return scatter_rows_run(g, order, start, B, N, E, C, out, negate ? minuend : nullptr, negate ? 1 : 0, stream, ldo);
 }
 
 static int pt_train_check(const char* what, int B, int N, int k, int D, const void* p0, const void* p1, const void* p2, const void* p3) {
@@ -1792,7 +1798,20 @@
     if (!dres || !da || !dvp) return fail(PTT_EINVAL, "ptt_pt_attn_train_bwd_f32: null pointer");
     const long long pts = (long long)B * N;
     PTT_PAIR_EW(attn_bwd_kernel, attn, vf, knn, pos,
-                       dres, N, D, pts, scale, da, dvp);
+                       dres, N, D, pts, scale, da, dvp, D);
+    return check_launch("attn_bwd_kernel");
+}
+
+extern "C" int ptt_pt_attn_train_bwd_ld_f32(const float* attn, const float* vf, int ldv, const int32_t* knn, const float* pos,
+                                            const float* dres, int B, int N, int k, int D, float scale, float* da, float* dvp,
+                                            ptt_stream_t stream) {
+    if (int rc = pt_train_check("ptt_pt_attn_train_bwd_ld_f32", B, N, k, D, attn, vf, knn, pos)) return rc;
+    if (ldv < D || (ldv & 3)) return fail(PTT_EINVAL, "ptt_pt_attn_train_bwd_ld_f32: ldv=%d", ldv);
+    if (B == 0) return PTT_OK;
+    if (!dres || !da || !dvp) return fail(PTT_EINVAL, "ptt_pt_attn_train_bwd_ld_f32: null pointer");
+    const long long pts = (long long)B * N;
+    PTT_PAIR_EW(attn_bwd_kernel, attn, vf, knn, pos,
+                       dres, N, D, pts, scale, da, dvp, ldv);
     return check_launch("attn_bwd_kernel");
 }
 
@@ -1840,6 +1859,40 @@
     int rows = wgrad_stream_ok(R, Cout, Cin, Cout, Cin) ? wgrad_stream_rows(R) : wgrad_chunk_rows(R, Cout, Cin);
     if (wgrad_smallk_ok(Cout, Cin) && WK_ROWS < rows) rows = WK_ROWS;
     return (size_t)((R + rows - 1) / rows) * (size_t)Cout * Cin * sizeof(float);
+}
+
+static bool wgrad_stack_ok(int R, int Cout_part, int parts, int Cin) {
+    return R > 0 && parts >= 1 && parts <= 64 && Cout_part > 0 && Cin > 0 && Cout_part % 128 == 0 && Cin % 128 == 0;
+}
+extern "C" size_t ptt_linear_wgrad_stack_workspace(int R, int Cout_part, int parts, int Cin) {
+    if (!wgrad_stack_ok(R, Cout_part, parts, Cin)) return 0;
+    const int rows = wgrad_chunk_rows(R, Cout_part, Cin);
+    return (size_t)((R + rows - 1) / rows) * (size_t)parts * Cout_part * Cin * sizeof(float);
+}
+extern "C" int ptt_linear_wgrad_stack_partials_f32(const float* dZ, int ldz, const float* X, int ldx, int R, int Cout_part, int parts,
+                                                   int Cin, void* ws, size_t ws_bytes, int* nchunks_out, ptt_stream_t stream) {
+    if (!wgrad_stack_ok(R, Cout_part, parts, Cin))
+        return fail(PTT_EUNSUPPORTED, "ptt_linear_wgrad_stack_partials_f32: R=%d Cout_part=%d parts=%d Cin=%d (whole 128-blocks)", R, Cout_part, parts, Cin);
+    const int Cout = Cout_part * parts;
+    if (ldz < Cout || ldx < Cin || !dZ || !X || !nchunks_out) return fail(PTT_EINVAL, "ptt_linear_wgrad_stack_partials_f32: bad argument");
+    if (!ws || ws_bytes < ptt_linear_wgrad_stack_workspace(R, Cout_part, parts, Cin))
+        return fail(PTT_EWORKSPACE, "ptt_linear_wgrad_stack_partials_f32: workspace too small");
+    const int rows = wgrad_chunk_rows(R, Cout_part, Cin), nchunks = (R + rows - 1) / rows;
+    const int nbo = Cout / 128, nbi = Cin / 128;
+    hipStream_t s = as_stream(stream);
+    const int lds = 4 * WG_KC * WG_LD * (int)sizeof(float);
+    const bool vz = (ldz & 3) == 0 && (reinterpret_cast<uintptr_t>(dZ) & 15) == 0;
+    const bool vx = (ldx & 3) == 0 && (reinterpret_cast<uintptr_t>(X) & 15) == 0;
+#define PTT_WGRAD_CASE(VZ, VX)                                                                                        \
+    if (vz == VZ && vx == VX) {                                                                                       \
+        if (int rc = set_lds_limit(reinterpret_cast<const void*>(linear_wgrad_kernel<VZ, VX, 1>), lds)) return rc;    \
+        hipLaunchKernelGGL((linear_wgrad_kernel<VZ, VX, 1>), dim3(nbo * nbi, nchunks), dim3(256), lds, s, dZ, ldz, X, ldx, R, Cout, \
+                           Cin, nbi, rows, static_cast<float*>(ws), nullptr, nullptr, 0, 0);                          \
+    }
+    PTT_WGRAD_CASE(true, true) PTT_WGRAD_CASE(true, false) PTT_WGRAD_CASE(false, true) PTT_WGRAD_CASE(false, false)
+#undef PTT_WGRAD_CASE
+    *nchunks_out = nchunks;
+    return check_launch("linear_wgrad_kernel");
 }
 
 static int linear_wgrad_run(const float* dZ, int ldz, const float* X, int ldx, int R, int Cout, int Cin, float* dW,
diff --git a/ptt_amd/models/transformer_block/multitransformer.py b/ptt_amd/models/transformer_block/multitransformer.py
--- a/ptt_amd/models/transformer_block/multitransformer.py
+++ b/ptt_amd/models/transformer_block/multitransformer.py
@@ -90,9 +90,9 @@
     def _train_rows(self, features, knn_idx, rel, order, start, want_attn):
         H = self.heads
         x = train_ops.rows_linear(self.fc1, features)
-        q, kf, vf = (train_ops.rows_linear(m, x) for m in (self.w_qs, self.w_ks, self.w_vs))
         pos_enc = train_ops.rows_mlp2(self.fc_delta, rel)
-        res, attn = train_ops.attn_core(self.fc_gamma, q, kf, vf, knn_idx, pos_enc, 1.0 / np.sqrt(self.head_dim), order, start, heads=H)
+        res, attn = train_ops.qkv_attn_core(self.w_qs, self.w_ks, self.w_vs, self.fc_gamma, x, knn_idx, pos_enc, 1.0 / np.sqrt(self.head_dim),
+                                            order, start, heads=H)
         res = train_ops.rows_layernorm(self.norm1, train_ops.rows_linear(self.proj, res))
         res = train_ops.rows_layernorm(self.norm2, train_ops.rows_linear(self.fc2, res), residual=features)
         if not want_attn:
diff --git a/ptt_amd/models/transformer_block/variants.py b/ptt_amd/models/transformer_block/variants.py
--- a/ptt_amd/models/transformer_block/variants.py
+++ b/ptt_amd/models/transformer_block/variants.py
@@ -117,12 +117,13 @@
             if xyz.requires_grad:
                 rel = train_ops._KnnRel.apply(xyz, knn_idx, rel)
             x = train_ops.rows_linear(self.fc1, features)
-            q, kf, vf = (train_ops.rows_linear(m, x) for m in (self.w_qs, self.w_ks, self.w_vs))
             pos_enc = train_ops.rows_mlp2(self.fc_delta, rel)
             order, start = ops.scatter_csr(knn_idx.view(knn_idx.shape[0], -1), knn_idx.shape[1])
             if train_ops.ATTN_CORE:
-                res, attn = train_ops.attn_core(self.fc_gamma, q, kf, vf, knn_idx, pos_enc, 1.0 / np.sqrt(self.d_model), order, start)
+                res, attn = train_ops.qkv_attn_core(self.w_qs, self.w_ks, self.w_vs, self.fc_gamma, x, knn_idx, pos_enc,
+                                                    1.0 / np.sqrt(self.d_model), order, start)
             else:
+                q, kf, vf = (train_ops.rows_linear(m, x) for m in (self.w_qs, self.w_ks, self.w_vs))
                 t = train_ops._PairInput.apply(q, kf, knn_idx, pos_enc, order, start)
                 a = train_ops.rows_mlp2(self.fc_gamma, t)
                 res, attn = train_ops._AttnAggregate.apply(a, vf, knn_idx, pos_enc, 1.0 / np.sqrt(self.d_model), order, start)
diff --git a/ptt_amd/ops.py b/ptt_amd/ops.py
--- a/ptt_amd/ops.py
+++ b/ptt_amd/ops.py
@@ -969,6 +969,10 @@
                                                    int(ldo if ldo is not None else N)))
 
 
+def rows_gemm_rounds(rows, K, N):
+    return int(_host("ptt_rows_gemm_rounds", int(rows), int(K), int(N)))
+
+
 def rows_gemm(x, wpacked, cout, in_scale=None, in_shift=None, bias=None, relu=False, residual=None, want_stats=False, out=None):
     _rows(x, "x")
     rows, K = x.shape
@@ -1172,6 +1176,25 @@
     ws = _ws(nb2 if two else _host("ptt_linear_wgrad_workspace", R, Cout, Cin), dz.device)
     _launch("ptt_linear_wgrad2_partials_f32" if two else "ptt_linear_wgrad_partials_f32", dz.device, _ptr(dz), dz.stride(0), _ptr(x), x.stride(0),
             R, Cout, Cin, _ptr(ws), ws.numel() * 8, _ptr(x_scale), _ptr(x_shift), ctypes.byref(nch), timed='ptt_linear_wgrad_f32')
+    return ws, nch.value
+
+
+def linear_wgrad_stack_partials(dz, x, parts):
+    _rows(dz, "dz"); _rows(x, "x")
+    R, Cin, parts = dz.shape[0], x.shape[1], int(parts)
+    if parts < 1 or dz.shape[1] % parts:
+        raise ValueError("linear_wgrad_stack_partials: %d columns in %d parts" % (dz.shape[1], parts))
+    Cout = dz.shape[1] // parts
+    ok2 = (dz.stride(0) % 4 == 0 and x.stride(0) % 4 == 0 and dz.data_ptr() % 16 == 0 and x.data_ptr() % 16 == 0
+           and R * max(dz.stride(0), x.stride(0)) < (1 << 29))
+    two = bool(ok2 and WGRAD2 and _host("ptt_linear_wgrad2_workspace", R, Cout, Cin))
+    nb = _host("ptt_linear_wgrad2_stack_workspace" if two else "ptt_linear_wgrad_stack_workspace", R, Cout, parts, Cin)
+    if not nb:
+        return None
+    nch = ctypes.c_int(0)
+    ws = _ws(nb, dz.device)
+    _launch("ptt_linear_wgrad2_stack_partials_f32" if two else "ptt_linear_wgrad_stack_partials_f32", dz.device, _ptr(dz), dz.stride(0), _ptr(x),
+            x.stride(0), R, Cout, parts, Cin, _ptr(ws), ws.numel() * 8, ctypes.byref(nch), timed='ptt_linear_wgrad_f32')
     return ws, nch.value
 
 
@@ -1296,10 +1319,23 @@
     return out
 
 
+def packed_weight_elems(cout, k):
+    return int(_host("ptt_packed_weight_elems", int(cout), int(k)))
+
+
+def pack_job_rows(jobs):
+    arr = (_lib.PackJob * len(jobs))()
+    for n, job in enumerate(jobs):
+        ptr, off, so, sk, cout, k = job[:6]
+        nts, t0 = (int(job[6]), int(job[7])) if len(job) > 6 else (0, 0)
+        if nts and (cout % 32 or t0 < 0 or t0 + cout // 32 > nts):
+            raise ValueError("pack job %d: rows %d..%d of a stacked weight of %d column tiles" % (n, 32 * t0, 32 * t0 + cout, nts))
+        arr[n] = _lib.PackJob(W=ptr, out_offset=off, stride_out=so, stride_k=sk, Cout=cout, K=k, NT_stack=nts, tile0=t0)
+    return arr
+
+
 def pack_jobs_table(jobs, device):
-    arr = (_lib.PackJob * len(jobs))()
-    for n, (ptr, off, so, sk, cout, k) in enumerate(jobs):
-        arr[n] = _lib.PackJob(W=ptr, out_offset=off, stride_out=so, stride_k=sk, Cout=cout, K=k)
+    arr = pack_job_rows(jobs)
     host = torch.frombuffer(bytearray(bytes(arr)), dtype=torch.uint8)
     return host.to(device)
 
@@ -1393,11 +1429,23 @@
     return order, start
 
 
-def scatter_rows_det(g, idx, N, csr=None, minuend=None, negate=False):
+def scatter_rows_det(g, idx, N, csr=None, minuend=None, negate=False, out=None):
     _chk(g, "g", torch.float32, 3)
     _chk(idx, "idx", torch.int32, 2)
     B, E, C = g.shape
     order, start = csr if csr is not None else scatter_csr(idx, N)
+    if out is not None:
+        if (not out.is_cuda or out.dtype != torch.float32 or tuple(out.shape) != (B, int(N), C) or out.stride(2) != 1
+                or out.stride(0) != int(N) * out.stride(1) or out.data_ptr() % 16):
+            raise ValueError("scatter_rows_det: out must be a 16-byte aligned (B,N,C) column block of a contiguous (B,N,ld) float32 buffer")
+        if minuend is not None:
+            _chk(minuend, "minuend", torch.float32, 3)
+            if tuple(minuend.shape) != (B, int(N), C):
+                raise ValueError("minuend: (B,N,C) expected")
+        neg = int(bool(negate or minuend is not None))
+        _launch("ptt_scatter_rows_csr_ld_f32", g.device, _ptr(g), _ptr(order), _ptr(start), B, int(N), E, C, _ptr(minuend), neg, _ptr(out),
+                out.stride(1))
+        return out
     out = torch.empty((B, int(N), C), dtype=torch.float32, device=g.device)
     if minuend is None and not negate:
         _launch("ptt_scatter_rows_csr_f32", g.device, _ptr(g), _ptr(order), _ptr(start), B, int(N), E, C, _ptr(out))
@@ -1415,15 +1463,24 @@
                 and _host("ptt_rows_gemm_rsum16_supported", x.shape[0], int(K), int(N), x.stride(0)))
 
 
-def rows_gemm_rsum16(x, wpacked, N, residual):
+def _gsum_rows(gsum, groups, N, device):
+    if gsum is None:
+        return torch.empty((groups, int(N)), dtype=torch.float32, device=device)
+    if (not gsum.is_cuda or gsum.dtype != torch.float32 or tuple(gsum.shape) != (groups, int(N)) or gsum.stride(1) != 1
+            or gsum.stride(0) % 4 or gsum.data_ptr() % 16):
+        raise ValueError("rows_gemm_rsum16: gsum must be a 16-byte aligned (rows / 16, N) float32 block with unit column stride")
+    return gsum
+
+
+def rows_gemm_rsum16(x, wpacked, N, residual, gsum=None):
     _rows(x, "x"); _rows(residual, "residual")
     rows, K = x.shape
     if tuple(residual.shape) != (rows, int(N)):
         raise ValueError("rows_gemm_rsum16: residual (rows, N) expected")
     out, plain = (torch.empty((rows, int(N)), dtype=torch.float32, device=x.device) for _ in range(2))
-    gsum = torch.empty((rows // 16, int(N)), dtype=torch.float32, device=x.device)
+    gsum = _gsum_rows(gsum, rows // 16, N, x.device)
     _launch("ptt_rows_gemm_rsum16_f32", x.device, _ptr(x), rows, K, x.stride(0), _ptr(wpacked), int(N), _ptr(residual), residual.stride(0), _ptr(out),
-            int(N), _ptr(plain), int(N), _ptr(gsum), int(N), timed='ptt_linear_f32')
+            int(N), _ptr(plain), int(N), _ptr(gsum), gsum.stride(0), timed='ptt_linear_f32')
     return plain, out, gsum
 
 
@@ -1432,7 +1489,7 @@
                 and _host("ptt_rows_gemm_rsum16_heads_supported", x.shape[0], int(D), int(hd), x.stride(0)))
 
 
-def rows_gemm_rsum16_heads(x, wpacked, hd, residual):
+def rows_gemm_rsum16_heads(x, wpacked, hd, residual, gsum=None):
     _rows(x, "x"); _rows(residual, "residual")
     rows, D = x.shape
     hd = int(hd)
@@ -1441,9 +1498,9 @@
     if hd <= 0 or D % hd or wpacked.numel() < hd * hd:
         raise ValueError("rows_gemm_rsum16_heads: D %% hd == 0 and a packed hd x hd weight expected (D=%d hd=%d)" % (D, hd))
     out, plain = (torch.empty((rows, D), dtype=torch.float32, device=x.device) for _ in range(2))
-    gsum = torch.empty((rows // 16, D), dtype=torch.float32, device=x.device)
+    gsum = _gsum_rows(gsum, rows // 16, D, x.device)
     _launch("ptt_rows_gemm_rsum16_heads_f32", x.device, _ptr(x), rows, D, hd, x.stride(0), _ptr(wpacked), _ptr(residual), residual.stride(0),
-            _ptr(out), D, _ptr(plain), D, _ptr(gsum), D, timed='ptt_linear_f32')
+            _ptr(out), D, _ptr(plain), D, _ptr(gsum), gsum.stride(0), timed='ptt_linear_f32')
     return plain, out, gsum
 
 
@@ -1519,6 +1576,12 @@
 def pt_attn_train_bwd(attn, vf, knn, pos, dres, scale):
     B, N, k, D = attn.shape
     da, dvp = torch.empty_like(attn), torch.empty_like(attn)
+    if not vf.is_contiguous():
+        if tuple(vf.shape) != (B, N, D) or vf.stride(2) != 1 or vf.stride(0) != N * vf.stride(1):
+            raise ValueError("pt_attn_train_bwd: vf must be (B,N,D), dense or a column block of a contiguous (B,N,ld) buffer")
+        _launch("ptt_pt_attn_train_bwd_ld_f32", attn.device, _ptr(attn), _ptr(vf), vf.stride(1), _ptr(knn), _ptr(pos), _ptr(dres), B, N, k, D,
+                float(scale), _ptr(da), _ptr(dvp))
+        return da, dvp
     _launch("ptt_pt_attn_train_bwd_f32", attn.device, _ptr(attn), _ptr(vf), _ptr(knn), _ptr(pos), _ptr(dres), B, N, k, D, float(scale), _ptr(da),
             _ptr(dvp))
     return da, dvp
diff --git a/ptt_amd/train_ops.py b/ptt_amd/train_ops.py
--- a/ptt_amd/train_ops.py
+++ b/ptt_amd/train_ops.py
@@ -64,11 +64,17 @@
 
     def __init__(self):
         self.entries = {}
+        self.stacks = {}
         self.table = None
 
     def register(self, ekey, base, elems):
         if ekey not in self.entries:
             self.entries[ekey] = [weakref.ref(base), int(elems)]
+            self.table = None
+
+    def register_stack(self, skey, bases, elems):
+        if skey not in self.stacks:
+            self.stacks[skey] = [tuple(weakref.ref(b) for b in bases), int(elems)]
             self.table = None
 
     def _build(self, device):
@@ -85,7 +91,17 @@
             keys.append(ekey)
             ptrs.append(base.data_ptr())
             off += elems
-        self.table = (ops.pack_jobs_table(jobs, device), keys, ptrs, off) if jobs else None
+        skeys = []
+        for skey, (refs, elems) in list(self.stacks.items()):
+            bases = [r() for r in refs]
+            if any(b is None or id(b) != i or not b.is_cuda or b.device != device for b, i in zip(bases, skey[0])):
+                del self.stacks[skey]
+                continue
+            jobs += _stack_jobs([b.data_ptr() + o for b, o in zip(bases, skey[1])], skey[2], skey[3], skey[4], off)
+            skeys.append(skey)
+            ptrs.append(tuple(b.data_ptr() for b in bases))
+            off += elems
+        self.table = (ops.pack_jobs_table(jobs, device), keys, ptrs, off, len(jobs), skeys) if jobs else None
 
     def repack(self, device):
         if self.table is not None:
@@ -94,12 +110,17 @@
                 if base is None or base.data_ptr() != ptr:
                     self.table = None
                     break
+        if self.table is not None:
+            for skey, ptr in zip(self.table[5], self.table[2][len(self.table[1]):]):
+                if tuple(None if r() is None else r().data_ptr() for r in self.stacks[skey][0]) != ptr:
+                    self.table = None
+                    break
         if self.table is None:
             self._build(device)
             if self.table is None:
                 return False
-        table, keys, _, total = self.table
-        arena = ops.pack_weights(table, len(keys), torch.empty((total,), dtype=torch.float32, device=device))
+        table, keys, _, total, njobs, skeys = self.table
+        arena = ops.pack_weights(table, njobs, torch.empty((total,), dtype=torch.float32, device=device))
         off = 0
         for ekey in keys:
             ref, elems = self.entries[ekey]
@@ -110,7 +131,75 @@
                 del slot[k]
             slot[(ekey[1], ekey[2], ekey[3], version, ekey[4])] = arena[off:off + elems]
             off += elems
+        for skey in skeys:
+            refs, elems = self.stacks[skey]
+            bases = [r() for r in refs]
+            slot = _pack_slot(bases[0])
+            key = _stack_slot_key(bases, skey)
+            for k in [k for k in slot if k[3] != key[3]]:
+                del slot[k]
+            slot[key] = arena[off:off + elems]
+            off += elems
         return True
+
+
+def _stack_jobs(ptrs, shapes, strides, transposed, off):
+    jobs, done = [], 0
+    kin = shapes[0][1]
+    nt_all = sum(s[0] for s in shapes) // 32
+    for ptr, shape, stride in zip(ptrs, shapes, strides):
+        if transposed:
+            jobs.append((ptr, off + ops.packed_weight_elems(kin, done), stride[1], stride[0], kin, shape[0]))
+        else:
+            jobs.append((ptr, off, stride[0], stride[1], shape[0], kin, nt_all, done // 32))
+        done += shape[0]
+    return jobs
+
+
+def _stack_slot_key(bases, skey):
+    vers = tuple((b._version, b.data_ptr()) for b in bases)
+    return (skey[1], skey[2], skey[3], vers[0], skey[4], ('stack', skey[0], vers[1:]))
+
+
+def stack_packable(Ws):
+    return bool(len(Ws) > 1 and all(W.dim() == 2 and W.is_cuda and W.dtype == torch.float32 and W.device == Ws[0].device
+                                    and W.shape[1] == Ws[0].shape[1] and W.shape[0] % 32 == 0 for W in Ws))
+
+
+def packed_stack(Ws, transpose=False):
+    if _pack_capture is not None:
+        return _pack_capture.get_stack(Ws, transpose)
+    bases = [W._base if W._base is not None else W for W in Ws]
+    skey = _stack_key(Ws, bases, transpose)
+    slot = _pack_slot(bases[0])
+    key = _stack_slot_key(bases, skey)
+    hit = slot.get(key)
+    if hit is not None:
+        return hit
+    device = Ws[0].device
+    plan = _pack_plans.setdefault(device, _PackPlan()) if PACK_PLAN else None
+    if plan is not None and skey in plan.stacks and plan.repack(device):
+        hit = slot.get(key)
+        if hit is not None:
+            return hit
+    for k in [k for k in slot if k[3] != key[3]]:
+        del slot[k]
+    elems = ops.packed_weight_elems(*_stack_dims(skey))
+    jobs = _stack_jobs([W.data_ptr() for W in Ws], skey[2], skey[3], skey[4], 0)
+    hit = slot[key] = ops.pack_weights(ops.pack_jobs_table(jobs, device), len(jobs), torch.empty((elems,), dtype=torch.float32, device=device))
+    if plan is not None:
+        plan.register_stack(skey, bases, elems)
+    return hit
+
+
+def _stack_key(Ws, bases, transpose):
+    return (tuple(id(b) for b in bases), tuple(W.data_ptr() - b.data_ptr() for W, b in zip(Ws, bases)),
+            tuple(tuple(W.shape) for W in Ws), tuple(tuple(W.stride()) for W in Ws), bool(transpose))
+
+
+def _stack_dims(skey):
+    outs, kin = sum(s[0] for s in skey[2]), skey[2][0][1]
+    return (kin, outs) if skey[4] else (outs, kin)
 
 
 FUSED_BN_BWD = os.environ.get("PTT_FUSED_BN_BWD", "1") != "0"
@@ -131,6 +220,9 @@
         for ekey, (ref, elems) in (list(shared.entries.items()) if shared is not None else []):
             if ekey[0] in ids and ref() is not None:
                 self.plan.entries[ekey] = [ref, elems]
+        for skey, (refs, elems) in (list(shared.stacks.items()) if shared is not None else []):
+            if all(i in ids for i in skey[0]) and all(r() is not None for r in refs):
+                self.plan.stacks[skey] = [refs, elems]
         self.plan._build(self.device)
         self.cache, self.arena = {}, None
 
@@ -151,14 +243,7 @@
         hit = self.cache.get(ekey)
         if hit is not None:
             return hit
-        if self.arena is None and self.plan.table is not None:
-            table, keys, _, total = self.plan.table
-            self.arena = ops.pack_weights(table, len(keys), torch.empty((total,), dtype=torch.float32, device=self.device))
-            off = 0
-            for k in keys:
-                elems = self.plan.entries[k][1]
-                self.cache[k] = self.arena[off:off + elems]
-                off += elems
+        if self._pack_arena():
             hit = self.cache.get(ekey)
             if hit is not None:
                 return hit
@@ -166,6 +251,30 @@
         cout, k = (w.shape[1], w.shape[0]) if transpose else w.shape
         so, sk = (w.stride(1), w.stride(0)) if transpose else (w.stride(0), w.stride(1))
         hit = self.cache[ekey] = ops.pack_weight_strided(w, cout, k, so, sk, 1, 0)[0]
+        return hit
+
+    def _pack_arena(self):
+        if self.arena is not None or self.plan.table is None:
+            return False
+        table, keys, _, total, njobs, skeys = self.plan.table
+        self.arena = ops.pack_weights(table, njobs, torch.empty((total,), dtype=torch.float32, device=self.device))
+        off = 0
+        for k in keys:
+            elems = self.plan.entries[k][1]
+            self.cache[k] = self.arena[off:off + elems]
+            off += elems
+        for k in skeys:
+            elems = self.plan.stacks[k][1]
+            self.cache[k] = self.arena[off:off + elems]
+            off += elems
+        return True
+
+    def get_stack(self, Ws, transpose):
+        skey = _stack_key(Ws, [W._base if W._base is not None else W for W in Ws], transpose)
+        self._pack_arena()
+        hit = self.cache.get(skey)
+        if hit is None:
+            raise RuntimeError("PackCapture: a stacked weight the eager steps never packed — a step must have run eagerly before it is captured")
         return hit
 
 
@@ -304,6 +413,20 @@
     ws, nch = ops.linear_wgrad_partials(dz, x, x_scale, x_shift)
     sink.push(loc, ws, nch)
     return None
+
+
+def weight_grad_stack(Ws, dz, x):
+    sink = GradSink.active
+    cout = Ws[0].shape[0]
+    locs = [sink.locate(W) for W in Ws] if sink is not None and WGRAD_STACKED else None
+    if (locs and all(l is not None and l[1] == l[2] == l[3] and l[3] % 4 == 0 for l in locs)
+            and all(a[0] + a[3] == b[0] for a, b in zip(locs, locs[1:])) and all(tuple(W.shape) == tuple(Ws[0].shape) for W in Ws)):
+        got = ops.linear_wgrad_stack_partials(dz, x, len(Ws))
+        if got is not None:
+            n = sum(l[3] for l in locs)
+            sink.push((locs[0][0], n, n, n), got[0], got[1])
+            return [None] * len(Ws)
+    return [weight_grad(W, dz[:, n * cout:(n + 1) * cout], x) for n, W in enumerate(Ws)]
 
 
 def bias_grad(b, g2):
@@ -784,6 +907,104 @@
                            int(heads))
 
 
+QKV_STACKED = os.environ.get("PTT_QKV_STACKED", "1") != "0"
+WGRAD_STACKED = os.environ.get("PTT_WGRAD_STACKED", "1") != "0"
+
+
+class _RowsLinearStack(torch.autograd.Function):
+
+    @staticmethod
+    def forward(ctx, x, *Ws):
+        x2 = x.reshape(-1, x.shape[-1]).contiguous()
+        outs = sum(W.shape[0] for W in Ws)
+        ctx.save_for_backward(x2, *Ws)
+        ctx.Ws, ctx.shape = Ws, x.shape
+        if ops.rows_gemm_rounds(x2.shape[0], x2.shape[1], outs) == 1:
+            y = ops.rows_gemm(x2, packed_stack(Ws), outs)
+        else:
+            y, c0 = torch.empty((x2.shape[0], outs), dtype=torch.float32, device=x2.device), 0
+            for W in Ws:
+                ops.rows_gemm(x2, packed(W), W.shape[0], out=y[:, c0:c0 + W.shape[0]])
+                c0 += W.shape[0]
+        return y.view(*x.shape[:-1], outs)
+
+    @staticmethod
+    def backward(ctx, g):
+        x2, Ws = ctx.saved_tensors[0], ctx.Ws
+        g2 = g.reshape(-1, g.shape[-1]).contiguous()
+        dx = ops.rows_gemm(g2, packed_stack(Ws, True), x2.shape[1]).view(ctx.shape) if ctx.needs_input_grad[0] else None
+        if all(ctx.needs_input_grad[1:]):
+            dWs = weight_grad_stack(Ws, g2, x2)
+        else:
+            cout = Ws[0].shape[0]
+            dWs = [weight_grad(W, g2[:, n * cout:(n + 1) * cout], x2) if ctx.needs_input_grad[1 + n] else None for n, W in enumerate(Ws)]
+        return (dx, *dWs)
+
+
+def rows_linear_stack_usable(layers, x):
+    Ws = [m.weight for m in layers]
+    if any(m.bias is not None for m in layers) or not stack_packable(Ws) or len(set(W.shape[0] for W in Ws)) != 1:
+        return False
+    rows, K, outs = x.numel() // x.shape[-1], x.shape[-1], sum(W.shape[0] for W in Ws)
+    return bool(Ws[0].shape[0] % 4 == 0 and ops.rows_gemm_supported(rows, K, outs, K, outs) and ops.rows_gemm_supported(rows, outs, K, outs, K))
+
+
+class _AttnCoreQkv(torch.autograd.Function):
+
+    @staticmethod
+    def forward(ctx, qkv, knn, pos, W1, b1, W2, b2, scale, order, start, heads=1):
+        ctx.set_materialize_grads(False)
+        qkv, pos = qkv.contiguous(), pos.contiguous()
+        D = qkv.shape[-1] // 3
+        t = ops.pt_pair_input_qkv(qkv, knn, pos, D)
+        x2 = t.view(-1, D // heads)
+        h, a = _mlp2_forward(x2, W1, b1, W2, b2)
+        a = a.view(*t.shape[:-1], W2.shape[0] * heads)
+        res, attn = ops.pt_attn_fwd_qkv(a, qkv, knn, pos, D, scale, want_attn=True)
+        ctx.save_for_backward(x2, h, attn, qkv, knn, pos, order, start, W1, W2)
+        ctx.Ws, ctx.bs, ctx.scale, ctx.heads = (W1, W2), (b1, b2), float(scale), int(heads)
+        ctx.mark_non_differentiable(attn)
+        return res, attn
+
+    @staticmethod
+    def backward(ctx, dres, _dattn):
+        x2, h, attn, qkv, knn, pos, order, start = ctx.saved_tensors[:8]
+        W1, W2 = ctx.Ws
+        B, N, k, D = attn.shape
+        csr = (order, start)
+        dres = dres.contiguous()
+        dqkv = torch.empty_like(qkv)
+        dq_out, dkf_out, dvf_out = dqkv[..., :D], dqkv[..., D:2 * D], dqkv[..., 2 * D:]
+        da, dvp = ops.pt_attn_train_bwd(attn, qkv[..., 2 * D:], knn, pos, dres, ctx.scale)
+        ops.scatter_rows_det(dvp.view(B, N * k, D), knn.view(B, N * k), N, csr, out=dvf_out)
+        heads = ctx.heads
+        dz1, dW1, db1, dW2, db2 = _mlp2_backward(da.view(-1, D // heads), x2, h, W1, ctx.bs[0], W2, ctx.bs[1])
+        D1, Din = W1.shape
+        gsum = dqkv.view(B * N, 3 * D)[:, :D]
+        if heads == 1 and ops.rows_gemm_rsum16_supported(dz1, D1, Din) and k == 16 and Din == D:
+            dt, dpos, _ = ops.rows_gemm_rsum16(dz1, packed(W1, True), Din, dvp.view(-1, D), gsum=gsum)
+            dpos = dpos.view(B, N, k, D)
+        elif heads > 1 and k == 16 and Din * heads == D and ops.rows_gemm_rsum16_heads_supported(dz1.view(-1, D), D, Din):
+            dt, dpos, _ = ops.rows_gemm_rsum16_heads(dz1.view(-1, D), packed(W1, True), Din, dvp.view(-1, D), gsum=gsum)
+            dpos = dpos.view(B, N, k, D)
+        else:
+            dt = lin_rows(dz1, W1, transpose=True).view(B, N, k, D)
+            torch.sum(dt, dim=2, out=dq_out)
+            dpos = dt + dvp
+        ops.scatter_rows_det(dt.view(B, N * k, D), knn.view(B, N * k), N, csr, negate=True, out=dkf_out)
+        return dqkv, None, dpos, dW1, db1, dW2, db2, None, None, None, None
+
+
+def qkv_attn_core(w_qs, w_ks, w_vs, fc_gamma, x, knn, pos, scale, order, start, heads=1):
+    layers = (w_qs, w_ks, w_vs)
+    if QKV_STACKED and rows_linear_stack_usable(layers, x):
+        qkv = _RowsLinearStack.apply(x, *(m.weight for m in layers))
+        return _AttnCoreQkv.apply(qkv, knn, pos, fc_gamma[0].weight, fc_gamma[0].bias, fc_gamma[2].weight, fc_gamma[2].bias, scale, order,
+                                  start, int(heads))
+    q, kf, vf = (rows_linear(m, x) for m in layers)
+    return attn_core(fc_gamma, q, kf, vf, knn, pos, scale, order, start, heads=heads)
+
+
 def pt_block_usable(block, xyz, features):
     return (block.training and xyz.is_cuda and features.dtype == torch.float32 and block.k in (8, 16, 32) and block.d_model % 4 == 0
             and xyz.shape[1] * block.k <= 16384)
```
